# JacobChalk/TIM

Measured on AMD Instinct MI355X. Metric: interval-queries/sec (fwd+bwd), d=512 L=6 EPIC-100 window, higher is better.
Workload: dtype fp16; 1 GPU; C2a: EPIC-100 A+V recognition, d_model 512 (E 1024), 6 layers, 8 heads, 50+50 feature tokens, 15+10 interval queries, train-mode dropout; windows_per_gpu=64, global_batch=64, parallelism=dp1, precision=fp16

## Files before the change

### include/timhip.h

```cpp
#ifndef TIMHIP_H
#define TIMHIP_H

#include <stddef.h>
#include <stdint.h>

#ifdef __cplusplus
extern "C" {
#endif

#define TIMHIP_VERSION 6

enum {
  TIMHIP_OK = 0,
  TIMHIP_EINVAL = -1,
  TIMHIP_EUNSUPPORTED = -2,
  TIMHIP_EWORKSPACE = -3,
  TIMHIP_ELAUNCH = -4,
  TIMHIP_EALIGN = -5
};

enum { TIMHIP_PREC_BF16 = 0, TIMHIP_PREC_BF16X3 = 1, TIMHIP_PREC_FP32 = 2, TIMHIP_PREC_F16 = 3 };

enum {
  TIMHIP_EPI_STORE_T = 0,
  TIMHIP_EPI_RELU_T = 1,
  TIMHIP_EPI_STORE_F32 = 2,
  TIMHIP_EPI_GELU_DROP_T2 = 3,
  TIMHIP_EPI_DROP_RES_F32 = 4,
  TIMHIP_EPI_ADD_F32 = 5,
  TIMHIP_EPI_DGELU_T = 6,
  TIMHIP_EPI_DRELU_T = 7,
  TIMHIP_EPI_ATOMIC_F32 = 8,
  TIMHIP_EPI_SIGMOID_F32 = 9,
  TIMHIP_EPI_DRELU_F32IN_T = 10,
  TIMHIP_EPI_GELU_DROP_G2 = 11,
  TIMHIP_EPI_MULAUX_T = 12,
  TIMHIP_EPI_RELU_SPLIT3_T = 13,
  TIMHIP_EPI_GELU_T = 14
};

typedef struct TimDesc {
  int32_t B;
  int32_t S;
  int32_t F;
  int32_t d;
  int32_t E;
  int32_t H;
  int32_t FF;
  int32_t precision;
  float p_drop;
  uint64_t seed;
  int32_t layer;
  int32_t reserved;
  const float* grad_scale;
} TimDesc;
#define TIMHIP_DESC_ATTN_FP32 1
#define TIMHIP_DESC_ATTN_BWD_ONE_KERNEL 2
#define TIMHIP_DESC_WGRAD_OVERWRITE 4
#define TIMHIP_DESC_WGRAD_SEPARATE 8
#define TIMHIP_DESC_OUTPROJ_SPLIT 16
#define TIMHIP_DESC_INPROJ_SPLIT 32
#define TIMHIP_DESC_L1_SPLIT 64
#define TIMHIP_DESC_L2_SPLIT 128
#define TIMHIP_DESC_STREAM16 0x10000
#define TIMHIP_DESC_STREAM16_IN 0x20000
#define TIMHIP_DESC_STREAM16_OUT 0x40000
#define TIMHIP_DESC_ATTN_KEEP_BITS 0x80000

typedef struct TimLayerParams {
  const void *in_w, *in_wt;
  const void *out_w, *out_wt;
  const void *l1_w, *l1_wt;
  const void *l2_w, *l2_wt;
  const float *in_b, *out_b, *l1_b, *l2_b;
  const float *n1_w, *n1_b, *n2_w, *n2_b;
} TimLayerParams;

typedef struct TimLayerGrads {
  float *in_w, *in_b, *out_w, *out_b, *l1_w, *l1_b, *l2_w, *l2_b;
  float *n1_w, *n1_b, *n2_w, *n2_b;
  float* ln_partials;
} TimLayerGrads;
size_t timhip_layer_ln_partial_bytes(const TimDesc* d);
int timhip_ln_partials_reduce(const float* partials, int nsets, int rows, int cols, float* const* dgamma,
                              float* const* dbeta, void* stream);

int timhip_version(void);
void timhip_reload_env(void);
int timhip_gemm_p8_choice(int epi, int M, int N, int K);
int timhip_build_flags(void);
const char* timhip_strerror(int code);

size_t timhip_layer_saved_bytes(const TimDesc* d);
size_t timhip_layer_workspace_bytes(const TimDesc* d);
enum { TIMHIP_SAVED_QKV = 0, TIMHIP_SAVED_O = 1, TIMHIP_SAVED_Y1 = 2, TIMHIP_SAVED_X1T = 3, TIMHIP_SAVED_H = 4,
       TIMHIP_SAVED_Y2 = 5, TIMHIP_SAVED_FFN_KEEP_BITS = 6, TIMHIP_SAVED_ATTN_KEEP_BITS = 7 };
int timhip_layer_saved_field(const TimDesc* d, int field, size_t* offset, size_t* bytes);

int timhip_cast_weight(int precision, const float* src, int rows, int cols, void* dst, int ld,
                       int transpose, void* stream);

int timhip_cast_weight_both(int precision, const float* src, int rows, int cols, void* plain, int ldp,
                            void* tr, int ldt, void* stream);

typedef struct TimCastItem {
  const float* src;
  void* plain;
  void* tr;
  int32_t rows, cols, ldp, ldt;
} TimCastItem;
int timhip_cast_weights(int precision, const TimCastItem* items, int n, void* stream);

enum { TIMHIP_OPT_STEP = 0, TIMHIP_OPT_LR = 1, TIMHIP_OPT_NORM = 2, TIMHIP_OPT_COEF = 3, TIMHIP_OPT_FOUND_INF = 4,
       TIMHIP_OPT_SKIPPED = 5, TIMHIP_OPT_BC1 = 6, TIMHIP_OPT_BC2_SQRT = 7 };
#define TIMHIP_OPT_STATE_WORDS 8

typedef struct TimOptItem {
  float* p;
  const float* g;
  float* m;
  float* v;
  void* plain;
  void* tr;
  int32_t rows, cols, ldp, ldt;
} TimOptItem;

int timhip_optim_norm_partials(const TimOptItem* items, int n);

int timhip_optim_norm(const TimOptItem* items, int n, double* partials, void* stream);

int timhip_optim_finish(const double* partials, int n_partials, const uint32_t* const* flags, int n_flags, float max_norm,
                        float* const* states, const double* beta1, const double* beta2, int n_states, void* stream);

int timhip_optim_update(int precision, const TimOptItem* items, int n, const float* state, double beta1, double beta2,
                        double eps, double weight_decay, void* stream);

typedef struct TimEpi {
  void* out0;
  void* out1;
  const float* bias;
  const float* res;
  const void* aux;
  int32_t ld0, ld1, ldres, ldaux;
  float p_drop;
  uint32_t site;
  uint64_t seed;
  const void* mask;
  int32_t ldmask;
  int32_t reserved;
  const float* ln_stats;
  const float* ln_w;
  const float* ln_b;
  const float* acc_scale;
  int32_t a_wrap_k;
  int32_t reserved2;
} TimEpi;

typedef struct TimGemmItem {
  const void* A; const void* B;
  int32_t lda, ldb, M, N, K, reserved;
  TimEpi e;
} TimGemmItem;
int timhip_gemm_nt_group(int precision, int epi, const TimGemmItem* items, int n, void* stream);

int timhip_gemm_nt(int precision, int epi, const void* A, int lda, const void* B, int ldb, int M,
                   int N, int K, const TimEpi* e, int splitk, void* stream);

int timhip_transpose(int precision, const void* src, int rows, int cols, int lds, void* dst, int ld,
                     void* stream);

int timhip_colsum(int precision, const void* src, int rows, int cols, int ld, float* out,
                  void* stream);

int timhip_split3_many(int precision, int count, const float* const* src, const int* rows, const int* cols, const int* lds,
                       void* const* dst, const int* ldd, int mode, int relu, void* stream);

int timhip_dp_reduce(int wire_bf16, const void* recv, int world, long long per, float scale, void* out, void* stream);

int timhip_grad_scale(const float* const* cot, const long long* counts, int n, float target, float* out, void* stream);

int timhip_cast_rows(int precision, const float* src, int rows, int cols, int lds, void* dst, int ld,
                     float p_drop, uint64_t seed, uint32_t site, const float* scale, void* stream);
int timhip_cast_rows_pair(int precision, const float* const* src, const int* cols, void* const* dst, const int* ld, int rows,
                          float p_drop, uint64_t seed, const uint32_t* sites, void* stream);

int timhip_layernorm_fwd(int precision, const float* y, int rows, int cols, int ldy, int act,
                         const float* w, const float* b, float* x_f32, int ldx, void* x_T, int ldt,
                         float* stats, void* stream);
int timhip_layernorm_bwd(int precision, const float* dx, int lddx, const float* y, int ldy,
                         const float* stats, int rows, int cols, int act, const float* w,
                         float* dy_f32, int lddy, void* dy_T, int ldt, float p_drop, uint64_t seed,
                         uint32_t site, float* dgamma, float* dbeta, const float* t_scale, void* stream);
int timhip_layernorm_fwd2(int precision, const float* y, int rows, int cols, int ldy, int act, const float* w, const float* b,
                          int split_row, const float* w2, const float* b2, float* x_f32, int ldx, void* x_T, int ldt, float* stats,
                          void* stream);
int timhip_layernorm_bwd2(int precision, const float* dx, int lddx, const float* y, int ldy, const float* stats, int rows, int cols,
                          int act, const float* w, int split_row, const float* w2, float* dy_f32, int lddy, void* dy_T, int ldt,
                          float* dgamma, float* dbeta, float* dgamma2, float* dbeta2, const float* t_scale, void* stream);

int timhip_attention_fwd(const TimDesc* d, const void* qkv, void* o, float* lse, void* stream);
int timhip_attention_fwd_rows(const TimDesc* d, const void* qkv, int s0, void* o_rows, void* stream);
int timhip_attn_keep_bits(const TimDesc* d, int nlayers, void* const* saved, void* stream);
int timhip_attention_bwd(const TimDesc* d, const void* qkv, const void* o, const float* lse,
                         const void* d_o, void* dqkv, void* workspace, size_t workspace_bytes,
                         void* stream);
size_t timhip_attention_bwd_workspace_bytes(const TimDesc* d);

size_t timhip_wgrad_workspace_bytes(int precision, int Nout, int Kout, int M);
int timhip_wgrad(int precision, const void* dY, int ldy, int Nout, const void* X, int ldx, int Kout,
                 int M, float* dW, float* db, void* workspace, size_t workspace_bytes, const float* out_scale, void* stream);

typedef struct TimWgradItem {
  const void* dY;
  const void* X;
  float* dW;
  float* db;
  int32_t ldy, ldx, Nout, Kout;
} TimWgradItem;
size_t timhip_wgrad_group_workspace_bytes(int precision, const TimWgradItem* items, int n, int M);
int timhip_wgrad_group(int precision, const TimWgradItem* items, int n, int M, int accumulate, void* workspace,
                       size_t workspace_bytes, const float* out_scale, void* stream);

int timhip_dropout_rows_bwd(const float* g, int rows, int cols, int ldg, float* dx, int ldx,
                            float p_drop, uint64_t seed, uint32_t site, void* stream);

int timhip_time_l1_fwd(int precision, const float* times, int rows, int d, const float* w,
                       const float* b, void* h, int ld, void* stream);
int timhip_time_l1_fwd_split3(int precision, const float* times, int rows, int d, const float* w, const float* b, void* h3,
                              int ld, void* stream);
int timhip_time_l1_bwd(int precision, const float* times, int rows, int d, const float* w,
                       const void* dh, int ld, float* dw, float* db, float* dt, const float* out_scale, void* stream);

int timhip_dropout_mask(uint64_t seed, uint32_t site, float p, int rows, int cols, uint8_t* out,
                        void* stream);

int timhip_dropout_salt(const unsigned long long* dev_salt);

int timhip_layer_fwd(const TimDesc* d, const TimLayerParams* w, const float* x_in,
                     const void* x_in_T, float* x_out, void* x_out_T, void* saved, void* workspace,
                     size_t workspace_bytes, void* stream);
int timhip_layer_fwd_chained(const TimDesc* d, const TimLayerParams* w, const TimLayerParams* prev_w,
                             const void* prev_saved, const void* x_in_T, float* x_out, void* x_out_T, void* saved,
                             void* stream);
size_t timhip_stack_infer_workspace_bytes(const TimDesc* d, int nlayers, int tail_only);
int timhip_stack_infer(const TimDesc* d, int nlayers, const TimLayerParams* layers, const float* x_in, const void* x_in_T,
                       float* x_out, void* x_out_T, int tail_only, void* workspace, size_t workspace_bytes, void* stream);
int timhip_layer_bwd(const TimDesc* d, const TimLayerParams* w, const void* x_in_T,
                     const void* saved, float* dx_out, float* dx_in, const TimLayerGrads* g,
                     void* workspace, size_t workspace_bytes, void* stream);

size_t timhip_layer_dy_bytes(const TimDesc* d);
// ... 195 lines not shown
```

### tim_amd/_lib.py

```python
import ctypes as C
import os

_HERE = os.path.dirname(os.path.abspath(__file__))
LIB_PATH = os.environ.get("TIM_AMD_LIB") or os.path.join(_HERE, "libtimhip.so")

ABI_VERSION = 6
PREC_BF16, PREC_BF16X3, PREC_FP32, PREC_F16 = 0, 1, 2, 3
PRECISIONS = {"bf16": PREC_BF16, "bf16x3": PREC_BF16X3, "fp32": PREC_FP32, "fp16": PREC_F16}
H16 = (PREC_BF16, PREC_F16)

(EPI_STORE_T, EPI_RELU_T, EPI_STORE_F32, EPI_GELU_DROP_T2, EPI_DROP_RES_F32, EPI_ADD_F32,
 EPI_DGELU_T, EPI_DRELU_T, EPI_ATOMIC_F32, EPI_SIGMOID_F32, EPI_DRELU_F32IN_T, EPI_GELU_DROP_G2, EPI_MULAUX_T, EPI_RELU_SPLIT3_T,
 EPI_GELU_T) = range(15)

SITE_FEAT_V, SITE_FEAT_A, SITE_SEQ = 1, 2, 3
SITE_L_ATTN, SITE_L_DROP1, SITE_L_FFN, SITE_L_DROP2 = 0, 1, 2, 3


def layer_site(layer, which):
    return 16 + 8 * layer + which


SAVED_QKV, SAVED_O, SAVED_Y1, SAVED_X1T, SAVED_H, SAVED_Y2, SAVED_FFN_KEEP_BITS, SAVED_ATTN_KEEP_BITS = range(8)

vp, i32, u32, u64, f32, sz = C.c_void_p, C.c_int32, C.c_uint32, C.c_uint64, C.c_float, C.c_size_t


class TimDesc(C.Structure):
    _fields_ = [("B", i32), ("S", i32), ("F", i32), ("d", i32), ("E", i32), ("H", i32), ("FF", i32),
                ("precision", i32), ("p_drop", f32), ("seed", u64), ("layer", i32), ("reserved", i32),
                ("grad_scale", vp)]


_LP = ["in_w", "in_wt", "out_w", "out_wt", "l1_w", "l1_wt", "l2_w", "l2_wt",
       "in_b", "out_b", "l1_b", "l2_b", "n1_w", "n1_b", "n2_w", "n2_b"]
_LG = ["in_w", "in_b", "out_w", "out_b", "l1_w", "l1_b", "l2_w", "l2_b", "n1_w", "n1_b", "n2_w", "n2_b", "ln_partials"]


class TimLayerParams(C.Structure):
    _fields_ = [(n, vp) for n in _LP]


class TimLayerGrads(C.Structure):
    _fields_ = [(n, vp) for n in _LG]


DESC_ATTN_FP32, DESC_ATTN_BWD_ONE_KERNEL, DESC_WGRAD_OVERWRITE, DESC_WGRAD_SEPARATE, DESC_OUTPROJ_SPLIT = 1, 2, 4, 8, 16
DESC_INPROJ_SPLIT, DESC_L1_SPLIT, DESC_L2_SPLIT = 32, 64, 128
DESC_STREAM16, DESC_STREAM16_IN, DESC_STREAM16_OUT = 0x10000, 0x20000, 0x40000
EINVAL, EUNSUPPORTED, EWORKSPACE, ELAUNCH, EALIGN = -1, -2, -3, -4, -5
DESC_ATTN_KEEP_BITS = 0x80000


class TimCastItem(C.Structure):
    _fields_ = [("src", vp), ("plain", vp), ("tr", vp), ("rows", i32), ("cols", i32), ("ldp", i32), ("ldt", i32)]


class TimOptItem(C.Structure):
    _fields_ = [("p", vp), ("g", vp), ("m", vp), ("v", vp), ("plain", vp), ("tr", vp),
                ("rows", i32), ("cols", i32), ("ldp", i32), ("ldt", i32)]


OPT_STEP, OPT_LR, OPT_NORM, OPT_COEF, OPT_FOUND_INF, OPT_SKIPPED, OPT_BC1, OPT_BC2_SQRT = range(8)
OPT_STATE_WORDS, OPT_MAX_FLAGS, OPT_MAX_STATES = 8, 32, 8


class TimWgradItem(C.Structure):
    _fields_ = [("dY", vp), ("X", vp), ("dW", vp), ("db", vp), ("ldy", i32), ("ldx", i32), ("Nout", i32), ("Kout", i32)]


class TimEpi(C.Structure):
    _fields_ = [("out0", vp), ("out1", vp), ("bias", vp), ("res", vp), ("aux", vp),
                ("ld0", i32), ("ld1", i32), ("ldres", i32), ("ldaux", i32),
                ("p_drop", f32), ("site", u32), ("seed", u64), ("mask", vp), ("ldmask", i32), ("reserved", i32),
                ("ln_stats", vp), ("ln_w", vp), ("ln_b", vp), ("acc_scale", vp), ("a_wrap_k", i32), ("reserved2", i32)]


class TimGemmItem(C.Structure):
    _fields_ = [("A", vp), ("B", vp), ("lda", i32), ("ldb", i32), ("M", i32), ("N", i32), ("K", i32), ("reserved", i32),
                ("e", TimEpi)]


class TimRecHead(C.Structure):
    _fields_ = [("logits", vp), ("sum", vp), ("ld", C.c_int64), ("C", i32), ("pitch", i32)]


REC_MAX_HEADS = 3


class TimAvga(C.Structure):
    _fields_ = [(n, vp) for n in ("video", "audio", "w_video", "w_audio", "w_v", "w_g", "w_v_t", "w_g_t", "w_video_s", "w_audio_s", "b_video",
                                  "b_audio", "w_h")] + [("pitch", C.c_int64)] + \
               [(n, i32) for n in ("R", "S", "Cv", "Ca", "H", "map_size", "ld_audio", "ld_w_video", "ld_w_audio", "ld_w_v", "ld_w_g",
                                   "ld_w_v_t", "ld_w_g_t", "ld_w_video_s", "ld_w_audio_s", "reserved")]


class TimAvgaGrads(C.Structure):
    _fields_ = [(n, vp) for n in ("w_video", "b_video", "w_audio", "b_audio", "w_v", "w_g", "w_h")]


_SIGS = {
    "timhip_version": (C.c_int, []),
    "timhip_strerror": (C.c_char_p, [C.c_int]),
    "timhip_layer_saved_bytes": (sz, [C.POINTER(TimDesc)]),
    "timhip_layer_workspace_bytes": (sz, [C.POINTER(TimDesc)]),
    "timhip_layer_saved_field": (C.c_int, [C.POINTER(TimDesc), i32, C.POINTER(sz), C.POINTER(sz)]),
    "timhip_cast_weight": (C.c_int, [i32, vp, i32, i32, vp, i32, i32, vp]),
    "timhip_cast_weight_both": (C.c_int, [i32, vp, i32, i32, vp, i32, vp, i32, vp]),
    "timhip_cast_weights": (C.c_int, [i32, vp, i32, vp]),
    "timhip_gemm_nt": (C.c_int, [i32, i32, vp, i32, vp, i32, i32, i32, i32, C.POINTER(TimEpi), i32, vp]),
    "timhip_gemm_nt_group": (C.c_int, [i32, i32, vp, i32, vp]),
    "timhip_wgrad_workspace_bytes": (sz, [i32, i32, i32, i32]),
    "timhip_wgrad": (C.c_int, [i32, vp, i32, i32, vp, i32, i32, i32, vp, vp, vp, sz, vp, vp]),
    "timhip_wgrad_group_workspace_bytes": (sz, [i32, vp, i32, i32]),
    "timhip_wgrad_group": (C.c_int, [i32, vp, i32, i32, i32, vp, sz, vp, vp]),
    "timhip_transpose": (C.c_int, [i32, vp, i32, i32, i32, vp, i32, vp]),
    "timhip_colsum": (C.c_int, [i32, vp, i32, i32, i32, vp, vp]),
    "timhip_cast_rows": (C.c_int, [i32, vp, i32, i32, i32, vp, i32, f32, u64, u32, vp, vp]),
    "timhip_dropout_rows_bwd": (C.c_int, [vp, i32, i32, i32, vp, i32, f32, u64, u32, vp]),
    "timhip_layernorm_fwd": (C.c_int, [i32, vp, i32, i32, i32, i32, vp, vp, vp, i32, vp, i32, vp, vp]),
    "timhip_layernorm_bwd": (C.c_int, [i32, vp, i32, vp, i32, vp, i32, i32, i32, vp, vp, i32, vp, i32,
                                       f32, u64, u32, vp, vp, vp, vp]),
    "timhip_attention_fwd": (C.c_int, [C.POINTER(TimDesc), vp, vp, vp, vp]),
    "timhip_attention_fwd_rows": (C.c_int, [C.POINTER(TimDesc), vp, i32, vp, vp]),
    "timhip_attention_bwd": (C.c_int, [C.POINTER(TimDesc), vp, vp, vp, vp, vp, vp, sz, vp]),
    "timhip_attention_bwd_workspace_bytes": (sz, [C.POINTER(TimDesc)]),
    "timhip_time_l1_fwd": (C.c_int, [i32, vp, i32, i32, vp, vp, vp, i32, vp]),
    "timhip_time_l1_fwd_split3": (C.c_int, [i32, vp, i32, i32, vp, vp, vp, i32, vp]),
# ... 9 lines not shown
                                   C.POINTER(TimLayerGrads), vp, sz, vp]),
    "timhip_layer_bwd_split": (C.c_int, [C.POINTER(TimDesc), C.POINTER(TimLayerParams), vp, vp, vp, vp, vp, vp,
                                         C.POINTER(TimLayerGrads), vp, sz, vp]),
    "timhip_layer_bwd_data_split": (C.c_int, [C.POINTER(TimDesc), C.POINTER(TimLayerParams), vp, vp, vp, vp, vp, vp,
                                              C.POINTER(TimLayerGrads), vp, sz, vp]),
    "timhip_layer_dy_bytes": (sz, [C.POINTER(TimDesc)]),
    "timhip_layer_data_workspace_bytes": (sz, [C.POINTER(TimDesc)]),
    "timhip_layer_wgrad_workspace_bytes": (sz, [C.POINTER(TimDesc)]),
    "timhip_layer_bwd_data": (C.c_int, [C.POINTER(TimDesc), C.POINTER(TimLayerParams), vp, vp, vp, vp,
                                        C.POINTER(TimLayerGrads), vp, sz, vp]),
    "timhip_layer_bwd_weights": (C.c_int, [C.POINTER(TimDesc), vp, vp, vp, C.POINTER(TimLayerGrads), vp, sz, vp]),
    "timhip_layer_bwd_weights_pair": (C.c_int, [C.POINTER(TimDesc), vp, vp, vp, C.POINTER(TimLayerGrads), vp, vp, vp,
                                                C.POINTER(TimLayerGrads), vp, sz, vp]),
    "timhip_layer_wgrad_pair_wins": (C.c_int, [C.POINTER(TimDesc)]),
    "timhip_assemble_fwd": (C.c_int, [i32, vp, i32, i32, i32, vp, vp, i32, vp, vp, i32, vp, f32, u64, u32,
                                      vp, vp, vp]),
    "timhip_assemble_bwd": (C.c_int, [vp, i32, i32, i32, vp, i32, i32, f32, u64, u32, vp, vp, vp, vp, vp, vp]),
    "timhip_assemble_fwd_p": (C.c_int, [i32, vp, i32, i32, i32, vp, vp, i32, vp, i32, vp, i32, vp, i32, f32, u64, u32, vp, vp, vp]),
    "timhip_assemble_bwd_p": (C.c_int, [vp, i32, i32, i32, vp, i32, i32, f32, u64, u32, vp, vp, vp, i32, vp, vp, i32, vp]),
    "timhip_gather_rows": (C.c_int, [i32, vp, i32, i32, i32, i32, i32, vp, vp]),
    "timhip_ce_mixup_fwd": (C.c_int, [vp, i32, i32, i32, vp, vp, f32, f32, vp, vp, vp, vp]),
    "timhip_ce_mixup_bwd": (C.c_int, [vp, i32, i32, i32, vp, vp, f32, f32, vp, vp, vp, vp, i32, vp]),
    "timhip_focal_loss_fwd": (C.c_int, [vp, vp, i32, i32, vp, vp, f32, f32, vp, vp, vp]),
    "timhip_focal_loss_bwd": (C.c_int, [vp, vp, i32, i32, vp, vp, f32, f32, vp, vp, vp]),
    "timhip_diou_1d": (C.c_int, [vp, vp, i32, vp, f32, vp, vp, vp, vp]),
    "timhip_det_side_loss_fwd": (C.c_int, [vp, vp, vp, i32, i32, vp, vp, vp, f32, f32, f32, f32, f32, f32, vp, vp, vp]),
    "timhip_det_side_loss_bwd": (C.c_int, [vp, vp, vp, i32, i32, vp, vp, vp, f32, f32, f32, f32, f32, vp, vp, vp, vp, vp]),
    "timhip_softnms_1d_workspace_bytes": (C.c_size_t, [C.c_int64, i32]),
    "timhip_softnms_1d": (C.c_int, [vp, vp, vp, vp, i32, f32, f32, f32, i32, vp, vp, vp, vp, C.c_size_t, vp]),
    "timhip_nms_1d": (C.c_int, [vp, vp, vp, i32, f32, vp, vp, vp, vp]),
    "timhip_det_candidates_count": (C.c_int, [vp, C.c_int64, vp, vp, f32, vp, i32, i32, i32, f32, vp, vp, vp, vp]),
    "timhip_det_candidates_emit": (C.c_int, [vp, C.c_int64, vp, vp, vp, vp, i32, i32, i32, f32, C.c_int64, vp, vp, vp, vp, vp]),
    "timhip_ts_candidates_count": (C.c_int, [vp, C.c_int64, vp, C.c_int64, vp, vp, vp, f32, vp, i32, i32, i32, i32, i32, f32, f32, f32,
                                             vp, vp, vp, vp, vp, vp, vp]),
    "timhip_ts_candidates_emit": (C.c_int, [vp, vp, vp, vp, vp, vp, i32, i32, i32, i32, i32, C.c_int64, vp, vp, vp, vp, vp]),
    "timhip_det_match": (C.c_int, [vp, C.c_int64, vp, vp, vp, vp, vp, C.c_int64, vp, i32, vp, i32, vp, vp, vp, vp]),
    "timhip_det_ap": (C.c_int, [vp, C.c_int64, vp, vp, i32, i32, vp, vp]),
    "timhip_rec_accumulate": (C.c_int, [vp, i32, vp, vp, vp, C.c_int64, i32, i32, i32, i32, vp, vp, vp, vp, vp, vp]),
    "timhip_rec_finalize": (C.c_int, [vp, i32, i32, vp, vp, i32, i32, vp, i32, vp, vp, vp]),
    "timhip_rec_counts": (C.c_int, [vp, vp, vp, i32, vp, vp]),
    "timhip_window_gather": (C.c_int, [vp, i32, i32, vp, vp, i32, vp, i32, vp, vp, vp]),
    "timhip_window_times": (C.c_int, [vp, i32, vp, vp, i32, vp, vp, i32, vp, i32, vp, i32, vp, i32, vp, f32, vp, vp]),
    "timhip_gemm_timing_start": (C.c_int, [i32, C.c_double]),
    "timhip_gemm_timing_stop": (C.c_int, [vp, vp, vp]),
    "timhip_timing_stop_families": (C.c_int, [vp, vp, vp]),
    "timhip_drloc_gather": (C.c_int, [i32, vp, vp, C.c_int64, C.c_int64, i32, i32, i32, vp, vp, i32, vp, i32, vp]),
    "timhip_drloc_scatter_add": (C.c_int, [vp, i32, vp, vp, C.c_int64, C.c_int64, i32, i32, i32, vp, vp, i32, vp]),
    "timhip_scatter_rows_add": (C.c_int, [vp, i32, i32, i32, i32, i32, vp, vp]),
    "timhip_layer_ln_partial_bytes": (sz, [C.POINTER(TimDesc)]),
    "timhip_ln_partials_reduce": (C.c_int, [vp, i32, i32, i32, vp, vp, vp]),
    "timhip_gather_ranges": (C.c_int, [i32, vp, i32, i32, i32, i32, vp, vp, vp, vp]),
    "timhip_layernorm_fwd2": (C.c_int, [i32, vp, i32, i32, i32, i32, vp, vp, i32, vp, vp, vp, i32, vp, i32, vp, vp]),
    "timhip_layernorm_bwd2": (C.c_int, [i32, vp, i32, vp, i32, vp, i32, i32, i32, vp, i32, vp, vp, i32, vp, i32, vp, vp, vp, vp, vp, vp]),
    "timhip_cast_rows_pair": (C.c_int, [i32, vp, vp, vp, vp, i32, f32, u64, vp, vp]),
    "timhip_gather_split3_ranges": (C.c_int, [i32, vp, i32, i32, i32, i32, vp, vp, vp, vp]),
    "timhip_scatter_ranges_add": (C.c_int, [i32, i32, i32, i32, vp, vp, vp, vp, vp]),
    "timhip_dx_init": (C.c_int, [i32, i32, i32, i32, vp, i32, vp, vp, vp, vp, vp]),
    "timhip_sigmoid_bwd_rows": (C.c_int, [i32, vp, vp, i32, i32, vp, i32, vp, vp]),
    "timhip_dx_init_slabs": (C.c_int, [i32, i32, i32, i32, vp, i32, vp, vp, vp, vp, vp, vp]),
    "timhip_cast_rows_many": (C.c_int, [i32, i32, vp, vp, vp, vp, vp, vp, vp]),
    "timhip_grad_scale": (C.c_int, [vp, vp, i32, f32, vp, vp]),
    "timhip_reload_env": (None, []),
    "timhip_build_flags": (C.c_int, []),
    "timhip_attn_keep_bits": (C.c_int, [C.POINTER(TimDesc), i32, vp, vp]),
    "timhip_gemm_p8_choice": (C.c_int, [i32, i32, i32, i32]),
    "timhip_dp_reduce": (C.c_int, [i32, vp, i32, C.c_longlong, f32, vp, vp]),
    "timhip_split3_many": (C.c_int, [i32, i32, vp, vp, vp, vp, vp, vp, i32, i32, vp]),
    "timhip_label_queries": (C.c_int, [vp, vp, vp, i32, i32, i32, i32, f32, vp, vp, vp, vp]),
    "timhip_optim_norm_partials": (C.c_int, [vp, i32]),
    "timhip_optim_norm": (C.c_int, [vp, i32, vp, vp]),
    "timhip_optim_finish": (C.c_int, [vp, i32, vp, i32, f32, vp, vp, vp, i32, vp]),
    "timhip_optim_update": (C.c_int, [i32, vp, i32, vp, C.c_double, C.c_double, C.c_double, C.c_double, vp]),
    "timhip_smooth_one_hot": (C.c_int, [vp, i32, i32, C.c_int64, i32, f32, f32, vp, vp]),
    "timhip_avga_workspace_bytes": (sz, [i32, i32, i32, i32, i32, i32]),
    "timhip_avga_fwd": (C.c_int, [i32, C.POINTER(TimAvga), vp, i32, vp, i32, vp, sz, vp]),
    "timhip_avga_bwd": (C.c_int, [i32, C.POINTER(TimAvga), vp, i32, C.POINTER(TimAvgaGrads), vp, vp, sz, vp]),
}

_lib = None


class TimHipError(RuntimeError):
    pass


def load():
    global _lib
    if _lib is not None:
        return _lib
    if not os.path.exists(LIB_PATH):
        raise TimHipError("libtimhip.so not found at %s: build it with `python -c 'import __graft_entry__ as g; "
                          "g.build()'` (make -C tim_amd/csrc). There is no CPU fallback." % LIB_PATH)
    lib = C.CDLL(LIB_PATH)
    lib.timhip_version.restype = C.c_int
    if lib.timhip_version() != ABI_VERSION:
        raise TimHipError("%s is ABI version %d, this binding speaks %d: rebuild it (make -C tim_amd/csrc%s)"
                          % (LIB_PATH, lib.timhip_version(), ABI_VERSION, " TUNING=1" if "tuning" in LIB_PATH else ""))
    for name, (res, args) in _SIGS.items():
        fn = getattr(lib, name)
        fn.restype = res
        fn.argtypes = args
    _lib = lib
    return lib


def reload_env():
# ... 24 lines not shown
```

### tim_amd/csrc/api.hip

```cpp
#include <atomic>
#include "common.h"

namespace {

struct SavedLayout {
  Field qkv, o, lse, y1, st1, x1t, u, h, y2, st2, ffn_mask, attn_keep;
  size_t total;
};

SavedLayout saved_layout(const TimDesc& d) {
  const size_t M = (size_t)d.B * d.S, ts = opsize(d.precision);
  Arena a;
  SavedLayout L;
  L.qkv = a.take(M * 3 * d.E * ts);
  L.o = a.take(M * d.E * ts);
  L.lse = a.take((size_t)d.B * d.H * d.S * 4);
  L.y1 = a.take(M * d.E * 4);
  L.st1 = a.take(M * 2 * 4);
  L.x1t = a.take(M * d.E * ts);
  L.u = a.take(M * d.FF * ts);
  L.h = a.take(M * d.FF * ts);
  L.y2 = a.take(M * d.E * 4);
  L.st2 = a.take(M * 2 * 4);
  L.ffn_mask = a.take(M * d.FF / 8);
  L.attn_keep = a.take((size_t)d.B * d.H * d.S * 16);
  L.total = a.total();
  return L;
}

struct DyLayout { Field df, du, da, dqkv; size_t total; };
DyLayout dy_layout(const TimDesc& d) {
  const size_t M = (size_t)d.B * d.S, ts = opsize(d.precision);
  Arena a;
  DyLayout L;
  L.df = a.take(M * d.E * ts);
  L.du = a.take(M * d.FF * ts);
  L.da = a.take(M * d.E * ts);
  L.dqkv = a.take(M * 3 * d.E * ts);
  L.total = a.total();
  return L;
}

void layer_products(const TimDesc& d, const void* saved, const void* dy, const void* x_in_T, const TimLayerGrads* g,
                    TimWgradItem it[4]) {
  const SavedLayout L = saved_layout(d);
  const DyLayout Y = dy_layout(d);
  const int E = d.E, FF = d.FF;
  auto in = [](const void* base, const Field& f) { return base ? (const void*)f.at(base) : nullptr; };
  it[0] = TimWgradItem{in(dy, Y.df), in(saved, L.h), g ? g->l2_w : nullptr, g ? g->l2_b : nullptr, E, FF, E, FF};
  it[1] = TimWgradItem{in(dy, Y.du), in(saved, L.x1t), g ? g->l1_w : nullptr, g ? g->l1_b : nullptr, FF, E, FF, E};
  it[2] = TimWgradItem{in(dy, Y.da), in(saved, L.o), g ? g->out_w : nullptr, g ? g->out_b : nullptr, E, E, E, E};
  it[3] = TimWgradItem{in(dy, Y.dqkv), x_in_T, g ? g->in_w : nullptr, g ? g->in_b : nullptr, 3 * E, E, 3 * E, E};
}

int splitk_for(int Mout, int Nout, int Kp) {
  const int tiles = ((Mout + 127) / 128) * ((Nout + 127) / 128);
  int sk = (512 + tiles - 1) / tiles;
  const int maxk = Kp / 256 > 0 ? Kp / 256 : 1;
  if (sk > maxk) sk = maxk;
  if (sk > 8) sk = 8;
  if (sk < 1) sk = 1;
  return sk;
}

struct WgradWs { Field tA, tB, slab; size_t total; };
WgradWs wgrad_ws(int prec, int Nout, int Kout, int M) {
  const size_t Mp = round_up(M, 64), ts = opsize(prec);
  Arena a;
  WgradWs w{};
  if (h16_storage(prec)) {
    w.total = tim_wgrad_tn_ws(Nout, Kout, M);
    return w;
  }
  w.tA = a.take((size_t)Nout * Mp * ts);
  w.tB = a.take((size_t)Kout * Mp * ts);
  const int sk = splitk_for(Nout, Kout, (int)Mp);
  w.slab = a.take(sk > 1 ? (size_t)sk * Nout * Kout * 4 : 0);
  w.total = a.total();
  return w;
}

struct WsLayout {
  Field f32a, f32b, Tb, Tc, wg, attn, lnp;
  size_t total;
};

WsLayout ws_layout(const TimDesc& d) {
  const size_t M = (size_t)d.B * d.S, ts = opsize(d.precision);
  TimWgradItem it[4];
  layer_products(d, nullptr, nullptr, nullptr, nullptr, it);
  size_t wg = h16_storage(d.precision) ? tim_wgrad_group_ws(it, 4, (int)M) : 0;
  for (int i = 0; i < 4; ++i) {
    if (i == 2) continue;
    const size_t one = wgrad_ws(d.precision, it[i].Nout, it[i].Kout, (int)M).total;
    if (one > wg) wg = one;
  }
  Arena a;
  WsLayout L;
  L.f32a = a.take(M * d.E * 4);
  L.f32b = a.take(M * d.E * 4);
  L.Tb = a.take(M * d.E * ts);
  L.Tc = a.take(M * d.E * ts);
  L.wg = a.take(wg);
  L.attn = a.take(tim_attention_bwd_ws(d));
  L.lnp = a.take(tim_layernorm_bwd_ws((int)M, d.E));
  L.total = a.total();
  return L;
}

int check_layer_desc(const TimDesc& d) {
  if (d.B <= 0 || d.S <= 0 || d.F <= 0 || d.F > d.S || d.E <= 0 || d.H <= 0 || d.FF <= 0) return TIMHIP_EINVAL;
  if (d.E % 64 || d.FF % 64 || d.E % d.H) return TIMHIP_EUNSUPPORTED;
  if (!valid_precision(d.precision)) return TIMHIP_EUNSUPPORTED;
  if (d.p_drop < 0.f || d.p_drop >= 1.f) return TIMHIP_EINVAL;
  return TIMHIP_OK;
}

TimEpi epi0() {
  TimEpi e;
  e.out0 = e.out1 = nullptr; e.bias = e.res = nullptr; e.aux = nullptr;
  e.ld0 = e.ld1 = e.ldres = e.ldaux = 0; e.p_drop = 0.f; e.site = 0; e.seed = 0;
  e.mask = nullptr; e.ldmask = 0; e.reserved = 0; e.a_wrap_k = 0; e.reserved2 = 0;
  e.ln_stats = e.ln_w = e.ln_b = nullptr;
  e.acc_scale = nullptr;
  return e;
}

int wgrad(int prec, const void* dY, int ldy, int Nout, const void* X, int ldx, int Kout, int M, float* dW, float* db,
          void* ws, size_t ws_bytes, hipStream_t s, int accumulate = 1, const float* out_scale = nullptr) {
  const int Mp = round_up(M, 64);
  const WgradWs W = wgrad_ws(prec, Nout, Kout, M);
  if (ws_bytes < W.total) return TIMHIP_EWORKSPACE;
  if (h16_storage(prec)) return tim_wgrad_tn_h16(prec, dY, ldy, Nout, X, ldx, Kout, M, dW, db, ws, ws_bytes, s, accumulate, out_scale);
  if (!accumulate || out_scale) return TIMHIP_EUNSUPPORTED;
  char* w = (char*)ws;
  void* tA = W.tA.at(w); void* tB = W.tB.at(w); float* slab = (float*)W.slab.at(w);
  int rc;
  if ((rc = tim_transpose(prec, dY, M, Nout, ldy, tA, Mp, db, s))) return rc;
  if ((rc = tim_transpose(prec, X, M, Kout, ldx, tB, Mp, nullptr, s))) return rc;
  const int sk = splitk_for(Nout, Kout, Mp);
  TimEpi e = epi0();
  if (sk == 1 || (Kout % 4) != 0) {
    e.out0 = dW; e.ld0 = Kout;
    return tim_gemm_nt(prec, TIMHIP_EPI_ATOMIC_F32, tA, Mp, tB, Mp, Nout, Kout, Mp, e, sk, s);
  }
  e.out0 = slab; e.ld0 = Kout;
  if ((rc = tim_gemm_nt(prec, TIMHIP_EPI_STORE_F32, tA, Mp, tB, Mp, Nout, Kout, Mp, e, sk, s))) return rc;
  return tim_slab_reduce(slab, (long long)Nout * Kout, sk, dW, s);
}

struct LayerPass {
  const float* gs_in;
  const float* gs_out;
  int accumulate;
  const unsigned long long* akeep;
};
LayerPass layer_pass(const TimDesc& d, const unsigned long long* keep_bits = nullptr) {
  LayerPass P;
  P.gs_in = (d.precision == TIMHIP_PREC_F16 && d.grad_scale) ? d.grad_scale : nullptr;
  P.gs_out = P.gs_in ? P.gs_in + 1 : nullptr;
  P.accumulate = (d.reserved & TIMHIP_DESC_WGRAD_OVERWRITE) ? 0 : 1;
  P.akeep = ((d.reserved & TIMHIP_DESC_ATTN_KEEP_BITS) && d.p_drop > 0.f) ? keep_bits : nullptr;
  return P;
}

bool wgrad_grouped(const TimDesc& d) { return h16_storage(d.precision) && !(d.reserved & TIMHIP_DESC_WGRAD_SEPARATE); }

int linear_fwd(int prec, int epi, const void* A, const void* W, int M, int N, int K, bool split, TimEpi e, hipStream_t s) {
  if (!split) return tim_gemm_nt(prec, epi, A, K, W, K, M, N, K, e, 1, s);
  e.a_wrap_k = K; e.reserved = 2;
  return tim_gemm_nt(prec, epi, A, K, W, 3 * K, M, N, 2 * K, e, 1, s);
}

}

// ... 49 lines not shown
}

int timhip_dropout_salt(const unsigned long long* dev_salt) {
  tim_salt_ptr = dev_salt;
  return TIMHIP_OK;
}

const char* timhip_strerror(int code) {
  switch (code) {
    case TIMHIP_OK: return "ok";
    case TIMHIP_EINVAL: return "invalid argument (null pointer or bad descriptor field)";
    case TIMHIP_EUNSUPPORTED: return "shape or precision not supported by the gfx950 kernels";
    case TIMHIP_EWORKSPACE: return "workspace too small";
    case TIMHIP_ELAUNCH: return "HIP kernel launch failed";
    case TIMHIP_EALIGN: return "pointer or leading dimension not aligned";
    default: return "unknown timhip error";
  }
}

int timhip_attn_keep_bits(const TimDesc* d, int nlayers, void* const* saved, void* stream) {
  if (!d || !saved || nlayers <= 0) return TIMHIP_EINVAL;
  if (!h16_storage(d->precision) || !(d->p_drop > 0.f) || d->B <= 0 || d->S <= 0 || d->H <= 0 || d->E / d->H != 128 ||
      (d->F + 31) / 32 != 4)
    return TIMHIP_EUNSUPPORTED;
  const SavedLayout L = saved_layout(*d);
  for (int l0 = 0; l0 < nlayers; l0 += 8) {
    unsigned long long* out[8] = {};
    const int n = nlayers - l0 < 8 ? nlayers - l0 : 8;
    for (int i = 0; i < n; ++i) {
      if (!saved[l0 + i]) return TIMHIP_EINVAL;
      out[i] = reinterpret_cast<unsigned long long*>(L.attn_keep.at(saved[l0 + i]));
    }
    const int rc = tim_attn_keep_bits(*d, l0, n, out, (hipStream_t)stream);
    if (rc) return rc;
  }
  return TIMHIP_OK;
}

size_t timhip_layer_saved_bytes(const TimDesc* d) { return d ? saved_layout(*d).total : 0; }

int timhip_layer_saved_field(const TimDesc* d, int field, size_t* offset, size_t* bytes) {
  if (!d || !offset || !bytes) return TIMHIP_EINVAL;
  const SavedLayout L = saved_layout(*d);
  const Field* f;
  switch (field) {
    case TIMHIP_SAVED_QKV: f = &L.qkv; break;
    case TIMHIP_SAVED_O: f = &L.o; break;
    case TIMHIP_SAVED_Y1: f = &L.y1; break;
    case TIMHIP_SAVED_X1T: f = &L.x1t; break;
    case TIMHIP_SAVED_H: f = &L.h; break;
    case TIMHIP_SAVED_Y2: f = &L.y2; break;
    case TIMHIP_SAVED_FFN_KEEP_BITS: f = &L.ffn_mask; break;
    case TIMHIP_SAVED_ATTN_KEEP_BITS: f = &L.attn_keep; break;
    default: return TIMHIP_EINVAL;
  }
  *offset = f->off; *bytes = f->bytes;
  return TIMHIP_OK;
}

int timhip_gemm_nt(int precision, int epi, const void* A, int lda, const void* B, int ldb, int M, int N, int K,
                   const TimEpi* e, int splitk, void* stream) {
  if (!e) return TIMHIP_EINVAL;
  return tim_gemm_nt(precision, epi, A, lda, B, ldb, M, N, K, *e, splitk, (hipStream_t)stream);
}

size_t timhip_wgrad_workspace_bytes(int precision, int Nout, int Kout, int M) {
  return wgrad_ws(precision, Nout, Kout, M).total;
}

int timhip_gemm_nt_group(int precision, int epi, const TimGemmItem* items, int n, void* stream) {
  return tim_gemm_nt_group(precision, epi, items, n, (hipStream_t)stream);
}

size_t timhip_wgrad_group_workspace_bytes(int precision, const TimWgradItem* items, int n, int M) {
  return (h16_storage(precision) && items && n > 0) ? tim_wgrad_group_ws(items, n, M) : 0;
}

int timhip_wgrad_group(int precision, const TimWgradItem* items, int n, int M, int accumulate, void* workspace,
                       size_t workspace_bytes, const float* out_scale, void* stream) {
  return tim_wgrad_group_h16(precision, items, n, M, accumulate, workspace, workspace_bytes, out_scale, (hipStream_t)stream);
}

int timhip_wgrad(int precision, const void* dY, int ldy, int Nout, const void* X, int ldx, int Kout, int M,
                 float* dW, float* db, void* workspace, size_t workspace_bytes, const float* out_scale, void* stream) {
  if (!dY || !X || !dW || !workspace) return TIMHIP_EINVAL;
  return wgrad(precision, dY, ldy, Nout, X, ldx, Kout, M, dW, db, workspace, workspace_bytes, (hipStream_t)stream, 1, out_scale);
}

struct LayerBufs {
  void* qkv; void* o; float* lse; float* y1; float* st1; void* x1t; void* u; void* h; float* y2; float* st2;
  uint8_t* ffn_mask; const unsigned long long* attn_keep;
};

static LayerBufs saved_bufs(const TimDesc& d, void* saved) {
  const SavedLayout L = saved_layout(d);
  return LayerBufs{L.qkv.at(saved), L.o.at(saved), (float*)L.lse.at(saved), (float*)L.y1.at(saved), (float*)L.st1.at(saved),
                   L.x1t.at(saved), L.u.at(saved), L.h.at(saved), (float*)L.y2.at(saved), (float*)L.st2.at(saved),
                   (uint8_t*)L.ffn_mask.at(saved), reinterpret_cast<const unsigned long long*>(L.attn_keep.at(saved))};
}

static int layer_fwd_body(const TimDesc& d, const TimLayerParams* w, const float* x_in, const float* x_in_prenorm,
                          const float* x_in_stats, const float* x_in_lnw, const float* x_in_lnb, const void* x_in_T,
                          float* x_out, void* x_out_T, const LayerBufs& bufs, int s0, hipStream_t s) {
  int rc;
  const int Mall = d.B * d.S, M = d.B * (d.S - s0), E = d.E, FF = d.FF, prec = d.precision;
  void* qkv = bufs.qkv; void* o = bufs.o; float* y1 = bufs.y1; float* st1 = bufs.st1; void* x1t = bufs.x1t;
  void* u = bufs.u; void* h = bufs.h; float* y2 = bufs.y2; float* st2 = bufs.st2;

  auto split = [&](int flag) { return (d.reserved & flag) != 0 && h16_storage(prec); };
  TimEpi e = epi0();
  e.out0 = qkv; e.ld0 = 3 * E; e.bias = w->in_b;
  if ((rc = linear_fwd(prec, TIMHIP_EPI_STORE_T, x_in_T, w->in_w, Mall, 3 * E, E, split(TIMHIP_DESC_INPROJ_SPLIT), e, s))) return rc;
  if ((rc = tim_attention_fwd(d, qkv, o, bufs.lse, s, layer_pass(d, bufs.attn_keep).akeep, s0))) return rc;
  e = epi0();
  e.out0 = y1; e.ld0 = E; e.bias = w->out_b; e.ldres = E;
  if (x_in) {
    e.res = x_in;
  } else {
    e.res = x_in_prenorm; e.ln_stats = x_in_stats; e.ln_w = x_in_lnw; e.ln_b = x_in_lnb;
  }
  e.p_drop = d.p_drop; e.seed = d.seed; e.site = layer_site(d.layer, SITE_L_DROP1);
  uint8_t* fmask = d.p_drop > 0.f ? bufs.ffn_mask : nullptr;
  const bool fuse_ln = tim_knobs().fuse_ln == 1;
  const uint32_t* ln_run_if = nullptr;
  bool fused1 = false;
  if (fuse_ln && h16_storage(prec) && !split(TIMHIP_DESC_OUTPROJ_SPLIT)) {
    TimLnFuse lf{x1t, E, nullptr, 0, st1, w->n1_w, w->n1_b, fmask, FF, d.p_drop, d.seed, layer_site(d.layer, SITE_L_FFN)};
    rc = tim_gemm_nt_fuse_ln(prec, o, E, w->out_w, E, M, E, E, e, lf, &ln_run_if, s);
    if (rc == TIMHIP_OK) fused1 = true;
    else if (rc != TIMHIP_EUNSUPPORTED) return rc;
  }
  if (!fused1 && (rc = linear_fwd(prec, TIMHIP_EPI_DROP_RES_F32, o, w->out_w, M, E, E, split(TIMHIP_DESC_OUTPROJ_SPLIT), e, s))) return rc;
  if ((rc = tim_layernorm_fwd(prec, y1, M, E, E, 0, w->n1_w, w->n1_b, nullptr, 0, x1t, E, st1, s, fmask, FF, d.p_drop, d.seed,
                              layer_site(d.layer, SITE_L_FFN), fused1 ? ln_run_if : nullptr))) return rc;
  e = epi0();
  e.out0 = h; e.ld0 = FF; e.bias = w->l1_b;
  const int epi1 = u ? TIMHIP_EPI_GELU_DROP_G2 : TIMHIP_EPI_GELU_T;
  if (u) {
    e.out1 = u; e.ld1 = FF;
    e.p_drop = d.p_drop; e.seed = d.seed; e.site = layer_site(d.layer, SITE_L_FFN);
    e.mask = fmask; e.ldmask = FF / 8;
  }
  if ((rc = linear_fwd(prec, epi1, x1t, w->l1_w, M, FF, E, split(TIMHIP_DESC_L1_SPLIT), e, s))) return rc;
  e = epi0();
  e.out0 = y2; e.ld0 = E; e.bias = w->l2_b; e.ldres = E;
  e.res = y1; e.ln_stats = st1; e.ln_w = w->n1_w; e.ln_b = w->n1_b;
  e.p_drop = d.p_drop; e.seed = d.seed; e.site = layer_site(d.layer, SITE_L_DROP2);
  bool fused2 = false;
  if (fuse_ln && h16_storage(prec) && !split(TIMHIP_DESC_L2_SPLIT)) {
    TimLnFuse lf{x_out_T, E, x_out, E, st2, w->n2_w, w->n2_b, nullptr, 0, 0.f, 0, 0};
    rc = tim_gemm_nt_fuse_ln(prec, h, FF, w->l2_w, FF, M, E, FF, e, lf, &ln_run_if, s);
    if (rc == TIMHIP_OK) fused2 = true;
    else if (rc != TIMHIP_EUNSUPPORTED) return rc;
  }
  if (!fused2 && (rc = linear_fwd(prec, TIMHIP_EPI_DROP_RES_F32, h, w->l2_w, M, E, FF, split(TIMHIP_DESC_L2_SPLIT), e, s))) return rc;
  return tim_layernorm_fwd(prec, y2, M, E, E, 0, w->n2_w, w->n2_b, x_out, E, x_out_T, E, st2, s, nullptr, 0, 0.f, 0, 0,
                           fused2 ? ln_run_if : nullptr);
}

int timhip_layer_fwd(const TimDesc* dp, const TimLayerParams* w, const float* x_in, const void* x_in_T, float* x_out,
                     void* x_out_T, void* saved, void* workspace, size_t workspace_bytes, void* stream) {
  (void)workspace; (void)workspace_bytes;
  if (!dp || !w || !x_in || !x_in_T || !x_out_T || !saved) return TIMHIP_EINVAL;
  int rc = check_layer_desc(*dp);
  if (rc) return rc;
  return layer_fwd_body(*dp, w, x_in, nullptr, nullptr, nullptr, nullptr, x_in_T, x_out, x_out_T, saved_bufs(*dp, saved), 0,
                        (hipStream_t)stream);
}

int timhip_layer_fwd_chained(const TimDesc* dp, const TimLayerParams* w, const TimLayerParams* prev_w, const void* prev_saved,
                             const void* x_in_T, float* x_out, void* x_out_T, void* saved, void* stream) {
  if (!dp || !w || !prev_w || !prev_saved || !x_in_T || !x_out_T || !saved) return TIMHIP_EINVAL;
  int rc = check_layer_desc(*dp);
  if (rc) return rc;
  const SavedLayout L = saved_layout(*dp);
  return layer_fwd_body(*dp, w, nullptr, (const float*)L.y2.at(prev_saved), (const float*)L.st2.at(prev_saved), prev_w->n2_w,
                        prev_w->n2_b, x_in_T, x_out, x_out_T, saved_bufs(*dp, saved), 0, (hipStream_t)stream);
}

struct InferLayout { Field qkv, o, y1, st1, x1t, h, y2, st2, xt, resg, stg; size_t total; };
static InferLayout infer_layout(const TimDesc& d, int tail_only) {
  const size_t M = (size_t)d.B * d.S, Mt = (size_t)d.B * (d.S - d.F), ts = opsize(d.precision);
  Arena a;
  InferLayout L;
  L.qkv = a.take(M * 3 * d.E * ts);
  L.o = a.take(M * d.E * ts);
  L.y1 = a.take(M * d.E * 4);
  L.st1 = a.take(M * 2 * 4);
  L.x1t = a.take(M * d.E * ts);
  L.h = a.take(M * d.FF * ts);
  L.y2 = a.take(M * d.E * 4);
  L.st2 = a.take(M * 2 * 4);
  L.xt = a.take(M * d.E * ts);
  L.resg = a.take(tail_only ? Mt * d.E * 4 : 0);
  L.stg = a.take(tail_only ? Mt * 2 * 4 : 0);
  L.total = a.total();
  return L;
}

size_t timhip_stack_infer_workspace_bytes(const TimDesc* d, int nlayers, int tail_only) {
  (void)nlayers;
  return (d && check_layer_desc(*d) == TIMHIP_OK) ? infer_layout(*d, tail_only).total : 0;
}

int timhip_stack_infer(const TimDesc* dp, int nlayers, const TimLayerParams* layers, const float* x_in, const void* x_in_T,
                       float* x_out, void* x_out_T, int tail_only, void* workspace, size_t workspace_bytes, void* stream) {
  if (!dp || !layers || nlayers <= 0 || !x_in || !x_in_T || !x_out_T || !workspace) return TIMHIP_EINVAL;
  TimDesc d = *dp;
  int rc = check_layer_desc(d);
  if (rc) return rc;
  if (d.p_drop != 0.f || (tail_only && d.S == d.F)) return TIMHIP_EINVAL;
  const InferLayout L = infer_layout(d, tail_only);
  if (workspace_bytes < L.total) return TIMHIP_EWORKSPACE;
  hipStream_t s = (hipStream_t)stream;
  void* ws = workspace;
  const LayerBufs bufs{L.qkv.at(ws), L.o.at(ws), nullptr, (float*)L.y1.at(ws), (float*)L.st1.at(ws), L.x1t.at(ws), nullptr,
                       L.h.at(ws), (float*)L.y2.at(ws), (float*)L.st2.at(ws), nullptr, nullptr};
  d.reserved &= ~TIMHIP_DESC_ATTN_KEEP_BITS;
  for (int l = 0; l < nlayers; ++l) {
    const bool last = l == nlayers - 1;
    const int s0 = (last && tail_only) ? d.F : 0;
    d.layer = l;
    const float* res = l == 0 ? x_in : nullptr;
    const float* pre = l == 0 ? nullptr : bufs.y2;
    const float* pst = l == 0 ? nullptr : bufs.st2;
    if (s0) {
      float* resg = (float*)L.resg.at(ws); float* stg = (float*)L.stg.at(ws);
      if ((rc = timhip_gather_rows(TIMHIP_PREC_FP32, l == 0 ? x_in : pre, d.B, d.S, d.E, s0, d.S - s0, resg, stream))) return rc;
      if (l > 0 && (rc = timhip_gather_rows(TIMHIP_PREC_FP32, pst, d.B, d.S, 2, s0, d.S - s0, stg, stream))) return rc;
      if (l == 0) res = resg; else { pre = resg; pst = stg; }
    }
    const void* in_T = l == 0 ? x_in_T : (const void*)L.xt.at(ws);
    if ((rc = layer_fwd_body(d, &layers[l], res, pre, pst, l ? layers[l - 1].n2_w : nullptr, l ? layers[l - 1].n2_b : nullptr, in_T,
                             last ? x_out : nullptr, last ? x_out_T : (void*)L.xt.at(ws), bufs, s0, s))) return rc;
  }
  return TIMHIP_OK;
}

size_t timhip_layer_ln_partial_bytes(const TimDesc* d) { return d ? 2 * tim_layernorm_bwd_ws(d->B * d->S, d->E) : 0; }
size_t timhip_layer_dy_bytes(const TimDesc* d) { return d ? dy_layout(*d).total : 0; }
size_t timhip_layer_workspace_bytes(const TimDesc* d) { return d ? ws_layout(*d).total + dy_layout(*d).total : 0; }
size_t timhip_layer_data_workspace_bytes(const TimDesc* d) { return d ? ws_layout(*d).total : 0; }
size_t timhip_layer_wgrad_workspace_bytes(const TimDesc* d) { return d ? ws_layout(*d).wg.bytes : 0; }

static int layer_bwd_data_impl(const TimDesc& d, const TimLayerParams* w, const void* saved, const float* dx_out,
                               const void* dx_out_add, float* dx_in, void* dx_in_add, void* dy, const TimLayerGrads* g,
                               void* workspace, size_t workspace_bytes, hipStream_t s) {
  int rc = check_layer_desc(d);
  if (rc) return rc;
  const WsLayout W = ws_layout(d);
  if (workspace_bytes < W.total) return TIMHIP_EWORKSPACE;
  const int M = d.B * d.S, E = d.E, FF = d.FF, prec = d.precision;
  const SavedLayout L = saved_layout(d);
  const DyLayout Y = dy_layout(d);
  const void* qkv = L.qkv.at(saved); const void* o = L.o.at(saved); const float* lse = (const float*)L.lse.at(saved);
  const float* y1 = (const float*)L.y1.at(saved); const float* st1 = (const float*)L.st1.at(saved);
  const void* u = L.u.at(saved);
  const float* y2 = (const float*)L.y2.at(saved); const float* st2 = (const float*)L.st2.at(saved);
  void* ws = workspace;
  float* f32a = (float*)W.f32a.at(ws); float* f32b = (float*)W.f32b.at(ws); float* lnp = (float*)W.lnp.at(ws);
  void* Tb = W.Tb.at(ws); void* Tc = W.Tc.at(ws);
  void* df = Y.df.at(dy); void* du = Y.du.at(dy); void* da = Y.da.at(dy); void* dqkv = Y.dqkv.at(dy);
  const LayerPass P = layer_pass(d, reinterpret_cast<const unsigned long long*>(L.attn_keep.at(saved)));
  const float* gs_in = P.gs_in; const float* gs_out = P.gs_out;

  const bool s16 = gs_in != nullptr && (d.reserved & TIMHIP_DESC_STREAM16) != 0;
  const bool s16_in = s16 && (d.reserved & TIMHIP_DESC_STREAM16_IN) != 0;
  const bool s16_out = s16 && (d.reserved & TIMHIP_DESC_STREAM16_OUT) != 0;
  if (((d.reserved & (TIMHIP_DESC_STREAM16_IN | TIMHIP_DESC_STREAM16_OUT)) != 0 && !s16) || (s16_out && !dx_in_add)) return TIMHIP_EINVAL;
  if ((rc = tim_layernorm_bwd(prec, dx_out, E, y2, E, st2, M, E, 0, w->n2_w, f32a, E, df, E, d.p_drop, d.seed,
                              layer_site(d.layer, SITE_L_DROP2), g->n2_w, g->n2_b,
                              g->ln_partials ? g->ln_partials : lnp, s, g->ln_partials != nullptr, gs_in,
                              dx_out_add, E, gs_out, (s16_in ? 1 : 0) | (s16 ? 2 : 0)))) return rc;
  TimEpi e = epi0();
  e.out0 = du; e.ld0 = FF; e.aux = u; e.ldaux = FF;
  if ((rc = tim_gemm_nt(prec, TIMHIP_EPI_MULAUX_T, df, E, w->l2_wt, E, M, FF, E, e, 1, s))) return rc;
  const bool branch_split = prec != TIMHIP_PREC_BF16;
  e = epi0();
  if (branch_split) {
    e.out0 = Tb; e.ld0 = E;
    if ((rc = tim_gemm_nt(prec, TIMHIP_EPI_STORE_T, du, FF, w->l1_wt, FF, M, E, FF, e, 1, s))) return rc;
  } else {
    e.out0 = f32b; e.ld0 = E; e.res = f32a; e.ldres = E;
    if ((rc = tim_gemm_nt(prec, TIMHIP_EPI_ADD_F32, du, FF, w->l1_wt, FF, M, E, FF, e, 1, s))) return rc;
  }
  const float* ln1_in = branch_split ? f32a : f32b;
  float* dy1 = dx_in_add ? dx_in : (branch_split ? f32b : f32a);
  if ((rc = tim_layernorm_bwd(prec, ln1_in, E, y1, E, st1, M, E, 0, w->n1_w, dy1, E, da, E, d.p_drop, d.seed,
                              layer_site(d.layer, SITE_L_DROP1), g->n1_w, g->n1_b,
                              g->ln_partials ? g->ln_partials + tim_layernorm_bwd_ws(M, E) / sizeof(float) : lnp, s,
                              g->ln_partials != nullptr, gs_in, branch_split ? Tb : nullptr, E, gs_out,
                              (s16 ? 1 : 0) | (s16_out ? 2 : 0)))) return rc;
  e = epi0();
  e.out0 = Tc; e.ld0 = E;
  if ((rc = tim_gemm_nt(prec, TIMHIP_EPI_STORE_T, da, E, w->out_wt, E, M, E, E, e, 1, s))) return rc;
  if ((rc = tim_attention_bwd(d, qkv, o, lse, Tc, dqkv, W.attn.at(ws), W.attn.bytes, s, P.akeep))) return rc;
  e = epi0();
  if (dx_in_add) {
    e.out0 = dx_in_add; e.ld0 = E;
    return tim_gemm_nt(prec, TIMHIP_EPI_STORE_T, dqkv, 3 * E, w->in_wt, 3 * E, M, E, 3 * E, e, 1, s);
  }
  e.out0 = dx_in; e.ld0 = E; e.res = dy1; e.ldres = E; e.acc_scale = gs_out;
  return tim_gemm_nt(prec, TIMHIP_EPI_ADD_F32, dqkv, 3 * E, w->in_wt, 3 * E, M, E, 3 * E, e, 1, s);
}

int timhip_layer_bwd_data(const TimDesc* dp, const TimLayerParams* w, const void* saved, float* dx_out, float* dx_in,
                          void* dy, const TimLayerGrads* g, void* workspace, size_t workspace_bytes, void* stream) {
  if (!dp || !w || !saved || !dx_out || !dx_in || !dy || !g || !workspace) return TIMHIP_EINVAL;
  return layer_bwd_data_impl(*dp, w, saved, dx_out, nullptr, dx_in, nullptr, dy, g, workspace, workspace_bytes, (hipStream_t)stream);
}

int timhip_layer_bwd_data_split(const TimDesc* dp, const TimLayerParams* w, const void* saved, const float* dx_out,
                                const void* dx_out_add, float* dx_in, void* dx_in_add, void* dy, const TimLayerGrads* g,
                                void* workspace, size_t workspace_bytes, void* stream) {
  if (!dp || !w || !saved || !dx_out || !dx_in || !dy || !g || !workspace) return TIMHIP_EINVAL;
  return layer_bwd_data_impl(*dp, w, saved, dx_out, dx_out_add, dx_in, dx_in_add, dy, g, workspace, workspace_bytes,
                             (hipStream_t)stream);
}

int timhip_layer_bwd_weights(const TimDesc* dp, const void* x_in_T, const void* saved, const void* dy,
                             const TimLayerGrads* g, void* workspace, size_t workspace_bytes, void* stream) {
  if (!dp || !x_in_T || !saved || !dy || !g || !workspace) return TIMHIP_EINVAL;
  const TimDesc& d = *dp;
  int rc = check_layer_desc(d);
  if (rc) return rc;
  const int M = d.B * d.S;
  hipStream_t s = (hipStream_t)stream;
  const LayerPass P = layer_pass(d);
  TimWgradItem it[4];
  layer_products(d, saved, dy, x_in_T, g, it);
  if (wgrad_grouped(d)) return tim_wgrad_group_h16(d.precision, it, 4, M, P.accumulate, workspace, workspace_bytes, P.gs_out, s);
  for (const TimWgradItem& p : it)
    if ((rc = wgrad(d.precision, p.dY, p.ldy, p.Nout, p.X, p.ldx, p.Kout, M, p.dW, p.db, workspace, workspace_bytes, s, P.accumulate,
                    P.gs_out))) return rc;
  return TIMHIP_OK;
}

int timhip_layer_bwd_weights_pair(const TimDesc* dp, const void* x_in_T_a, const void* saved_a, const void* dy_a, const TimLayerGrads* ga,
                                  const void* x_in_T_b, const void* saved_b, const void* dy_b, const TimLayerGrads* gb,
                                  void* workspace, size_t workspace_bytes, void* stream) {
  if (!dp || !x_in_T_a || !saved_a || !dy_a || !ga || !x_in_T_b || !saved_b || !dy_b || !gb || !workspace) return TIMHIP_EINVAL;
  const TimDesc& d = *dp;
  int rc = check_layer_desc(d);
  if (rc) return rc;
  if (!wgrad_grouped(d)) return TIMHIP_EUNSUPPORTED;
// ... 44 lines not shown
```

### tim_amd/csrc/common.h

```cpp
#pragma once
#include <hip/hip_runtime.h>
#include <stdint.h>

#include "../../include/timhip.h"

typedef __bf16 bf16_t;
typedef _Float16 f16_t;
template <typename T> using vec8 = T __attribute__((ext_vector_type(8)));
template <typename T> using vec4 = T __attribute__((ext_vector_type(4)));
typedef vec8<bf16_t> bf16x8_t;
typedef vec4<bf16_t> bf16x4_t;
typedef float f32x4_t __attribute__((ext_vector_type(4)));
typedef float f32x16_t __attribute__((ext_vector_type(16)));
typedef short s16x4_t __attribute__((ext_vector_type(4)));

#define TIM_CHECK_LAUNCH()                                   \
  do {                                                       \
    if (hipGetLastError() != hipSuccess) return TIMHIP_ELAUNCH; \
  } while (0)

static inline int round_up(int x, int m) { return (x + m - 1) / m * m; }
__host__ __device__ static inline size_t align_up(size_t x, size_t a) { return (x + a - 1) / a * a; }

struct Field {
// ... 89 lines not shown
__host__ __device__ __forceinline__ Philox4 philox4x32_7(uint64_t seed, uint32_t site, uint64_t ctr) {
  uint32_t k0 = (uint32_t)seed, k1 = (uint32_t)(seed >> 32);
  uint32_t c0 = (uint32_t)ctr, c1 = (uint32_t)(ctr >> 32), c2 = site, c3 = 0x7149u;
#pragma unroll
  for (int r = 0; r < PHILOX_ROUNDS; ++r) {
    const uint64_t p0 = (uint64_t)0xD2511F53u * (uint64_t)c0, p1 = (uint64_t)0xCD9E8D57u * (uint64_t)c2;
    const uint32_t hi0 = (uint32_t)(p0 >> 32), lo0 = (uint32_t)p0, hi1 = (uint32_t)(p1 >> 32), lo1 = (uint32_t)p1;
    uint32_t n0 = hi1 ^ c1 ^ k0, n1 = lo1, n2 = hi0 ^ c3 ^ k1, n3 = lo0;
    c0 = n0; c1 = n1; c2 = n2; c3 = n3;
    k0 += 0x9E3779B9u; k1 += 0xBB67AE85u;
  }
  return Philox4{c0, c1, c2, c3};
}

extern const unsigned long long* tim_salt_ptr;
struct TimSeed {
  uint64_t base;
  const unsigned long long* salt;
  __host__ __device__ TimSeed() : base(0), salt(nullptr) {}
  __host__ TimSeed(uint64_t s) : base(s), salt(tim_salt_ptr) {}
  __device__ __forceinline__ operator uint64_t() const { return salt ? base + (uint64_t)*salt : base; }
};

__host__ __device__ __forceinline__ uint32_t drop_threshold(float p) {
  double t = (double)p * 4294967296.0;
  if (t < 0) t = 0;
  if (t > 4294967295.0) t = 4294967295.0;
  return (uint32_t)t;
}

__device__ __forceinline__ void drop_mask4(uint64_t seed, uint32_t site, uint64_t q, uint32_t thr,
                                           float scale, float& m0, float& m1, float& m2, float& m3) {
  const Philox4 r = philox4x32_7(seed, site, q >> 1);
  const uint32_t a = (q & 1) ? r.z : r.x, b = (q & 1) ? r.w : r.y, t = thr >> 16;
  m0 = (a & 0xffffu) >= t ? scale : 0.f;
  m1 = (a >> 16) >= t ? scale : 0.f;
  m2 = (b & 0xffffu) >= t ? scale : 0.f;
  m3 = (b >> 16) >= t ? scale : 0.f;
}
__device__ __forceinline__ void drop_mask4_words(uint32_t a, uint32_t b, uint32_t thr, float scale, float& m0, float& m1,
                                                 float& m2, float& m3) {
  const uint32_t t = thr >> 16;
  m0 = (a & 0xffffu) >= t ? scale : 0.f;
  m1 = (a >> 16) >= t ? scale : 0.f;
  m2 = (b & 0xffffu) >= t ? scale : 0.f;
  m3 = (b >> 16) >= t ? scale : 0.f;
}
__device__ __forceinline__ float drop_mask1(uint64_t seed, uint32_t site, uint64_t idx, uint32_t thr, float scale) {
  const Philox4 r = philox4x32_7(seed, site, idx >> 3);
  const int e = (int)(idx & 7), wsel = e >> 1;
  const uint32_t w = wsel == 0 ? r.x : (wsel == 1 ? r.y : (wsel == 2 ? r.z : r.w));
  return ((w >> (16 * (e & 1))) & 0xffffu) >= (thr >> 16) ? scale : 0.f;
}
__device__ __forceinline__ uint32_t drop_bits8(uint64_t seed, uint32_t site, uint64_t c, uint32_t thr) {
  const Philox4 r = philox4x32_7(seed, site, c);
  const uint32_t t = thr >> 16;
  return ((r.x & 0xffffu) >= t ? 1u : 0u) | ((r.x >> 16) >= t ? 2u : 0u) | ((r.y & 0xffffu) >= t ? 4u : 0u) |
         ((r.y >> 16) >= t ? 8u : 0u) | ((r.z & 0xffffu) >= t ? 16u : 0u) | ((r.z >> 16) >= t ? 32u : 0u) |
         ((r.w & 0xffffu) >= t ? 64u : 0u) | ((r.w >> 16) >= t ? 128u : 0u);
}

__device__ __forceinline__ uint32_t drop_bits32(uint64_t seed, uint32_t site, uint64_t q0, uint32_t thr) {
  uint32_t bits = 0;
#pragma unroll
  for (int j = 0; j < 4; ++j) bits |= drop_bits8(seed, site, (q0 >> 1) + j, thr) << (8 * j);
  return bits;
}
__device__ __forceinline__ void drop_mask4_bits(uint32_t nib, float scale, float& m0, float& m1, float& m2, float& m3) {
  m0 = (nib & 1u) ? scale : 0.f;
  m1 = (nib & 2u) ? scale : 0.f;
  m2 = (nib & 4u) ? scale : 0.f;
  m3 = (nib & 8u) ? scale : 0.f;
}

struct PerDeviceOnce {
  bool done[32] = {};
  bool first() {
    int dev = 0;
    (void)hipGetDevice(&dev);
    dev = dev < 0 ? 0 : (dev > 31 ? 31 : dev);
    if (done[dev]) return false;
    done[dev] = true;
    return true;
  }
};

enum {
  SITE_FEAT_V = 1, SITE_FEAT_A = 2, SITE_SEQ = 3,
  SITE_L_BASE = 16, SITE_L_ATTN = 0, SITE_L_DROP1 = 1, SITE_L_FFN = 2, SITE_L_DROP2 = 3, SITE_L_STRIDE = 8
};
static inline uint32_t layer_site(int layer, int which) {
  return SITE_L_BASE + (uint32_t)layer * SITE_L_STRIDE + (uint32_t)which;
}

__device__ __forceinline__ float erf_half_f(float x, float& e) {
  const float z = fabsf(x) * 0.70710678118654752440f;
  const float t = __builtin_amdgcn_rcpf(fmaf(0.3275911f, z, 1.0f));
  e = __expf(-0.5f * x * x);
  float p = fmaf(1.061405429f, t, -1.453152027f);
  p = fmaf(p, t, 1.421413741f);
  p = fmaf(p, t, -0.284496736f);
  p = fmaf(p, t, 0.254829592f);
  const float r = fmaf(-p * t, e, 1.0f);
  return copysignf(r, x);
}
__device__ __forceinline__ float gelu_f(float x) {
  float e;
  return 0.5f * x * (1.0f + erf_half_f(x, e));
}
__device__ __forceinline__ float gelu_grad_f(float x) {
  const float kInvSqrt2Pi = 0.3989422804014327f;
  float e;
// ... 127 lines not shown
  asm volatile("s_waitcnt vmcnt(%0)" ::"n"(N) : "memory");
}

struct TimGemmScope {
  TimGemmScope(double flops, hipStream_t s, int family = 0);
  ~TimGemmScope();
  int slot;
  hipStream_t stream;
};

int tim_gemm_nt(int precision, int epi, const void* A, int lda, const void* B, int ldb, int M, int N,
                int K, const TimEpi& e, int splitk, hipStream_t s);
int tim_gemm_nt_group(int precision, int epi, const TimGemmItem* items, int n, hipStream_t s);
bool tim_gemm_pp_wins(int M, int N, int K, int splitk);
int tim_gemm_p8_choice(int epi, int M, int N, int K);
struct TimLnFuse {
  void* xt; int ldt; float* xf; int ldx; float* stats; const float* g; const float* b;
  uint8_t* mask_out; int mask_cols; float mask_p; uint64_t mask_seed; uint32_t mask_site;
};
int tim_gemm_nt_pp_ln(int precision, const void* A, int lda, const void* B, int ldb, int M, int N, int K, const void* epi_dev,
                      const TimLnFuse& lf, const uint32_t** fail, hipStream_t s);
int tim_gemm_nt_fuse_ln(int precision, const void* A, int lda, const void* B, int ldb, int M, int N, int K, const TimEpi& te,
                        const TimLnFuse& lf, const uint32_t** fail, hipStream_t s);
int tim_gemm_nt_pp(int precision, int epi, const void* A, int lda, const void* B, int ldb, int M, int N, int K, const void* epi_dev,
                   hipStream_t s);
int tim_transpose(int precision, const void* src, int rows, int cols, int lds, void* dst, int ld,
                  float* colsum, hipStream_t s);
int tim_slab_reduce(const float* slab, long long n, int nslab, float* dW, hipStream_t s);
size_t tim_wgrad_tn_ws(int Nout, int Kout, int M);
int tim_wgrad_tn_h16(int precision, const void* dY, int ldy, int Nout, const void* X, int ldx, int Kout, int M, float* dW,
                     float* db, void* ws, size_t ws_bytes, hipStream_t s, int accumulate = 1, const float* out_scale = nullptr);
size_t tim_wgrad_group_ws(const TimWgradItem* it, int n, int M);
int tim_wgrad_group_splits(const TimWgradItem* it, int n, int M);
int tim_wgrad_group_h16(int precision, const TimWgradItem* it, int n, int M, int accumulate, void* ws, size_t ws_bytes,
                        const float* out_scale, hipStream_t s);
bool tim_wgrad_pp_wins(const TimWgradItem* it, int n, int M);
int tim_wgrad_group_pp(int precision, const TimWgradItem* it, int n, int M, int accumulate, const float* out_scale, hipStream_t s);
bool tim_wgrad_p8_wins(const TimWgradItem* it, int n, int M);
int tim_wgrad_group_p8(int precision, const TimWgradItem* it, int n, int M, int accumulate, const float* out_scale, hipStream_t s);
int tim_colsum(int precision, const void* src, int rows, int cols, int ld, float* out, hipStream_t s);
int tim_layernorm_fwd(int precision, const float* y, int rows, int cols, int ldy, int act,
                      const float* w, const float* b, float* x_f32, int ldx, void* x_T, int ldt,
                      float* stats, hipStream_t s, uint8_t* mask_out = nullptr, int mask_cols = 0, float mask_p = 0.f,
                      uint64_t mask_seed = 0, uint32_t mask_site = 0,
                      const uint32_t* run_if = nullptr,
                      int split_row = 0, const float* w2 = nullptr, const float* b2 = nullptr);
int tim_layernorm_bwd(int precision, const float* dx, int lddx, const float* y, int ldy,
                      const float* stats, int rows, int cols, int act, const float* w, float* dy_f32,
                      int lddy, void* dy_T, int ldt, float p_drop, uint64_t seed, uint32_t site,
                      float* dgamma, float* dbeta, float* partial_ws, hipStream_t s, bool defer_colsum = false,
                      const float* t_scale = nullptr,
                      const void* add_T = nullptr, int ldadd = 0, const float* add_scale = nullptr,
                      int stream16 = 0,
                      int split_row = 0, const float* w2 = nullptr, float* dgamma2 = nullptr, float* dbeta2 = nullptr);
size_t tim_layernorm_bwd_ws(int rows, int cols);
int tim_layernorm_bwd_blocks(int rows);
int tim_attention_fwd(const TimDesc& d, const void* qkv, void* o, float* lse, hipStream_t s, const unsigned long long* kbits = nullptr,
                      int s0 = 0);
int tim_attention_bwd(const TimDesc& d, const void* qkv, const void* o, const float* lse,
                      const void* d_o, void* dqkv, void* ws, size_t ws_bytes, hipStream_t s, const unsigned long long* kbits = nullptr);
int tim_attn_keep_bits(const TimDesc& d, int first_layer, int n, unsigned long long* const* out, hipStream_t s);
size_t tim_attention_bwd_ws(const TimDesc& d);

static inline bool h16_storage(int precision) { return precision == TIMHIP_PREC_BF16 || precision == TIMHIP_PREC_F16; }
static inline bool f32_storage(int precision) { return !h16_storage(precision); }
static inline bool valid_precision(int precision) { return precision >= TIMHIP_PREC_BF16 && precision <= TIMHIP_PREC_F16; }
#define DISPATCH_T(prec, ...)                                           \
  do {                                                                  \
    if (f32_storage(prec)) { using T = float; __VA_ARGS__; }            \
    else if ((prec) == TIMHIP_PREC_F16) { using T = f16_t; __VA_ARGS__; } \
    else { using T = bf16_t; __VA_ARGS__; }                             \
  } while (0)
#define DISPATCH_H16(precision, ...)                                   \
  do {                                                                 \
    if ((precision) == TIMHIP_PREC_F16) { using HT = f16_t; __VA_ARGS__; } \
    else { using HT = bf16_t; __VA_ARGS__; }                            \
  } while (0)
static inline size_t opsize(int precision) { return f32_storage(precision) ? 4 : 2; }
```

### tim_amd/csrc/gemm.hip

```cpp
#include <stdlib.h>

#include "gemm_epi.h"

namespace {

template <typename HT, int EPI, int BM, int BN, int WM, int WN, int BKT, int NST, int GM, int ABL = 0>
__device__ __forceinline__ void gemm_nt_h16_body(
    const HT* __restrict__ A, int lda, const HT* __restrict__ B, int ldb, int M, int N,
    int K, int ksteps_per_split, EpiDev e, int t, int zsplit) {
  constexpr int NW = WM * WN;
  constexpr int TM = BM / WM / 32, TN = BN / WN / 32;
  constexpr int ROWB = BKT * 2;
  constexpr int NCH = ROWB / 16;
  constexpr int RPI = 1024 / ROWB;
  constexpr int A_BYTES = BM * ROWB, B_BYTES = BN * ROWB, ST_BYTES = A_BYTES + B_BYTES;
  constexpr int A_INSTR = BM / RPI / NW, B_INSTR = BN / RPI / NW, LPS = A_INSTR + B_INSTR;
  static_assert(A_INSTR >= 1 && B_INSTR >= 1, "tile too small for the wave count");
  extern __shared__ __attribute__((aligned(16))) char lds[];

  const int tid = threadIdx.x, lane = tid & 63;
  const int wave = __builtin_amdgcn_readfirstlane(tid >> 6);
  const int wm = wave / WN, wn = wave % WN;

  const int tiles_n = (N + BN - 1) / BN, tiles_m = (M + BM - 1) / BM;
// ... 231 lines not shown
#pragma unroll
    for (int i = 0; i < TN; ++i)
#pragma unroll
      for (int q = 0; q < 4; ++q)
        *reinterpret_cast<float4*>(ep + frow * EP_LD + i * 32 + 8 * q + 4 * fhalf) =
            make_float4(acc[i][j][4 * q] * asc, acc[i][j][4 * q + 1] * asc, acc[i][j][4 * q + 2] * asc, acc[i][j][4 * q + 3] * asc);
    asm volatile("s_waitcnt lgkmcnt(0)" ::: "memory");
    if (epi_has_oct(EPI) && e.vec8) {
      constexpr int OPR = EP_COLS / 8;
#pragma unroll
      for (int it = 0; it < 32 * OPR / 64; ++it) {
        const int idx = it * 64 + lane;
        const int row = idx / OPR, ch = idx % OPR;
        const float4 lo = *reinterpret_cast<const float4*>(ep + row * EP_LD + ch * 8);
        const float4 hi = *reinterpret_cast<const float4*>(ep + row * EP_LD + ch * 8 + 4);
        const int m = m0 + wm * (BM / WM) + j * 32 + row;
        const int n = n0 + wn * (BN / WN) + ch * 8;
        if (m < M && n + 7 < N) {
          epi_oct<EPI, HT>(e, m, n, N, lo, hi, mbyte[j][it], pre_aux, abuf[j % PD][PRE_AUX ? it : 0], pre_b8, bias8[0], bias8[1]);
        } else if (m < M) {
          if (n < N) epi_quad<EPI, HT>(e, m, n, N, lo.x, lo.y, lo.z, lo.w);
          if (n + 4 < N) epi_quad<EPI, HT>(e, m, n + 4, N, hi.x, hi.y, hi.z, hi.w);
        }
      }
    } else {
      constexpr int NITQ_ = 32 * CPR / 64;
      bool has_k = false;
      if constexpr (EPI == TIMHIP_EPI_DROP_RES_F32 && (NITQ_ % 2) == 0) has_k = e.thr != 0u && !e.mask && e.vec && (N & 7) == 0 && e.pair;
      auto quad = [&](int it, bool hk, float4 kf) {
        const int idx = it * 64 + lane;
        const int row = idx / CPR, ch = idx % CPR;
        const float4 v = *reinterpret_cast<const float4*>(ep + row * EP_LD + ch * 4);
        const int m = m0 + wm * (BM / WM) + j * 32 + row;
        const int n = n0 + wn * (BN / WN) + ch * 4;
        if (m < M && n < N)
          epi_quad<EPI, HT>(e, m, n, N, v.x, v.y, v.z, v.w, pre_res && n + 3 < N, rbuf[j % PD][PRE_RES ? it : 0],
                                pre_b4 && n + 3 < N, bias4, pre_ln && pre_gb && n + 3 < N, sbuf[j % PD][PRE_RES ? it : 0],
                                lng, lnb, hk, kf);
      };
      if (has_k) {
        if constexpr ((NITQ_ % 2) == 0) {
#pragma unroll
          for (int it = 0; it < NITQ_; it += 2) {
            const int idx = (it + (lane & 1)) * 64 + (lane & ~1);
            const long long m_ = m0 + wm * (BM / WM) + j * 32 + idx / CPR, n_ = n0 + wn * (BN / WN) + (idx % CPR) * 4;
            const Philox4 r = philox4x32_7(e.seed, e.site, (uint64_t)(m_ * (long long)N + n_) >> 3);
            const bool odd = (lane & 1) != 0;
            const uint32_t sa = odd ? r.x : r.z, sb = odd ? r.y : r.w;
            const uint32_t pa = (uint32_t)__builtin_amdgcn_mov_dpp((int)sa, 0xB1, 0xF, 0xF, true);
            const uint32_t pb = (uint32_t)__builtin_amdgcn_mov_dpp((int)sb, 0xB1, 0xF, 0xF, true);
            float4 ka, kb;
            drop_mask4_words(odd ? pa : r.x, odd ? pb : r.y, e.thr, e.scale, ka.x, ka.y, ka.z, ka.w);
            drop_mask4_words(odd ? r.z : pa, odd ? r.w : pb, e.thr, e.scale, kb.x, kb.y, kb.z, kb.w);
            quad(it, true, ka);
            quad(it + 1, true, kb);
          }
        }
      } else {
#pragma unroll
        for (int it = 0; it < NITQ_; ++it) quad(it, false, make_float4(1.f, 1.f, 1.f, 1.f));
      }
    }
    asm volatile("s_waitcnt lgkmcnt(0)" ::: "memory");
  });
  if constexpr (PROF) {
    asm volatile("s_waitcnt vmcnt(0)" ::: "memory");
    const long long t_end = __builtin_readcyclecounter();
    if (tid == 0 && e.aux) {
      unsigned long long* c = (unsigned long long*)e.aux;
      atomicAdd(c + 0, (unsigned long long)t_wait);
      atomicAdd(c + 1, (unsigned long long)t_issue);
      atomicAdd(c + 2, (unsigned long long)t_mma);
      atomicAdd(c + 3, (unsigned long long)(t_end - t_loop_end));
      atomicAdd(c + 4, (unsigned long long)(t_end - t_begin));
      atomicAdd(c + 5, 1ull);
      atomicAdd(c + 6, (unsigned long long)(wall_clock64() - w_begin));
    }
  }
}

template <typename HT, int EPI, int BM, int BN, int WM, int WN, int BKT, int NST, int GM, int ABL = 0>
__global__ __launch_bounds__(WM* WN * 64) void gemm_nt_h16_kernel(
    const HT* __restrict__ A, int lda, const HT* __restrict__ B, int ldb, int M, int N,
    int K, int ksteps_per_split, EpiDev e) {
  const int tiles = ((M + BM - 1) / BM) * ((N + BN - 1) / BN);
  gemm_nt_h16_body<HT, EPI, BM, BN, WM, WN, BKT, NST, GM, ABL>(A, lda, B, ldb, M, N, K, ksteps_per_split, e,
                                                           xcd_remap(blockIdx.x, tiles), (int)blockIdx.z);
}

constexpr int GG_MAX = 6;
struct GemmGroupDev {
  const void* A[GG_MAX]; const void* B[GG_MAX];
  int lda[GG_MAX], ldb[GG_MAX], M[GG_MAX], N[GG_MAX], K[GG_MAX], tile0[GG_MAX + 1];
  EpiDev e[GG_MAX];
  int n;
};
template <typename HT, int EPI, int BM, int BN, int WM, int WN, int BKT, int NST>
__global__ __launch_bounds__(WM* WN * 64) void gemm_nt_group_kernel(const GemmGroupDev g) {
  const int t = blockIdx.x;
  int i = 0;
#pragma unroll
  for (int k = 1; k < GG_MAX; ++k)
    if (k < g.n && t >= g.tile0[k]) i = k;
  gemm_nt_h16_body<HT, EPI, BM, BN, WM, WN, BKT, NST, 1, 0>((const HT*)g.A[i], g.lda[i], (const HT*)g.B[i], g.ldb[i], g.M[i], g.N[i], g.K[i],
                                                        g.K[i] / BK, g.e[i], t - g.tile0[i], 0);
}
// ... 274 lines not shown
        case 11: launch_h16<bf16_t, EPI, 128, 128, 2, 2, 64, 2, 4>(A, lda, B, ldb, M, N, K, e, splitk, s); break;
        case 12: launch_h16<bf16_t, EPI, 128, 128, 2, 2, 64, 2, 16>(A, lda, B, ldb, M, N, K, e, splitk, s); break;
        case 13: launch_h16<bf16_t, EPI, 128, 128, 2, 2, 64, 2, 39>(A, lda, B, ldb, M, N, K, e, splitk, s); break;
        case 10: launch_h16<bf16_t, EPI, 128, 128, 2, 2, 32, 3, 8>(A, lda, B, ldb, M, N, K, e, splitk, s); break;
        case 14: launch_h16<bf16_t, EPI, 160, 128, 1, 4, 64, 2, 1>(A, lda, B, ldb, M, N, K, e, splitk, s); break;
        case 19: launch_h16<bf16_t, EPI, 192, 128, 2, 2, 64, 2, 1>(A, lda, B, ldb, M, N, K, e, splitk, s); break;
        case 22: launch_h16<bf16_t, EPI, 320, 128, 2, 4, 64, 2, 1>(A, lda, B, ldb, M, N, K, e, splitk, s); break;
        case 24: launch_h16<bf16_t, EPI, 160, 128, 1, 4, 64, 3, 1>(A, lda, B, ldb, M, N, K, e, splitk, s); break;
        case 25: launch_h16<bf16_t, EPI, 192, 128, 1, 4, 64, 2, 1>(A, lda, B, ldb, M, N, K, e, splitk, s); break;
        default: launch_h16<bf16_t, EPI, 128, 128, 2, 2, 64, 2, 1>(A, lda, B, ldb, M, N, K, e, splitk, s); break;
      }
    } else
#endif
    {
      (void)variant;
      const long long t128 = (long long)((M + 127) / 128) * ((N + 127) / 128) * splitk;
      DISPATCH_H16(precision,
        if (t128 <= 256 && M > 64) {
          const int nst = small_nst((long long)((M + 63) / 64) * ((N + 127) / 128) * splitk);
          if (nst >= 4 && tim_knobs().gemm_small_w8 != 0) launch_h16<HT, EPI, 64, 128, 2, 4, 64, 4, 1>(A, lda, B, ldb, M, N, K, e, splitk, s);
          else if (nst >= 4) launch_h16<HT, EPI, 64, 128, 1, 4, 64, 4, 1>(A, lda, B, ldb, M, N, K, e, splitk, s);
          else if (nst == 3) launch_h16<HT, EPI, 64, 128, 1, 4, 64, 3, 1>(A, lda, B, ldb, M, N, K, e, splitk, s);
          else launch_h16<HT, EPI, 64, 128, 1, 4, 64, 2, 1>(A, lda, B, ldb, M, N, K, e, splitk, s);
        } else if (tall_tile_wins(M, N, splitk))
          launch_h16<HT, EPI, 160, 128, 1, 4, 64, 2, 1>(A, lda, B, ldb, M, N, K, e, splitk, s);
        else
          launch_h16<HT, EPI, 128, 128, 2, 2, 64, 2, 1>(A, lda, B, ldb, M, N, K, e, splitk, s));
    }
  }
  if (hipGetLastError() != hipSuccess) return TIMHIP_ELAUNCH;
  return TIMHIP_OK;
}

}

static int prepare_gemm(int precision, int epi, const void* A, int lda, const void* B, int ldb, int M, int N, int K,
                        const TimEpi& te, int splitk, EpiDev& e) {
  if (!A || !B || !te.out0) return TIMHIP_EINVAL;
  if (M <= 0 || N <= 0 || K <= 0) return TIMHIP_EINVAL;
  if (!valid_precision(precision)) return TIMHIP_EUNSUPPORTED;
  const int Kp = round_up(K, 64);
  if (te.a_wrap_k < 0 || te.a_wrap_k % 64 || (te.a_wrap_k > 0 && (Kp != 2 * te.a_wrap_k || !h16_storage(precision) || splitk > 1)))
    return TIMHIP_EUNSUPPORTED;
  if (lda % 64 || ldb % 64 || lda < (te.a_wrap_k > 0 ? te.a_wrap_k : Kp) || ldb < Kp) return TIMHIP_EALIGN;
  if (((uintptr_t)A | (uintptr_t)B) & 15) return TIMHIP_EALIGN;
  if ((size_t)M * lda * 2 >= (1ull << 32) || (size_t)N * ldb * 2 >= (1ull << 32)) return TIMHIP_EUNSUPPORTED;
  if (splitk > 1 && epi != TIMHIP_EPI_ATOMIC_F32 && epi != TIMHIP_EPI_STORE_F32) return TIMHIP_EINVAL;
  e.out0 = te.out0; e.out1 = te.out1; e.bias = te.bias; e.res = te.res; e.aux = te.aux;
  e.ld0 = te.ld0; e.ld1 = te.ld1; e.ldres = te.ldres; e.ldaux = te.ldaux;
  e.thr = te.p_drop > 0.f ? drop_threshold(te.p_drop) : 0u;
  e.scale = te.p_drop > 0.f ? 1.f / (1.f - te.p_drop) : 1.f;
  e.site = te.site; e.seed = te.seed;
  e.mask = (const uint8_t*)te.mask; e.ldmask = te.ldmask;
  e.ln_stats = te.ln_stats; e.ln_w = te.ln_w; e.ln_b = te.ln_b;
  e.acc_scale = te.acc_scale;
  e.a_wrap = te.a_wrap_k / 64;
  e.pair = tim_knobs().epi_pair;
  if (e.ln_stats && (epi != TIMHIP_EPI_DROP_RES_F32 || !e.res || !e.ln_w || !e.ln_b)) return TIMHIP_EINVAL;
  if (epi == TIMHIP_EPI_RELU_SPLIT3_T && (!h16_storage(precision) || e.out1 || e.ld1 % 64 || e.ld1 < N || e.ld0 < 3 * e.ld1 || splitk > 1))
    return TIMHIP_EINVAL;
  e.slab_stride = splitk > 1 ? (long long)M * te.ld0 : 0;

  bool vec = (e.ld0 % 4 == 0) && (((uintptr_t)e.out0 & 15) == 0);
  if (e.out1) vec = vec && (e.ld1 % 4 == 0) && (((uintptr_t)e.out1 & 15) == 0);
  if (e.res) vec = vec && (e.ldres % 4 == 0) && (((uintptr_t)e.res & 15) == 0);
  if (e.aux) vec = vec && (e.ldaux % 4 == 0) && (((uintptr_t)e.aux & 15) == 0);
  if (e.bias) vec = vec && (((uintptr_t)e.bias & 15) == 0);
  e.vec = vec ? 1 : 0;
  bool vec8 = vec && h16_storage(precision) && (e.ld0 % 8 == 0);
  if (e.out1) vec8 = vec8 && (e.ld1 % 8 == 0);
  if (e.aux) vec8 = vec8 && (e.ldaux % 8 == 0);
  e.vec8 = vec8 ? 1 : 0;
  if (e.thr != 0u && (N % 4) != 0) return TIMHIP_EUNSUPPORTED;
  return TIMHIP_OK;
}

int tim_gemm_nt_group(int precision, int epi, const TimGemmItem* items, int n, hipStream_t s) {
  if (!h16_storage(precision)) return TIMHIP_EUNSUPPORTED;
  if (!items || n < 1 || n > GG_MAX) return TIMHIP_EINVAL;
  if (epi != TIMHIP_EPI_STORE_F32 && epi != TIMHIP_EPI_ADD_F32 && epi != TIMHIP_EPI_STORE_T && epi != TIMHIP_EPI_RELU_T)
    return TIMHIP_EUNSUPPORTED;
  GemmGroupDev g;
  g.n = n;
  g.tile0[0] = 0;
  double flops = 0.0;
  for (int i = 0; i < GG_MAX; ++i) {
    if (i >= n) {
      g.A[i] = g.B[i] = nullptr; g.lda[i] = g.ldb[i] = g.M[i] = g.N[i] = g.K[i] = 0; g.tile0[i + 1] = g.tile0[i];
      g.e[i] = g.e[0];
      continue;
    }
    const TimGemmItem& t = items[i];
    const int rc = prepare_gemm(precision, epi, t.A, t.lda, t.B, t.ldb, t.M, t.N, t.K, t.e, 1, g.e[i]);
    if (rc) return rc;
    g.A[i] = t.A; g.B[i] = t.B; g.lda[i] = t.lda; g.ldb[i] = t.ldb;
    g.M[i] = t.M; g.N[i] = t.N; g.K[i] = round_up(t.K, 64);
    g.tile0[i + 1] = g.tile0[i] + ((t.M + 63) / 64) * ((t.N + 127) / 128);
    flops += 2.0 * t.M * t.N * t.K / (t.reserved > 1 ? t.reserved : 1);
  }
  TimGemmScope timing(flops, s);
  if (g.tile0[n] <= 512 && epi == TIMHIP_EPI_ADD_F32) {
    for (int i = 0; i < n; ++i) g.tile0[i + 1] = g.tile0[i] + ((items[i].M + 63) / 64) * ((items[i].N + 63) / 64);
    for (int i = n; i < GG_MAX; ++i) g.tile0[i + 1] = g.tile0[n];
    DISPATCH_H16(precision, hipLaunchKernelGGL((gemm_nt_group_kernel<HT, TIMHIP_EPI_ADD_F32, 64, 64, 2, 2, 64, 2>),
                                               dim3((unsigned)g.tile0[n]), dim3(256), (size_t)2 * (64 + 64) * 64 * 2, s, g));
    return hipGetLastError() == hipSuccess ? TIMHIP_OK : TIMHIP_ELAUNCH;
// ... 68 lines not shown
```

### tim_amd/csrc/gemm_epi.h

```cpp
#pragma once
#include <utility>
#include "common.h"

namespace {


struct EpiDev {
  void* out0; void* out1;
  const float* bias; const float* res; const void* aux;
  int ld0, ld1, ldres, ldaux;
  uint32_t thr; float scale; uint32_t site; TimSeed seed;
  const uint8_t* mask; int ldmask;
  const float* ln_stats; const float* ln_w; const float* ln_b;
  const float* acc_scale;
  int vec;
  int vec8;
  long long slab_stride;
  int pair;
  int a_wrap;
};

#ifndef TIMHIP_NT_MASK
#define TIMHIP_NT_MASK 3
#endif
template <typename T>
__device__ __forceinline__ void nt_store4(T* p, float a, float b, float c, float d) {
  if constexpr ((sizeof(T) == 4 && !(TIMHIP_NT_MASK & 4)) || (sizeof(T) == 2 && !(TIMHIP_NT_MASK & 1))) {
    store4<T>(p, a, b, c, d);
  } else if constexpr (sizeof(T) == 4) {
    typedef float f4_t __attribute__((ext_vector_type(4)));
    f4_t v = {a, b, c, d};
    __builtin_nontemporal_store(v, reinterpret_cast<f4_t*>(p));
  } else {
    vec4<T> v;
    v[0] = (T)a; v[1] = (T)b; v[2] = (T)c; v[3] = (T)d;
    __builtin_nontemporal_store(v, reinterpret_cast<vec4<T>*>(p));
  }
}

template <int EPI, typename T>
__device__ __forceinline__ void epi_one(const EpiDev& e, int m, int n, int N, float v, float mask) {
  size_t i0 = (size_t)m * e.ld0 + n;
  if (e.bias && EPI != TIMHIP_EPI_ADD_F32 && EPI != TIMHIP_EPI_DGELU_T && EPI != TIMHIP_EPI_DRELU_T &&
      EPI != TIMHIP_EPI_ATOMIC_F32 && EPI != TIMHIP_EPI_DRELU_F32IN_T && EPI != TIMHIP_EPI_MULAUX_T)
    v += e.bias[n];
  if (EPI == TIMHIP_EPI_STORE_T) {
    ((T*)e.out0)[i0] = OpT<T>::from_f(v);
  } else if (EPI == TIMHIP_EPI_RELU_T) {
    ((T*)e.out0)[i0] = OpT<T>::from_f(fmaxf(v, 0.f));
  } else if (EPI == TIMHIP_EPI_STORE_F32) {
    ((float*)e.out0)[i0] = v;
  } else if (EPI == TIMHIP_EPI_GELU_DROP_T2) {
    ((T*)e.out1)[(size_t)m * e.ld1 + n] = OpT<T>::from_f(v);
    ((T*)e.out0)[i0] = OpT<T>::from_f(gelu_f(v) * mask);
  } else if (EPI == TIMHIP_EPI_GELU_DROP_G2) {
    float gl, dg;
    gelu_both_f(v, gl, dg);
    ((T*)e.out1)[(size_t)m * e.ld1 + n] = OpT<T>::from_f(dg * mask);
    ((T*)e.out0)[i0] = OpT<T>::from_f(gl * mask);
  } else if (EPI == TIMHIP_EPI_GELU_T) {
    float gl, dg;
    gelu_both_f(v, gl, dg);
    ((T*)e.out0)[i0] = OpT<T>::from_f(gl);
  } else if (EPI == TIMHIP_EPI_MULAUX_T) {
    ((T*)e.out0)[i0] = OpT<T>::from_f(v * OpT<T>::to_f(((const T*)e.aux)[(size_t)m * e.ldaux + n]));
  } else if (EPI == TIMHIP_EPI_DROP_RES_F32) {
    float r = e.res[(size_t)m * e.ldres + n];
    if (e.ln_stats) r = (r - e.ln_stats[2 * m]) * e.ln_stats[2 * m + 1] * e.ln_w[n] + e.ln_b[n];
    ((float*)e.out0)[i0] = r + v * mask;
  } else if (EPI == TIMHIP_EPI_ADD_F32) {
    ((float*)e.out0)[i0] = v + (e.res ? e.res[(size_t)m * e.ldres + n] : 0.f);
  } else if (EPI == TIMHIP_EPI_DGELU_T) {
    float u = OpT<T>::to_f(((const T*)e.aux)[(size_t)m * e.ldaux + n]);
    ((T*)e.out0)[i0] = OpT<T>::from_f(v * mask * gelu_grad_f(u));
  } else if (EPI == TIMHIP_EPI_DRELU_T) {
    float h = OpT<T>::to_f(((const T*)e.aux)[(size_t)m * e.ldaux + n]);
    ((T*)e.out0)[i0] = OpT<T>::from_f(h > 0.f ? v : 0.f);
  } else if (EPI == TIMHIP_EPI_DRELU_F32IN_T) {
    float h = ((const float*)e.aux)[(size_t)m * e.ldaux + n];
    ((T*)e.out0)[i0] = OpT<T>::from_f(h > 0.f ? v : 0.f);
  } else if (EPI == TIMHIP_EPI_ATOMIC_F32) {
    atomicAdd(((float*)e.out0) + i0, v);
  } else if (EPI == TIMHIP_EPI_SIGMOID_F32) {
    ((float*)e.out0)[i0] = 1.f / (1.f + __expf(-v));
  } else if (EPI == TIMHIP_EPI_RELU_SPLIT3_T) {
    const float r = fmaxf(v, 0.f);
    const T hi = OpT<T>::from_f(r);
    ((T*)e.out0)[i0] = hi;
    ((T*)e.out0)[i0 + e.ld1] = OpT<T>::from_f(r - OpT<T>::to_f(hi));
    ((T*)e.out0)[i0 + 2 * (size_t)e.ld1] = hi;
  }
}

constexpr bool epi_uses_dropout(int EPI) {
  return EPI == TIMHIP_EPI_GELU_DROP_T2 || EPI == TIMHIP_EPI_DROP_RES_F32 || EPI == TIMHIP_EPI_DGELU_T ||
         EPI == TIMHIP_EPI_GELU_DROP_G2;
}

template <int EPI, typename T>
__device__ __forceinline__ void epi_quad(const EpiDev& e, int m, int n, int N, float v0, float v1,
                                         float v2, float v3, bool has_pre = false,
                                         float4 pre = make_float4(0.f, 0.f, 0.f, 0.f), bool has_b = false,
                                         float4 pb = make_float4(0.f, 0.f, 0.f, 0.f), bool has_ln = false,
                                         float2 pst = make_float2(0.f, 1.f),
                                         float4 pg = make_float4(1.f, 1.f, 1.f, 1.f),
                                         float4 pbe = make_float4(0.f, 0.f, 0.f, 0.f), bool has_k = false,
                                         float4 kpre = make_float4(1.f, 1.f, 1.f, 1.f)) {
  float k0 = 1.f, k1 = 1.f, k2 = 1.f, k3 = 1.f;
  if (epi_uses_dropout(EPI) && e.thr != 0u) {
    if (has_k) {
      k0 = kpre.x; k1 = kpre.y; k2 = kpre.z; k3 = kpre.w;
    } else if (e.mask)
      drop_mask4_bits((uint32_t)e.mask[(size_t)m * e.ldmask + (n >> 3)] >> (n & 4), e.scale, k0, k1, k2, k3);
    else
      drop_mask4(e.seed, e.site, ((uint64_t)m * (uint64_t)N + (uint64_t)n) >> 2, e.thr, e.scale, k0, k1, k2, k3);
  }
  if (e.vec && n + 3 < N) {
    size_t i0 = (size_t)m * e.ld0 + n;
    if (EPI != TIMHIP_EPI_ADD_F32 && EPI != TIMHIP_EPI_DGELU_T && EPI != TIMHIP_EPI_DRELU_T &&
        EPI != TIMHIP_EPI_ATOMIC_F32 && EPI != TIMHIP_EPI_DRELU_F32IN_T && EPI != TIMHIP_EPI_MULAUX_T && e.bias) {
      float4 b = pb;
      if (!has_b) b = *reinterpret_cast<const float4*>(e.bias + n);
      v0 += b.x; v1 += b.y; v2 += b.z; v3 += b.w;
    }
    if (EPI == TIMHIP_EPI_STORE_T) {
      nt_store4<T>((T*)e.out0 + i0, v0, v1, v2, v3);
    } else if (EPI == TIMHIP_EPI_RELU_T) {
      nt_store4<T>((T*)e.out0 + i0, fmaxf(v0, 0.f), fmaxf(v1, 0.f), fmaxf(v2, 0.f), fmaxf(v3, 0.f));
    } else if (EPI == TIMHIP_EPI_STORE_F32) {
      nt_store4<float>((float*)e.out0 + i0, v0, v1, v2, v3);
    } else if (EPI == TIMHIP_EPI_GELU_DROP_T2) {
      nt_store4<T>((T*)e.out1 + (size_t)m * e.ld1 + n, v0, v1, v2, v3);
      nt_store4<T>((T*)e.out0 + i0, gelu_f(v0) * k0, gelu_f(v1) * k1, gelu_f(v2) * k2, gelu_f(v3) * k3);
    } else if (EPI == TIMHIP_EPI_GELU_DROP_G2) {
      float g0, g1, g2, g3, d0, d1, d2, d3;
      gelu_both_f(v0, g0, d0); gelu_both_f(v1, g1, d1); gelu_both_f(v2, g2, d2); gelu_both_f(v3, g3, d3);
      nt_store4<T>((T*)e.out1 + (size_t)m * e.ld1 + n, d0 * k0, d1 * k1, d2 * k2, d3 * k3);
      nt_store4<T>((T*)e.out0 + i0, g0 * k0, g1 * k1, g2 * k2, g3 * k3);
    } else if (EPI == TIMHIP_EPI_GELU_T) {
      float g0, g1, g2, g3, d0, d1, d2, d3;
      gelu_both_f(v0, g0, d0); gelu_both_f(v1, g1, d1); gelu_both_f(v2, g2, d2); gelu_both_f(v3, g3, d3);
      nt_store4<T>((T*)e.out0 + i0, g0, g1, g2, g3);
    } else if (EPI == TIMHIP_EPI_MULAUX_T) {
      float u0, u1, u2, u3;
      load4<T>((const T*)e.aux + (size_t)m * e.ldaux + n, u0, u1, u2, u3);
      nt_store4<T>((T*)e.out0 + i0, v0 * u0, v1 * u1, v2 * u2, v3 * u3);
    } else if (EPI == TIMHIP_EPI_DROP_RES_F32) {
      float4 r = pre;
      if (!has_pre) r = *reinterpret_cast<const float4*>(e.res + (size_t)m * e.ldres + n);
      if (e.ln_stats) {
        float2 st = pst;
        float4 g = pg, be = pbe;
        if (!has_ln) {
          st = *reinterpret_cast<const float2*>(e.ln_stats + 2 * (size_t)m);
          g = *reinterpret_cast<const float4*>(e.ln_w + n);
          be = *reinterpret_cast<const float4*>(e.ln_b + n);
        }
        r.x = (r.x - st.x) * st.y * g.x + be.x; r.y = (r.y - st.x) * st.y * g.y + be.y;
        r.z = (r.z - st.x) * st.y * g.z + be.z; r.w = (r.w - st.x) * st.y * g.w + be.w;
      }
      nt_store4<float>((float*)e.out0 + i0, r.x + v0 * k0, r.y + v1 * k1, r.z + v2 * k2, r.w + v3 * k3);
    } else if (EPI == TIMHIP_EPI_ADD_F32) {
      float4 r = make_float4(0.f, 0.f, 0.f, 0.f);
      if (has_pre) r = pre;
      else if (e.res) r = *reinterpret_cast<const float4*>(e.res + (size_t)m * e.ldres + n);
      nt_store4<float>((float*)e.out0 + i0, r.x + v0, r.y + v1, r.z + v2, r.w + v3);
    } else if (EPI == TIMHIP_EPI_DGELU_T) {
// ... 133 lines not shown
```

### tim_amd/csrc/gemm_pp.hip

```cpp
#include <stdlib.h>
#include <mutex>

#include "gemm_epi.h"

namespace {

constexpr int PP_BN = 256, PP_ROWB = 128, PP_NST = 3, PP_TNW = 4;

__device__ __forceinline__ void pp_barrier() {
  __builtin_amdgcn_sched_barrier(0);
  __builtin_amdgcn_s_barrier();
  __builtin_amdgcn_sched_barrier(0);
}
__device__ __forceinline__ void pp_wait_lds() { asm volatile("s_waitcnt lgkmcnt(0)" ::: "memory"); }

struct PpNoSync { __device__ __forceinline__ void operator()() const {} };
template <typename HT, int EPI, int TMW, int PFD = TMW, typename AFTER = PpNoSync, int PFA = TMW>
__device__ __forceinline__ void pp_epilogue(const EpiDev& e, const f32x4_t (&acc)[PP_TNW][TMW], int mw0, int nw0, int M, int N,
                                            float* ep, int lane, AFTER after = AFTER{}) {
  constexpr int EP_COLS = 64, EP_LD = EP_COLS + 4, CPR = EP_COLS / 4, OPR = EP_COLS / 8, RBS = 16;
  constexpr int NITQ = RBS * CPR / 64, NITO = RBS * OPR / 64;
  const float asc = e.acc_scale ? *e.acc_scale : 1.f;
  const int frow = lane & 15, fq = lane >> 4;

// ... 72 lines not shown
      lnb = *reinterpret_cast<const float4*>(e.ln_b + n4);
      pre_gb = true;
    }
  }

  static_for<TMW>([&](auto jc) {
    constexpr int j = decltype(jc)::value;
#pragma unroll
    for (int i = 0; i < PP_TNW; ++i)
      *reinterpret_cast<float4*>(ep + frow * EP_LD + i * 16 + 4 * fq) =
          make_float4(acc[i][j][0] * asc, acc[i][j][1] * asc, acc[i][j][2] * asc, acc[i][j][3] * asc);
    pp_wait_lds();
    if (epi_has_oct(EPI) && e.vec8) {
#pragma unroll
      for (int it = 0; it < NITO; ++it) {
        const int idx = it * 64 + lane;
        const int row = idx / OPR, ch = idx % OPR;
        const float4 lo = *reinterpret_cast<const float4*>(ep + row * EP_LD + ch * 8);
        const float4 hi = *reinterpret_cast<const float4*>(ep + row * EP_LD + ch * 8 + 4);
        const int m = mw0 + j * RBS + row, n = nw0 + ch * 8;
        if (m < M && n + 7 < N) {
          epi_oct<EPI, HT>(e, m, n, N, lo, hi, mbyte[j][it], pre_aux, abuf[j % PFA][PRE_AUX ? it : 0], pre_b8, bias8[0], bias8[1]);
        } else if (m < M) {
          if (n < N) epi_quad<EPI, HT>(e, m, n, N, lo.x, lo.y, lo.z, lo.w);
          if (n + 4 < N) epi_quad<EPI, HT>(e, m, n + 4, N, hi.x, hi.y, hi.z, hi.w);
        }
      }
    } else {
      bool has_k = false;
      if constexpr (EPI == TIMHIP_EPI_DROP_RES_F32 && (NITQ % 2) == 0) has_k = e.thr != 0u && !e.mask && e.vec && (N & 7) == 0 && e.pair;
      auto quad = [&](int it, bool hk, float4 kf) {
        const int idx = it * 64 + lane;
        const int row = idx / CPR, ch = idx % CPR;
        const float4 v = *reinterpret_cast<const float4*>(ep + row * EP_LD + ch * 4);
        const int m = mw0 + j * RBS + row, n = nw0 + ch * 4;
        if (m < M && n < N)
          epi_quad<EPI, HT>(e, m, n, N, v.x, v.y, v.z, v.w, pre_res && n + 3 < N, rbuf[j % PFD][PRE_RES ? it : 0], pre_b4 && n + 3 < N,
                            bias4, pre_ln && pre_gb && n + 3 < N, sbuf[j % PFD][PRE_RES ? it : 0], lng, lnb, hk, kf);
      };
      if (has_k) {
        if constexpr ((NITQ % 2) == 0) {
#pragma unroll
          for (int it = 0; it < NITQ; it += 2) {
            const int idx = (it + (lane & 1)) * 64 + (lane & ~1);
            const long long m_ = mw0 + j * RBS + idx / CPR, n_ = nw0 + (idx % CPR) * 4;
            const Philox4 r = philox4x32_7(e.seed, e.site, (uint64_t)(m_ * (long long)N + n_) >> 3);
            const bool odd = (lane & 1) != 0;
            const uint32_t sa = odd ? r.x : r.z, sb = odd ? r.y : r.w;
            const uint32_t pa = (uint32_t)__builtin_amdgcn_mov_dpp((int)sa, 0xB1, 0xF, 0xF, true);
            const uint32_t pb = (uint32_t)__builtin_amdgcn_mov_dpp((int)sb, 0xB1, 0xF, 0xF, true);
            float4 ka, kb;
            drop_mask4_words(odd ? pa : r.x, odd ? pb : r.y, e.thr, e.scale, ka.x, ka.y, ka.z, ka.w);
            drop_mask4_words(odd ? r.z : pa, odd ? r.w : pb, e.thr, e.scale, kb.x, kb.y, kb.z, kb.w);
            quad(it, true, ka);
            quad(it + 1, true, kb);
          }
        }
      } else {
#pragma unroll
        for (int it = 0; it < NITQ; ++it) quad(it, false, make_float4(1.f, 1.f, 1.f, 1.f));
      }
    }
    if constexpr (j + PFD < TMW) fetch_res(std::integral_constant<int, j + PFD>{});
    if constexpr (j + PFA < TMW) fetch_aux(std::integral_constant<int, j + PFA>{});
    pp_wait_lds();
    after();
  });
}

template <int TMW, int G> struct PpShare {
  static constexpr int CNT = G == 0 ? 7 : 6, P0 = G == 0 ? 4 : 3;
  static_assert(4 * 7 + 4 * 6 == 2 * TMW * 2 + 32, "the share table is written for the 160 x 256 tile");
};

template <typename HT, int TMW, int G, bool PROF = false, int ABL = 0, bool LATE_ = false>
__device__ __forceinline__ void pp_mainloop(const HT* __restrict__ A, const HT* __restrict__ B, int nk, const char* lds, uint32_t lds0,
                                            const uint32_t (&off)[7], int first_piece, int a_frag, int b_frag, int c0, int c1,
                                            f32x4_t (&acc)[PP_TNW][TMW], long long* prof = nullptr, bool primed = false,
                                            int a_wrap = 0x7fffffff) {
  constexpr int BM = 32 * TMW, A_PIECES = BM / 8;
  constexpr int A_BYTES = BM * PP_ROWB, B_BYTES = PP_BN * PP_ROWB, ST_BYTES = A_BYTES + B_BYTES;
  constexpr int CNT = PpShare<TMW, G>::CNT;
  constexpr bool LATE = LATE_ && G == 0;

  auto piece = [&](int kt, int slot, int i) {
    const int p = first_piece + i;
    if constexpr (ABL == 4) {
      const char* g = p < A_PIECES ? reinterpret_cast<const char*>(A) + (size_t)kt * A_BYTES : reinterpret_cast<const char*>(B) + (size_t)kt * B_BYTES;
      glds16_s(uniform_ptr(g), off[i], lds0 + slot * ST_BYTES + p * 1024);
      return;
    }
    const char* g = p < A_PIECES ? reinterpret_cast<const char*>(A) + (size_t)(kt >= a_wrap ? kt - a_wrap : kt) * PP_ROWB
                                 : reinterpret_cast<const char*>(B) + (size_t)kt * PP_ROWB;
    glds16_s(uniform_ptr(g), off[i], lds0 + slot * ST_BYTES + p * 1024);
  };

  if (primed) {
    glds_wait<0>();
  } else {
#pragma unroll
    for (int i = 0; i < CNT; ++i) piece(0, 0, i);
    if (nk > 1) {
#pragma unroll
      for (int i = 0; i < CNT; ++i) piece(1, 1, i);
      glds_wait<CNT>();
    } else {
// ... 1280 lines not shown
```

### tim_amd/csrc/rowops.hip

```cpp
#include <stdlib.h>

#include "common.h"

namespace {

template <typename T>
__global__ void cast_weight_kernel(const float* __restrict__ src, int rows, int cols, T* __restrict__ dst,
                                   int ld) {
  const int r = blockIdx.y;
  for (int c = blockIdx.x * blockDim.x + threadIdx.x; c < ld; c += gridDim.x * blockDim.x)
    dst[(size_t)r * ld + c] = OpT<T>::from_f(c < cols ? src[(size_t)r * cols + c] : 0.f);
}

constexpr int TP_ROWS = 256;
template <typename TS, typename TD>
__global__ __launch_bounds__(256) void transpose_kernel(const TS* __restrict__ src, int rows, int cols, int lds_,
                                                        TD* __restrict__ dst, int ld, float* __restrict__ colsum) {
  __shared__ float tile[32][33];
  __shared__ float part[8][32];
  const int c0 = blockIdx.x * 32, rp0 = blockIdx.y * TP_ROWS;
  const int tx = threadIdx.x & 31, ty = threadIdx.x >> 5;
  float acc = 0.f;
  for (int r0 = rp0; r0 < rp0 + TP_ROWS && r0 < ld; r0 += 32) {
    for (int i = ty; i < 32; i += 8) {
// ... 329 lines not shown
  }
  float s = 0.f;
#pragma unroll
  for (int i = 0; i < NS; ++i)
#pragma unroll
    for (int h = 0; h < 2; ++h) {
      float4 t = v[i][h];
      t.x = act_f(act, t.x); t.y = act_f(act, t.y); t.z = act_f(act, t.z); t.w = act_f(act, t.w);
      v[i][h] = t;
      s += (t.x + t.y) + (t.z + t.w);
    }
  const float mean = wave_sum(s) / (float)cols;
  float q = 0.f;
#pragma unroll
  for (int i = 0; i < NS; ++i)
#pragma unroll
    for (int h = 0; h < 2; ++h) {
      const float a0 = v[i][h].x - mean, a1 = v[i][h].y - mean, a2 = v[i][h].z - mean, a3 = v[i][h].w - mean;
      q += (a0 * a0 + a1 * a1) + (a2 * a2 + a3 * a3);
    }
  const float var = wave_sum(q) / (float)cols;
  const float rstd = rsqrtf(var + 1e-5f);
  if (lane == 0 && stats) *reinterpret_cast<float2*>(stats + 2 * row) = make_float2(mean, rstd);
#pragma unroll
  for (int i = 0; i < NS; ++i) {
    float o[8];
#pragma unroll
    for (int h = 0; h < 2; ++h) {
      const float4 t = v[i][h], g = gw[i][h], be = gb[i][h];
      o[4 * h] = (t.x - mean) * rstd * g.x + be.x; o[4 * h + 1] = (t.y - mean) * rstd * g.y + be.y;
      o[4 * h + 2] = (t.z - mean) * rstd * g.z + be.z; o[4 * h + 3] = (t.w - mean) * rstd * g.w + be.w;
    }
    const int c = i * 512 + lane * 8;
    if (xf) {
      store4<float>(xf + (size_t)row * ldx + c, o[0], o[1], o[2], o[3]);
      store4<float>(xf + (size_t)row * ldx + c + 4, o[4], o[5], o[6], o[7]);
    }
    if (xt) {
      if constexpr (sizeof(T) == 2) {
        typedef T v8_t __attribute__((ext_vector_type(8)));
        v8_t pk;
#pragma unroll
        for (int u = 0; u < 8; ++u) pk[u] = OpT<T>::from_f(o[u]);
        *reinterpret_cast<v8_t*>(xt + (size_t)row * ldt + c) = pk;
      } else {
        store4<T>(xt + (size_t)row * ldt + c, o[0], o[1], o[2], o[3]);
        store4<T>(xt + (size_t)row * ldt + c + 4, o[4], o[5], o[6], o[7]);
      }
    }
  }
  }
}

template <typename T, int LN_MAXV, bool ACT0 = false, int S16 = 0>
__global__ __launch_bounds__(256) void ln_bwd_kernel(const float* __restrict__ dx, int lddx,
                                                     const float* __restrict__ y, int ldy,
                                                     const float* __restrict__ stats, int rows, int cols, int act,
                                                     const float* __restrict__ w, float* __restrict__ dyf, int lddy,
                                                     T* __restrict__ dyt, int ldt, uint32_t thr, float scale,
                                                     TimSeed seed, uint32_t site, float* __restrict__ dgamma,
                                                     float* __restrict__ dbeta, int rows_pb,
                                                     float* __restrict__ partial, const float* __restrict__ t_scale,
                                                     const T* __restrict__ addt, int ldadd, const float* __restrict__ add_scale,
                                                     LnSplit sp, int pair_sw) {
  extern __shared__ float red[];
  if (blockIdx.x * rows_pb >= sp.row) { w = sp.w2; dgamma = sp.dg2; dbeta = sp.db2; }
  const float ts = t_scale ? *t_scale : 1.f;
  const float as = ((addt || (S16 & 1) != 0) && add_scale) ? *add_scale : 1.f;
  const int lane = threadIdx.x & 63, wave = threadIdx.x >> 6;
  const int nv = (cols + 255) >> 8;
  float4 ag[LN_MAXV], ab[LN_MAXV];
#pragma unroll
  for (int i = 0; i < LN_MAXV; ++i) { ag[i] = make_float4(0, 0, 0, 0); ab[i] = make_float4(0, 0, 0, 0); }
  const int r0 = blockIdx.x * rows_pb, r1 = min(rows, r0 + rows_pb);
  float4 ww[LN_MAXV];
#pragma unroll
  for (int i = 0; i < LN_MAXV; ++i) {
    const int c = (i * 64 + lane) * 4;
    ww[i] = (i < nv && c < cols) ? *reinterpret_cast<const float4*>(w + c) : make_float4(0, 0, 0, 0);
  }
  constexpr bool IN16 = (S16 & 1) != 0, OUT16 = (S16 & 2) != 0;
  float4 tn[LN_MAXV], dn[LN_MAXV];
  typedef T t4_t __attribute__((ext_vector_type(4)));
  t4_t an[LN_MAXV], dn16[LN_MAXV];
  float2 stn = make_float2(0.f, 0.f);
  auto fetch = [&](int row) {
    stn = *reinterpret_cast<const float2*>(stats + 2 * row);
#pragma unroll
    for (int i = 0; i < LN_MAXV; ++i) {
      const int c = (i * 64 + lane) * 4;
      if (i < nv && c < cols) {
        {
          typedef float f4_t __attribute__((ext_vector_type(4)));
          const f4_t q0_ = __builtin_nontemporal_load(reinterpret_cast<const f4_t*>(y + (size_t)row * ldy + c));
          tn[i] = make_float4(q0_[0], q0_[1], q0_[2], q0_[3]);
        }
        if constexpr (IN16) dn16[i] = *reinterpret_cast<const t4_t*>(reinterpret_cast<const T*>(dx) + (size_t)row * lddx + c);
        else dn[i] = *reinterpret_cast<const float4*>(dx + (size_t)row * lddx + c);
        if (addt) an[i] = *reinterpret_cast<const t4_t*>(addt + (size_t)row * ldadd + c);
      }
    }
  };
  if (r0 + wave < r1) fetch(r0 + wave);
  float kq[4] = {1.f, 1.f, 1.f, 1.f};
  const bool pair_ok = (cols % 512) == 0 && nv <= LN_MAXV && pair_sw;
#pragma unroll 1
  for (int row = r0 + wave; row < r1; row += 4) {
    const float mean = stn.x, rstd = stn.y;
    float4 xh[LN_MAXV], d[LN_MAXV], ga[LN_MAXV];
#pragma unroll
    for (int i = 0; i < LN_MAXV; ++i) {
      xh[i] = tn[i];
      if constexpr (IN16) {
        d[i] = make_float4(OpT<T>::to_f(dn16[i][0]) * as, OpT<T>::to_f(dn16[i][1]) * as, OpT<T>::to_f(dn16[i][2]) * as,
                           OpT<T>::to_f(dn16[i][3]) * as);
      } else {
        d[i] = dn[i];
      }
      if (addt) {
        d[i].x = fmaf(OpT<T>::to_f(an[i][0]), as, d[i].x); d[i].y = fmaf(OpT<T>::to_f(an[i][1]), as, d[i].y);
        d[i].z = fmaf(OpT<T>::to_f(an[i][2]), as, d[i].z); d[i].w = fmaf(OpT<T>::to_f(an[i][3]), as, d[i].w);
      }
    }
    if (row + 4 < r1) fetch(row + 4);
    float s1 = 0.f, s2 = 0.f;
#pragma unroll
    for (int i = 0; i < LN_MAXV; ++i) {
      const int c = (i * 64 + lane) * 4;
      if (i < nv && c < cols) {
        const float4 t = xh[i];
        if (!ACT0 && act != 0) ga[i] = make_float4(act_grad_f(act, t.x), act_grad_f(act, t.y), act_grad_f(act, t.z),
                                          act_grad_f(act, t.w));
        float4 h;
        if (ACT0) {
          h.x = (t.x - mean) * rstd; h.y = (t.y - mean) * rstd; h.z = (t.z - mean) * rstd; h.w = (t.w - mean) * rstd;
        } else {
          h.x = (act_f(act, t.x) - mean) * rstd; h.y = (act_f(act, t.y) - mean) * rstd;
          h.z = (act_f(act, t.z) - mean) * rstd; h.w = (act_f(act, t.w) - mean) * rstd;
        }
        xh[i] = h;
        ag[i].x += d[i].x * h.x; ag[i].y += d[i].y * h.y; ag[i].z += d[i].z * h.z; ag[i].w += d[i].w * h.w;
        ab[i].x += d[i].x; ab[i].y += d[i].y; ab[i].z += d[i].z; ab[i].w += d[i].w;
        d[i].x *= ww[i].x; d[i].y *= ww[i].y; d[i].z *= ww[i].z; d[i].w *= ww[i].w;
        s1 += (d[i].x + d[i].y) + (d[i].z + d[i].w);
        s2 += (d[i].x * h.x + d[i].y * h.y) + (d[i].z * h.z + d[i].w * h.w);
      }
    }
    s1 = wave_sum(s1) / (float)cols;
    s2 = wave_sum(s2) / (float)cols;
    const bool paired = LN_MAXV >= 2 && pair_ok && thr != 0u && dyt != nullptr;
#pragma unroll
    for (int i = 0; i < LN_MAXV; ++i) {
      const int c = (i * 64 + lane) * 4;
      float kp[4] = {ts, ts, ts, ts};
      if constexpr (LN_MAXV >= 2) {
        if (paired && (i & 1) == 0) {
          const int isel = i + (lane & 1);
          const Philox4 r = philox4x32_7(seed, site, ((uint64_t)row * cols + (uint64_t)((isel * 64 + (lane & ~1)) * 4)) >> 3);
          const bool odd = (lane & 1) != 0;
          const uint32_t sa = odd ? r.x : r.z, sb = odd ? r.y : r.w;
          const uint32_t pa = (uint32_t)__builtin_amdgcn_mov_dpp((int)sa, 0xB1, 0xF, 0xF, true);
          const uint32_t pb = (uint32_t)__builtin_amdgcn_mov_dpp((int)sb, 0xB1, 0xF, 0xF, true);
          drop_mask4_words(odd ? pa : r.x, odd ? pb : r.y, thr, scale, kp[0], kp[1], kp[2], kp[3]);
          drop_mask4_words(odd ? r.z : pa, odd ? r.w : pb, thr, scale, kq[0], kq[1], kq[2], kq[3]);
#pragma unroll
          for (int u = 0; u < 4; ++u) { kp[u] *= ts; kq[u] *= ts; }
        } else if (paired) {
#pragma unroll
          for (int u = 0; u < 4; ++u) kp[u] = kq[u];
        }
      }
      if (i < nv && c < cols) {
        float o0 = rstd * (d[i].x - s1 - xh[i].x * s2), o1 = rstd * (d[i].y - s1 - xh[i].y * s2);
        float o2 = rstd * (d[i].z - s1 - xh[i].z * s2), o3 = rstd * (d[i].w - s1 - xh[i].w * s2);
        if (!ACT0 && act != 0) { o0 *= ga[i].x; o1 *= ga[i].y; o2 *= ga[i].z; o3 *= ga[i].w; }
        if constexpr (OUT16) {
          if (dyf) store4<T>(reinterpret_cast<T*>(dyf) + (size_t)row * lddy + c, o0 * ts, o1 * ts, o2 * ts, o3 * ts);
        } else {
          if (dyf) store4<float>(dyf + (size_t)row * lddy + c, o0, o1, o2, o3);
        }
        if (dyt) {
          float k0 = kp[0], k1 = kp[1], k2 = kp[2], k3 = kp[3];
          if (thr != 0u && !paired) {
            drop_mask4(seed, site, ((uint64_t)row * cols + c) >> 2, thr, scale, k0, k1, k2, k3);
            k0 *= ts; k1 *= ts; k2 *= ts; k3 *= ts;
          }
          store4<T>(dyt + (size_t)row * ldt + c, o0 * k0, o1 * k1, o2 * k2, o3 * k3);
        }
      }
    }
  }
  float* rg = red + (size_t)wave * 2 * cols;
  float* rb = rg + cols;
#pragma unroll
  for (int i = 0; i < LN_MAXV; ++i) {
    const int c = (i * 64 + lane) * 4;
    if (i < nv && c < cols) {
      *reinterpret_cast<float4*>(rg + c) = ag[i];
      *reinterpret_cast<float4*>(rb + c) = ab[i];
    }
  }
  __syncthreads();
  for (int c = threadIdx.x; c < cols; c += 256) {
    float sg = 0.f, sb = 0.f;
#pragma unroll
    for (int k = 0; k < 4; ++k) { sg += red[(size_t)k * 2 * cols + c]; sb += red[(size_t)k * 2 * cols + cols + c]; }
    if (partial) {
      partial[(size_t)blockIdx.x * 2 * cols + c] = sg;
      partial[(size_t)blockIdx.x * 2 * cols + cols + c] = sb;
    } else {
      if (dgamma) atomicAdd(dgamma + c, sg);
      if (dbeta) atomicAdd(dbeta + c, sb);
    }
  }
}

template <typename T>
__global__ __launch_bounds__(256) void time_l1_fwd_kernel(const float* __restrict__ times, int rows, int d,
                                                          const float* __restrict__ w, const float* __restrict__ b,
                                                          T* __restrict__ h, int ld, int rows_pb, int split) {
  const int rs = split ? 3 * ld : ld;
  const int r0 = blockIdx.x * rows_pb, r1 = min(rows, r0 + rows_pb);
  if ((ld & 3) == 0) {
    const int nq = ld >> 2, rl_n = max(1, 256 / nq);
    const int q = threadIdx.x % nq, rl = threadIdx.x / nq;
    if (threadIdx.x >= nq * rl_n && nq <= 256) return;
    for (int q0 = q; q0 < nq; q0 += 256) {
      float w0[4], w1[4], bb[4];
#pragma unroll
      for (int u = 0; u < 4; ++u) {
        const int j = 4 * q0 + u;
        w0[u] = j < d ? w[2 * j] : 0.f; w1[u] = j < d ? w[2 * j + 1] : 0.f; bb[u] = j < d ? b[j] : 0.f;
      }
      for (int r = r0 + (nq <= 256 ? rl : 0); r < r1; r += (nq <= 256 ? rl_n : 1)) {
        const float t0 = times[2 * r], t1 = times[2 * r + 1];
        float v[4];
// ... 522 lines not shown
  if (mask_out && mask_p > 0.f) {
    if (mask_cols % 32 || ((uintptr_t)mask_out & 3)) return TIMHIP_EUNSUPPORTED;
    mbits = (uint32_t*)mask_out; mwords = mask_cols / 32; mthr = drop_threshold(mask_p);
  }
#define LN_FWD(NV) hipLaunchKernelGGL((ln_fwd_kernel<T, NV>), grid, dim3(256), 0, s, y, rows, cols, ldy, act, w, b, \
                                   xf, ldx, (T*)xt, ldt, stats, mbits, mwords, mthr, TimSeed(mask_seed), mask_site, sp)
  const int nv = (cols + 255) / 256;
  const bool al8 = (ldy % 4) == 0 && (!xt || ldt % 8 == 0) && (!xf || ldx % 4 == 0) &&
                   ((((uintptr_t)y | (uintptr_t)xt | (uintptr_t)xf | (uintptr_t)w | (uintptr_t)b) & 15) == 0);
  const int frpb = tim_knobs().ln_fwd_rpb >= 4 ? tim_knobs().ln_fwd_rpb / 4 * 4 : 4;
  const dim3 grid8 = run_if ? dim3(min((int)grid.x, 256)) : dim3((rows + frpb - 1) / frpb);
#define LN_FWD8(NS) hipLaunchKernelGGL((ln_fwd8_kernel<T, NS>), grid8, dim3(256), 0, s, y, rows, ldy, act, w, b, xf, ldx, (T*)xt, ldt, \
                                     stats, mbits, mwords, mthr, TimSeed(mask_seed), mask_site, run_if, sp)
  if (run_if && !(al8 && (cols == 512 || cols == 1024 || cols == 2048))) return TIMHIP_EUNSUPPORTED;
  if (al8 && (cols == 512 || cols == 1024 || cols == 2048)) {
    DISPATCH_T(precision, if (cols == 512) LN_FWD8(1); else if (cols == 1024) LN_FWD8(2); else LN_FWD8(4));
  } else {
    DISPATCH_T(precision, if (nv <= 1) LN_FWD(1); else if (nv <= 2) LN_FWD(2); else if (nv <= 4) LN_FWD(4); else LN_FWD(8));
  }
#undef LN_FWD8
#undef LN_FWD
  TIM_CHECK_LAUNCH();
  return TIMHIP_OK;
}

struct DropArgs { uint32_t thr; float scale; };
static DropArgs drop_args(float p) { return p > 0.f ? DropArgs{drop_threshold(p), 1.f / (1.f - p)} : DropArgs{0u, 1.f}; }

static int ln_bwd_rows_per_block(int rows) {
  if (tim_knobs().ln_rpb >= 4) return tim_knobs().ln_rpb / 4 * 4;
  int rpb = 16;
  if (rows > 16 * 768) rpb = (((rows + 767) / 768) + 3) / 4 * 4;
  else if (rows < 16 * 512) { rpb = (((rows + 511) / 512) + 3) / 4 * 4; if (rpb < 4) rpb = 4; }
  else {
    double best = 0.0;
    for (int c = 16; c <= 24; c += 4) {
      const int blocks = (rows + c - 1) / c, rounds = (blocks + 255) / 256;
      const double fill = (double)blocks / (rounds * 256.0);
      if (fill > best + 0.02) { best = fill; rpb = c; }
    }
  }
  return rpb;
}

size_t tim_layernorm_bwd_ws(int rows, int cols) {
  const int rpb = ln_bwd_rows_per_block(rows);
  return (size_t)((rows + rpb - 1) / rpb) * 2 * cols * sizeof(float);
}

int tim_layernorm_bwd(int precision, const float* dx, int lddx, const float* y, int ldy, const float* stats,
                      int rows, int cols, int act, const float* w, float* dyf, int lddy, void* dyt, int ldt,
                      float p_drop, uint64_t seed, uint32_t site, float* dgamma, float* dbeta, float* partial_ws,
                      hipStream_t s, bool defer_colsum, const float* t_scale, const void* addt, int ldadd,
                      const float* add_scale, int stream16, int split_row, const float* w2, float* dgamma2, float* dbeta2) {
  if (!dx || !y || !stats || !w || rows <= 0) return TIMHIP_EINVAL;
  TimGemmScope timing((double)rows * cols * (8 + (addt ? 2 : 0) + (dyf ? 4 : 0) + (dyt ? (f32_storage(precision) ? 4 : 2) : 0)), s, 2);
  LnSplit sp{0x7fffffff, nullptr, nullptr, nullptr, nullptr};
  if (stream16 && (act != 0 || !h16_storage(precision) || !add_scale || !t_scale)) return TIMHIP_EUNSUPPORTED;
  if (cols % 4 || cols > 256 * LN_MAXV_MAX || ldy % 4 || lddx % 4 || (dyf && lddy % 4) || (dyt && ldt % 4) || (addt && ldadd % 4))
    return TIMHIP_EUNSUPPORTED;
  int rpb = ln_bwd_rows_per_block(rows);
  if (!partial_ws && tim_knobs().ln_rpb_small >= 4) rpb = tim_knobs().ln_rpb_small / 4 * 4;
  if (split_row > 0 && split_row < rows) {
    if (!w2 || partial_ws) return TIMHIP_EINVAL;
    if (split_row % rpb) {
      rpb = 0;
      for (int c = 16; c >= 4 && !rpb; c -= 4) if (split_row % c == 0) rpb = c;
      if (!rpb) return TIMHIP_EINVAL;
    }
    sp.row = split_row; sp.w2 = w2; sp.dg2 = dgamma2; sp.db2 = dbeta2;
  }
  dim3 grid((rows + rpb - 1) / rpb);
  const size_t shmem = (size_t)4 * 2 * cols * sizeof(float);
  const DropArgs dr = drop_args(p_drop);
  const int pair_sw = tim_knobs().ln_pair;
  const int nv = (cols + 255) / 256;
#define LN_BWD(T_, NV, ACT0, S16) hipLaunchKernelGGL((ln_bwd_kernel<T_, NV, ACT0, S16>), grid, dim3(256), shmem, s, dx, lddx, y, ldy, stats, \
                                   rows, cols, act, w, dyf, lddy, (T_*)dyt, ldt, dr.thr, dr.scale, seed, site, dgamma, dbeta, rpb, partial_ws, \
                                   t_scale, (const T_*)addt, ldadd, add_scale, sp, pair_sw)
#define LN_BWD_NV(T_, ACT0, S16) do { if (nv <= 1) LN_BWD(T_, 1, ACT0, S16); else if (nv <= 2) LN_BWD(T_, 2, ACT0, S16); \
                                      else if (nv <= 4) LN_BWD(T_, 4, ACT0, S16); else LN_BWD(T_, 8, ACT0, S16); } while (0)
  if (stream16) {
    DISPATCH_H16(precision, { if (stream16 == 1) LN_BWD_NV(HT, true, 1); else if (stream16 == 2) LN_BWD_NV(HT, true, 2); else LN_BWD_NV(HT, true, 3); });
  } else if (act == 0 && nv == 4) {
    DISPATCH_T(precision, LN_BWD(T, 4, true, 0));
  } else {
    DISPATCH_T(precision, LN_BWD_NV(T, false, 0));
  }
#undef LN_BWD_NV
#undef LN_BWD
  TIM_CHECK_LAUNCH();
  if (partial_ws && (dgamma || dbeta) && !defer_colsum) {
    hipLaunchKernelGGL(partial_colsum_kernel, dim3((2 * cols + 255) / 256, 32), dim3(256), 0, s, partial_ws,
                       (int)grid.x, cols, dgamma, dbeta);
    TIM_CHECK_LAUNCH();
  }
  return TIMHIP_OK;
}

int tim_layernorm_bwd_blocks(int rows) {
  const int rpb = ln_bwd_rows_per_block(rows);
  return (rows + rpb - 1) / rpb;
}

extern "C" {

int timhip_cast_weight(int precision, const float* src, int rows, int cols, void* dst, int ld, int transpose,
                       void* stream) {
  hipStream_t s = (hipStream_t)stream;
  if (!src || !dst || rows <= 0 || cols <= 0 || ld % 64) return TIMHIP_EINVAL;
  if (!transpose) {
    if (ld < cols) return TIMHIP_EINVAL;
    dim3 grid((ld + 255) / 256, rows);
    DISPATCH_T(precision, hipLaunchKernelGGL(cast_weight_kernel<T>, grid, dim3(256), 0, s, src, rows, cols, (T*)dst, ld));
  } else {
    if (ld < rows) return TIMHIP_EINVAL;
    dim3 grid((cols + 31) / 32, (ld + TP_ROWS - 1) / TP_ROWS);
    DISPATCH_T(precision, hipLaunchKernelGGL((transpose_kernel<float, T>), grid, dim3(256), 0, s, src, rows, cols,
                                             cols, (T*)dst, ld, (float*)nullptr));
  }
  TIM_CHECK_LAUNCH();
  return TIMHIP_OK;
}

int timhip_cast_weight_both(int precision, const float* src, int rows, int cols, void* plain, int ldp, void* tr, int ldt,
                            void* stream) {
  if (!src || !plain || !tr || rows <= 0 || cols <= 0 || ldp % 64 || ldt % 64 || ldp < cols || ldt < rows)
    return TIMHIP_EINVAL;
  dim3 grid((max(ldp, cols) + 31) / 32, (max(ldt, rows) + 31) / 32);
  DISPATCH_T(precision, hipLaunchKernelGGL(cast_weight_both_kernel<T>, grid, dim3(256), 0, (hipStream_t)stream, src,
                                           rows, cols, (T*)plain, ldp, (T*)tr, ldt));
  TIM_CHECK_LAUNCH();
  return TIMHIP_OK;
}

int timhip_cast_weights(int precision, const TimCastItem* items, int n, void* stream) {
  if (!items || n < 0) return TIMHIP_EINVAL;
  for (int i0 = 0; i0 < n; i0 += CAST_MAX) {
    CastBatch cb;
    cb.n = n - i0 < CAST_MAX ? n - i0 : CAST_MAX;
    int blocks = 0;
    for (int i = 0; i < cb.n; ++i) {
      const TimCastItem& it = items[i0 + i];
// ... 26 lines not shown
  if (rows <= 0) return TIMHIP_EINVAL;
  CastRows cr = {};
  int maxq = 0;
  for (int i = 0; i < count; ++i) {
    if (!src[i] || !dst[i] || cols[i] <= 0 || ld[i] < cols[i] || ld[i] % 4) return TIMHIP_EINVAL;
    cr.src[i] = src[i]; cr.dst[i] = dst[i]; cr.cols[i] = cols[i]; cr.lds[i] = lds_[i]; cr.ld[i] = ld[i]; cr.site[i] = sites[i];
    maxq = ld[i] / 4 > maxq ? ld[i] / 4 : maxq;
  }
  const DropArgs dr = drop_args(p_drop);
  dim3 grid((maxq + 255) / 256, rows, count);
  DISPATCH_T(precision, hipLaunchKernelGGL(cast_rows_kernel<T>, grid, dim3(256), 0, (hipStream_t)stream, cr, rows, dr.thr,
                                           dr.scale, TimSeed(seed), vscale));
  TIM_CHECK_LAUNCH();
  return TIMHIP_OK;
}

int timhip_cast_rows(int precision, const float* src, int rows, int cols, int lds_, void* dst, int ld, float p_drop,
                     uint64_t seed, uint32_t site, const float* vscale, void* stream) {
  return cast_rows_launch(precision, 1, &src, &cols, &lds_, &dst, &ld, rows, p_drop, seed, &site, vscale, stream);
}

int timhip_dropout_rows_bwd(const float* g, int rows, int cols, int ldg, float* dx, int ldx, float p_drop,
                            uint64_t seed, uint32_t site, void* stream) {
  if (!g || !dx || rows <= 0 || cols <= 0) return TIMHIP_EINVAL;
  const DropArgs dr = drop_args(p_drop);
  dim3 grid(((cols + 3) / 4 + 255) / 256, rows);
  hipLaunchKernelGGL(drop_bwd_rows_kernel, grid, dim3(256), 0, (hipStream_t)stream, g, rows, cols, ldg, dx, ldx, dr.thr,
                     dr.scale, seed, site);
  TIM_CHECK_LAUNCH();
  return TIMHIP_OK;
}

int timhip_dropout_mask(uint64_t seed, uint32_t site, float p, int rows, int cols, uint8_t* out, void* stream) {
  if (!out || rows <= 0 || cols <= 0) return TIMHIP_EINVAL;
  hipLaunchKernelGGL(dropout_mask_kernel, dim3(1024), dim3(256), 0, (hipStream_t)stream, seed, site,
                     drop_threshold(p), rows, cols, out);
  TIM_CHECK_LAUNCH();
  return TIMHIP_OK;
}

int timhip_layernorm_fwd(int precision, const float* y, int rows, int cols, int ldy, int act, const float* w,
                         const float* b, float* x_f32, int ldx, void* x_T, int ldt, float* stats, void* stream) {
  return tim_layernorm_fwd(precision, y, rows, cols, ldy, act, w, b, x_f32, ldx, x_T, ldt, stats, (hipStream_t)stream);
}

int timhip_layernorm_bwd(int precision, const float* dx, int lddx, const float* y, int ldy, const float* stats,
                         int rows, int cols, int act, const float* w, float* dy_f32, int lddy, void* dy_T, int ldt,
                         float p_drop, uint64_t seed, uint32_t site, float* dgamma, float* dbeta, const float* t_scale,
                         void* stream) {
  return tim_layernorm_bwd(precision, dx, lddx, y, ldy, stats, rows, cols, act, w, dy_f32, lddy, dy_T, ldt, p_drop,
                           seed, site, dgamma, dbeta, nullptr, (hipStream_t)stream, false, t_scale);
}

int timhip_layernorm_fwd2(int precision, const float* y, int rows, int cols, int ldy, int act, const float* w, const float* b,
                          int split_row, const float* w2, const float* b2, float* x_f32, int ldx, void* x_T, int ldt, float* stats,
                          void* stream) {
  return tim_layernorm_fwd(precision, y, rows, cols, ldy, act, w, b, x_f32, ldx, x_T, ldt, stats, (hipStream_t)stream, nullptr, 0, 0.f,
                           0, 0, nullptr, split_row, w2, b2);
}

int timhip_layernorm_bwd2(int precision, const float* dx, int lddx, const float* y, int ldy, const float* stats, int rows, int cols,
                          int act, const float* w, int split_row, const float* w2, float* dy_f32, int lddy, void* dy_T, int ldt,
                          float* dgamma, float* dbeta, float* dgamma2, float* dbeta2, const float* t_scale, void* stream) {
  return tim_layernorm_bwd(precision, dx, lddx, y, ldy, stats, rows, cols, act, w, dy_f32, lddy, dy_T, ldt, 0.f, 0, 0, dgamma, dbeta,
                           nullptr, (hipStream_t)stream, false, t_scale, nullptr, 0, nullptr, 0, split_row, w2, dgamma2, dbeta2);
}

int timhip_cast_rows_pair(int precision, const float* const* src, const int* cols, void* const* dst, const int* ld, int rows,
                          float p_drop, uint64_t seed, const uint32_t* sites, void* stream) {
  if (!src || !cols || !dst || !ld || !sites) return TIMHIP_EINVAL;
  return cast_rows_launch(precision, 2, src, cols, cols, dst, ld, rows, p_drop, seed, sites, nullptr, stream);
}

int timhip_time_l1_fwd(int precision, const float* times, int rows, int d, const float* w, const float* b, void* h,
                       int ld, void* stream) {
  if (!times || !w || !b || !h || rows <= 0 || ld < d) return TIMHIP_EINVAL;
  const int rpb = rows >= 4096 ? 16 : (rows >= 512 ? 4 : 1);
  dim3 grid((rows + rpb - 1) / rpb);
  DISPATCH_T(precision, hipLaunchKernelGGL(time_l1_fwd_kernel<T>, grid, dim3(256), 0, (hipStream_t)stream, times,
                                           rows, d, w, b, (T*)h, ld, rpb, 0));
  TIM_CHECK_LAUNCH();
  return TIMHIP_OK;
}

int timhip_time_l1_fwd_split3(int precision, const float* times, int rows, int d, const float* w, const float* b, void* h3,
                              int ld, void* stream) {
  if (!times || !w || !b || !h3 || rows <= 0 || ld < d || (ld % 64) || !h16_storage(precision)) return TIMHIP_EINVAL;
  const int rpb = rows >= 4096 ? 16 : (rows >= 512 ? 4 : 1);
  dim3 grid((rows + rpb - 1) / rpb);
  DISPATCH_H16(precision, hipLaunchKernelGGL(time_l1_fwd_kernel<HT>, grid, dim3(256), 0, (hipStream_t)stream, times,
                                             rows, d, w, b, (HT*)h3, ld, rpb, 1));
  TIM_CHECK_LAUNCH();
  return TIMHIP_OK;
}

int timhip_time_l1_bwd(int precision, const float* times, int rows, int d, const float* w, const void* dh, int ld,
                       float* dw, float* db, float* dt, const float* out_scale, void* stream) {
  if (!times || !w || !dh || !dw || !db || rows <= 0) return TIMHIP_EINVAL;
  const int rpb = rows >= 2048 ? 128 : 32;
  dim3 grid((rows + rpb - 1) / rpb);
  DISPATCH_T(precision, hipLaunchKernelGGL(time_l1_bwd_kernel<T>, grid, dim3(256), 0, (hipStream_t)stream, times,
                                           rows, d, w, (const T*)dh, ld, dw, db, dt, rpb, out_scale));
  TIM_CHECK_LAUNCH();
  return TIMHIP_OK;
}

// ... 259 lines not shown
```

### tim_amd/functional.py

```python
import ctypes as C
import os
import weakref
from collections import namedtuple

import torch

from . import _lib as L
from ._lib import call, ptr


def _ru(x, m=64):
    return (x + m - 1) // m * m


def _stream():
    return torch.cuda.current_stream().cuda_stream


_SALT = {"word": None, "epoch": 0}
_SALT_STEP = 0x51B54A32D192ED03


def graph_safe_dropout(dev, enable=True):
    if not enable:
# ... 243 lines not shown

    def weight_split(self, p, mode=1):
        return self.copies.get(p, mode)[0]

    def split3(self, items, mode, relu=False):
        items = [it for it in items if it[1] > 0]
        for i0 in range(0, len(items), 6):
            grp = items[i0:i0 + 6]
            call("timhip_split3_many", self.prec, len(grp), _parr([g[0] for g in grp]), _iarr([g[1] for g in grp]),
                 _iarr([g[2] for g in grp]), _iarr([g[3] for g in grp]), _parr([g[4] for g in grp]),
                 _iarr([g[4].shape[1] for g in grp]), mode, 1 if relu else 0, _stream())

    def invalidate_weights(self):
        self.copies.invalidate()

    def next_seed(self):
        self.step += 1
        self.last_seed = self._next_seed()
        return self.last_seed

    def _next_seed(self):
        if _SALT["word"] is not None:
            _SALT["word"].add_(_SALT_STEP)
            _SALT["epoch"] += 1
            return (self.seed * 0x9E3779B97F4A7C15) & 0xFFFFFFFFFFFFFFFF
        return (self.seed * 0x9E3779B97F4A7C15 + self.step * 0xD1B54A32D192ED03) & 0xFFFFFFFFFFFFFFFF

    def grad_scale(self, cotangents, dev, out=None):
        if self.prec != L.PREC_F16:
            return None
        dev = torch.device(dev)
        gs = out if out is not None else torch.zeros(8, dtype=torch.float32, device=dev)
        self.nonfinite.add(gs, dev.type == "cuda" and torch.cuda.is_current_stream_capturing())
        cots = [c for c in cotangents if c is not None and c.numel() > 0]
        if not cots:
            gs[:2] = 1.0
            return gs
        for i0 in range(0, len(cots), 8):
            grp = cots[i0:i0 + 8]
            call("timhip_grad_scale", _parr(grp), (C.c_longlong * len(grp))(*[c.numel() for c in grp]), len(grp),
                 float(self.grad_scale_target), ptr(gs), _stream())
        return gs

    def adopt_captured(self, since=0):
        return self.nonfinite.adopt(since)

    def forget_captured(self):
        self.nonfinite.forget()

    def grads_finite(self, reset=True):
        return self.nonfinite.read(reset)

    def gemm(self, epi, A, B, M, N, K, out0, ld0, out1=None, ld1=0, bias=None, res=None, ldres=0, aux=None,
             ldaux=0, p_drop=0.0, seed=0, site=0, splitk=1, mask=None, ldmask=0, ln=None, acc_scale=None, rep=0, a_wrap_k=0):
        if M == 0 or N == 0:
            return
        st_, g_, b_ = ln if ln is not None else (None, None, None)
        e = L.TimEpi(ptr(out0), ptr(out1), ptr(bias), ptr(res), ptr(aux), ld0, ld1, ldres, ldaux,
                     float(p_drop), site, seed, ptr(mask), ldmask, rep, ptr(st_), ptr(g_), ptr(b_), acc_scale, a_wrap_k, 0)
        call("timhip_gemm_nt", self.prec, epi, ptr(A), A.stride(0), ptr(B), B.stride(0), M, N, K,
             C.byref(e), splitk, _stream())

    def wgrad(self, dY, Nout, X, Kout, M, dW, db, out_scale=None):
        if M == 0:
            return
        nbytes = L.load().timhip_wgrad_workspace_bytes(self.prec, Nout, Kout, M)
        ws = torch.empty(nbytes, dtype=torch.uint8, device=dY.device)
        call("timhip_wgrad", self.prec, ptr(dY), dY.stride(0), Nout, ptr(X), X.stride(0), Kout, M, ptr(dW),
             ptr(db), ptr(ws), nbytes, out_scale, _stream())

    def gemm_many(self, epi, items, acc_scale=None):
        items = [it for it in items if it["M"] > 0 and it["N"] > 0]
        if not self.h16 or len(items) < 2:
            for it in items:
                self.gemm(epi, it["A"], it["B"], it["M"], it["N"], it["K"], it["out0"], it["ld0"], bias=it.get("bias"),
                          res=it.get("res"), ldres=it.get("ldres", 0), acc_scale=acc_scale, rep=it.get("rep", 0))
            return
        for i0 in range(0, len(items), 6):
            grp = items[i0:i0 + 6]
            arr = (L.TimGemmItem * len(grp))()
            for a, it in zip(arr, grp):
                a.A, a.B = ptr(it["A"]), ptr(it["B"])
                a.lda, a.ldb = it["A"].stride(0), it["B"].stride(0)
                a.M, a.N, a.K, a.reserved = it["M"], it["N"], it["K"], it.get("rep", 0)
                a.e = L.TimEpi(ptr(it["out0"]), None, ptr(it.get("bias")), ptr(it.get("res")), None, it["ld0"], 0,
                               it.get("ldres", 0), 0, 0.0, 0, 0, None, 0, 0, None, None, None, acc_scale)
            call("timhip_gemm_nt_group", self.prec, epi, C.cast(arr, C.c_void_p), len(grp), _stream())

    def wgrad_many(self, items, out_scale=None):
        if not self.h16:
            for dY, Nout, X, Kout, M, dW, db in items:
                self.wgrad(dY, Nout, X, Kout, M, dW, db, out_scale)
            return
        by_m = {}
        for it in items:
            dY, Nout, X, Kout, M, dW, db = it
            if M == 0:
                continue
            if (Nout * Kout) % 4:
                self.wgrad(dY, Nout, X, Kout, M, dW, db, out_scale)
            else:
                by_m.setdefault(M, []).append((dY, Nout, X, Kout, dW, db))
        for M, grp in by_m.items():
            for i in range(0, len(grp), 8):
                self.wgrad_group(grp[i:i + 8], M, accumulate=True, out_scale=out_scale)

    def wgrad_group(self, items, M, accumulate=True, out_scale=None):
        arr = (L.TimWgradItem * len(items))(*[L.TimWgradItem(ptr(dY), ptr(X), ptr(dW), ptr(db), dY.stride(0), X.stride(0),
                                                             Nout, Kout) for dY, Nout, X, Kout, dW, db in items])
        pa = C.cast(arr, C.c_void_p)
        nbytes = L.load().timhip_wgrad_group_workspace_bytes(self.prec, pa, len(items), M)
        ws = torch.empty(max(nbytes, 16), dtype=torch.uint8, device=items[0][0].device)
# ... 195 lines not shown
    prec = rt.prec if prec is None else prec
    for i0 in range(0, len(ranges), 6):
        grp = ranges[i0:i0 + 6]
        call("timhip_gather_ranges", prec, ptr(x), B, S, E, len(grp), _iarr([r[0] for r in grp]), _iarr([r[1] for r in grp]),
             _parr([r[2] for r in grp]), st)


def _scatter_head_rows(B, S, E, items, dx, st):
    groups = []
    for it in items:
        if not groups or len(groups[-1]) == 6 or any(it[1] < g[1] + g[2] and g[1] < it[1] + it[2] for g in groups[-1]):
            groups.append([])
        groups[-1].append(it)
    for grp in groups:
        call("timhip_scatter_ranges_add", B, S, E, len(grp), _iarr([g[1] for g in grp]), _iarr([g[2] for g in grp]),
             _parr([g[0] for g in grp]), ptr(dx), st)


class _Pass:
    __slots__ = ("model", "rt", "cfg", "plan", "names", "dev", "st", "B", "T", "d", "S", "F", "M", "E", "R", "p_feat", "p_seq",
                 "p_enc", "seed", "salt_epoch")

    def __init__(self, model, plan, dev, B, T, training, seed):
        cfg = model.cfg
        self.model, self.rt, self.cfg, self.plan, self.names = model, model.rt, cfg, plan, model._encoder_param_names
        self.dev, self.st, self.seed = dev, _stream(), seed
        self.B, self.T, self.d, self.E, self.S, self.F = B, T, cfg.d_model, cfg.E, plan.S, plan.F
        self.M, self.R = B * plan.S, B * cfg.num_feats
        self.p_feat, self.p_seq, self.p_enc = (cfg.feat_drop, cfg.seq_drop, cfg.enc_dropout) if training else (0.0, 0.0, 0.0)
        self.salt_epoch = _SALT["epoch"] if training else None


_Embedder = namedtuple("_Embedder", "name slot xT u stats Cin site")
_Embedded = namedtuple("_Embedded", "mods paired u_all stats_all")
_Stack = namedtuple("_Stack", "saved xs_t lparams keep_flag")
_Head = namedtuple("_Head", "slot pname s0 n rows")
_RegHead = namedtuple("_RegHead", "slot pname s0 n rows h1 h2 y")
_Back = namedtuple("_Back", "P G gs_in gs_out")

_FE = "feature_encoding."


def _keep_bits_fwd(q, Lyr):
    rt, cfg = q.rt, q.cfg
    desc = L.TimDesc(q.B, q.S, q.F, q.d, q.E, cfg.nhead, cfg.FF, rt.prec, q.p_enc, q.seed, 0, rt.layer_split_flags(q.E, cfg.FF), None)
    saved_bytes = L.load().timhip_layer_saved_bytes(C.byref(desc))
    layer_saved = [torch.empty(saved_bytes, dtype=torch.uint8, device=q.dev) for _ in range(Lyr)]
    if q.p_enc > 0.0 and rt.h16 and os.environ.get("TIM_AMD_ATTN_KEEP_BITS", "1") != "0":
        rc = L.load().timhip_attn_keep_bits(C.byref(desc), Lyr, _parr(layer_saved), q.st)
        if rc == 0:
            desc.reserved |= L.DESC_ATTN_KEEP_BITS
        elif rc != L.EUNSUPPORTED:
            L.check(rc, "timhip_attn_keep_bits")
    return desc, layer_saved


def _embedders_fwd(q, P, visual, audio):
    rt, dev, st, plan, R, d = q.rt, q.dev, q.st, q.plan, q.R, q.d
    B, nf = q.B, q.cfg.num_feats
    inputs = [visual if name == "visual" else audio for name, _ in plan.embedders]
    for (name, _), x in zip(plan.embedders, inputs):
        if x.dim() != 3 or x.shape[0] != B or x.shape[1] != nf:
            raise ValueError("%s input must be [B=%d, num_feats=%d, C], got %s" % (name, B, nf, tuple(x.shape)))
    ne = len(plan.embedders)
    paired = ne == 2 and R % 16 == 0
    u_all = torch.empty((ne * R, d), dtype=torch.float32, device=dev)
    e_all = torch.empty((ne * R, d), dtype=torch.float32, device=dev)
    stats_all = torch.empty((ne * R, 2), dtype=torch.float32, device=dev)
    x2s = [_f32c(x).reshape(R, x.shape[2]) for x in inputs]
    xTs = [torch.empty((R, _ru(x.shape[2])), dtype=rt.op_dtype, device=dev) for x in inputs]
    sites = [L.SITE_FEAT_V if name == "visual" else L.SITE_FEAT_A for name, _ in plan.embedders]
    if paired:
        call("timhip_cast_rows_pair", rt.prec, _parr(x2s), _iarr([t.shape[1] for t in x2s]), _parr(xTs),
             _iarr([t.shape[1] for t in xTs]), R, q.p_feat, q.seed, (C.c_uint32 * 2)(*sites), st)
    mods, gemms, e_bufs = [], [], [None, None]
    for i, (name, slot) in enumerate(plan.embedders):
        x2, xT, site = x2s[i], xTs[i], sites[i]
        Cin = x2.shape[1]
        if not paired:
            call("timhip_cast_rows", rt.prec, ptr(x2), R, Cin, Cin, ptr(xT), xT.shape[1], q.p_feat, q.seed, site, None, st)
        u = u_all[i * R:(i + 1) * R]
        gemms.append(dict(A=xT, B=rt.weight(P[_FE + name + "_embedder.1.weight"]), M=R, N=d, K=Cin, out0=u, ld0=d,
                          bias=_f32c(P[_FE + name + "_embedder.1.bias"])))
        mods.append(_Embedder(name, slot, xT, u, stats_all[i * R:(i + 1) * R], Cin, site))
        e_bufs[slot] = e_all[i * R:(i + 1) * R]
    rt.gemm_many(L.EPI_STORE_F32, gemms)
    lnp = [(_f32c(P[_FE + name + "_embedder.3.weight"]), _f32c(P[_FE + name + "_embedder.3.bias"])) for name, _ in plan.embedders]
    if paired:
        call("timhip_layernorm_fwd2", rt.prec, ptr(u_all), 2 * R, d, d, 2, ptr(lnp[0][0]), ptr(lnp[0][1]), R, ptr(lnp[1][0]),
             ptr(lnp[1][1]), ptr(e_all), d, None, 0, ptr(stats_all), st)
    else:
        for m, (w, b) in zip(mods, lnp):
            rt.ln_fwd(m.u, R, d, 2, w, b, xf=e_bufs[m.slot], ldx=d, stats=m.stats)
    return _Embedded(mods, paired, u_all, stats_all), e_bufs


def _assemble_fwd(q, P, e_bufs, te_c):
    rt, plan = q.rt, q.plan
    cls_v = [_f32c(P[_FE + n]).reshape(-1) for n in plan.cls_names]
    mod_v = [_f32c(P[_FE + n]).reshape(-1) for n in plan.mod_names]
    x_f = torch.empty((q.M, q.E), dtype=torch.float32, device=q.dev)
    x_t = torch.empty((q.M, q.E), dtype=rt.op_dtype, device=q.dev)
    call("timhip_assemble_fwd_p", rt.prec, ptr(plan.table(q.dev)), q.B, q.S, q.d, ptr(e_bufs[0]), ptr(e_bufs[1]), q.cfg.num_feats,
         _parr(cls_v), len(cls_v), ptr(te_c), q.T, _parr(mod_v), len(mod_v), q.p_seq, q.seed, L.SITE_SEQ, ptr(x_f), ptr(x_t), q.st)
    return x_f, x_t


def _layers_fwd(q, P, desc, layer_saved, x0_f, x0_t):
    rt, model, dev, st = q.rt, q.model, q.dev, q.st
    Lyr = len(layer_saved)
    xL_f = torch.empty((q.M, q.E), dtype=torch.float32, device=dev)
    xs_t = [x0_t] + [torch.empty((q.M, q.E), dtype=rt.op_dtype, device=dev) for _ in range(Lyr)]
    ws_bytes = L.load().timhip_layer_workspace_bytes(C.byref(desc))
    ws = model._workspace(ws_bytes, dev)
    lparams = []
    for l in range(Lyr):
        lp = model._layer_params(rt, P, "%s.layers.%d." % (model._stack_prefix, l))
        lparams.append(lp)
        desc.layer = l
        out_f = xL_f if l == Lyr - 1 else None
        if l == 0:
            call("timhip_layer_fwd", C.byref(desc), C.byref(lp[0]), ptr(x0_f), ptr(x0_t), ptr(out_f),
                 ptr(xs_t[1]), ptr(layer_saved[0]), ptr(ws), ws_bytes, st)
        else:
            call("timhip_layer_fwd_chained", C.byref(desc), C.byref(lp[0]), C.byref(lparams[l - 1][0]),
                 ptr(layer_saved[l - 1]), ptr(xs_t[l]), ptr(out_f), ptr(xs_t[l + 1]), ptr(layer_saved[l]), st)
    return _Stack(layer_saved, xs_t, lparams, desc.reserved & L.DESC_ATTN_KEEP_BITS), xL_f


def _heads_fwd(q, P, xL_f, xL_t, outs, row0=0):
    rt, dev, st, B, S, E = q.rt, q.dev, q.st, q.B, q.S - row0, q.E
    heads, gemms, ranges = [], [], []
    for slot, pname, s0, n in q.plan.heads:
        w = P["cls_head." + pname + ".weight"]
        Cn = w.shape[0]
        logits = torch.empty((B * n, Cn), dtype=torch.float32, device=dev)
        bias = _f32c(P["cls_head." + pname + ".bias"])
        if rt.split:
            rows = torch.empty((B * n, 3 * E), dtype=rt.op_dtype, device=dev)
            item = dict(A=rows, B=rt.weight_split(w), M=B * n, N=Cn, K=3 * E, out0=logits, ld0=Cn, bias=bias, rep=3) if n > 0 else None
            heads.append(_Head(slot, pname, s0, n, rows[:, :E] if n > 0 else None))
        else:
            rows = torch.empty((B * n, E), dtype=rt.op_dtype, device=dev)
            item = dict(A=rows, B=rt.weight(w), M=B * n, N=Cn, K=E, out0=logits, ld0=Cn, bias=bias) if n > 0 else None
            heads.append(_Head(slot, pname, s0, n, rows))
        if n > 0:
            ranges.append((s0 - row0, n, rows))
            gemms.append(item)
        outs[slot] = logits
    if rt.split:
        for i0 in range(0, len(ranges), 6):
            grp = ranges[i0:i0 + 6]
            call("timhip_gather_split3_ranges", rt.prec, ptr(xL_f), B, S, E, len(grp), _iarr([r[0] for r in grp]),
                 _iarr([r[1] for r in grp]), _parr([r[2] for r in grp]), st)
    else:
        _gather_head_rows(rt, xL_t, B, S, E, ranges, st)
    rt.gemm_many(L.EPI_STORE_F32, gemms)
    return heads


def _reg_heads_fwd(q, P, xL_t, outs, row0=0):
    rt, dev, B, E = q.rt, q.dev, q.B, q.E
    hid = E // 2
    regs = []
    for slot, pname, s0, n in q.plan.reg:
        pre = "reg_head." + pname + "."
        rows = torch.empty((B * n, E), dtype=rt.op_dtype, device=dev)
        h1 = rt.out_op(B * n, hid, dev)
        h2 = rt.out_op(B * n, hid, dev)
        y = torch.empty((B * n, 2), dtype=torch.float32, device=dev)
        if n > 0:
            _gather_head_rows(rt, xL_t, B, q.S - row0, E, [(s0 - row0, n, rows)], q.st)
            rt.gemm(L.EPI_RELU_T, rows, rt.weight(P[pre + "0.weight"]), B * n, hid, E, h1, h1.shape[1],
                    bias=_f32c(P[pre + "0.bias"]))
            rt.gemm(L.EPI_RELU_T, h1, rt.weight(P[pre + "2.weight"]), B * n, hid, hid, h2, h2.shape[1],
                    bias=_f32c(P[pre + "2.bias"]))
            rt.gemm(L.EPI_SIGMOID_F32, h2, rt.weight(P[pre + "4.weight"]), B * n, 2, hid, y, 2,
                    bias=_f32c(P[pre + "4.bias"]))
        outs[slot] = y
        regs.append(_RegHead(slot, pname, s0, n, rows, h1, h2, y))
# ... 360 lines not shown
```

Baseline: 332,700 interval-queries/s.

## Save residual dropout keep bits in forward and reuse them in LayerNorm backward

The forward residual-dropout GEMM epilogues now write a packed keep-bit mask per element into new saved-activation fields. The LayerNorm backward kernel then reads these bits instead of regenerating the Philox random stream, through a new BITS template path. This removes Philox recomputation from the backward LN pass. In exchange it adds byte stores in the forward epilogue and extra saved memory. It also disables fused-LN forward and the paired LN backward path whenever the bits are used, which may cost more than it saves.

```diff
diff --git a/include/timhip.h b/include/timhip.h
--- a/include/timhip.h
+++ b/include/timhip.h
@@ -66,6 +66,7 @@
 #define TIMHIP_DESC_STREAM16_IN 0x20000
 #define TIMHIP_DESC_STREAM16_OUT 0x40000
 #define TIMHIP_DESC_ATTN_KEEP_BITS 0x80000
+#define TIMHIP_DESC_RES_KEEP_BITS 0x100000
 
 typedef struct TimLayerParams {
   const void *in_w, *in_wt;
@@ -94,7 +95,8 @@
 size_t timhip_layer_saved_bytes(const TimDesc* d);
 size_t timhip_layer_workspace_bytes(const TimDesc* d);
 enum { TIMHIP_SAVED_QKV = 0, TIMHIP_SAVED_O = 1, TIMHIP_SAVED_Y1 = 2, TIMHIP_SAVED_X1T = 3, TIMHIP_SAVED_H = 4,
-       TIMHIP_SAVED_Y2 = 5, TIMHIP_SAVED_FFN_KEEP_BITS = 6, TIMHIP_SAVED_ATTN_KEEP_BITS = 7 };
+       TIMHIP_SAVED_Y2 = 5, TIMHIP_SAVED_FFN_KEEP_BITS = 6, TIMHIP_SAVED_ATTN_KEEP_BITS = 7, TIMHIP_SAVED_RES1_KEEP_BITS = 8,
+       TIMHIP_SAVED_RES2_KEEP_BITS = 9 };
 int timhip_layer_saved_field(const TimDesc* d, int field, size_t* offset, size_t* bytes);
 
 int timhip_cast_weight(int precision, const float* src, int rows, int cols, void* dst, int ld,
@@ -154,6 +156,7 @@
   const float* acc_scale;
   int32_t a_wrap_k;
   int32_t reserved2;
+  void* keep_out;
 } TimEpi;
 
 typedef struct TimGemmItem {
@@ -197,6 +200,11 @@
 int timhip_layernorm_bwd2(int precision, const float* dx, int lddx, const float* y, int ldy, const float* stats, int rows, int cols,
                           int act, const float* w, int split_row, const float* w2, float* dy_f32, int lddy, void* dy_T, int ldt,
                           float* dgamma, float* dbeta, float* dgamma2, float* dbeta2, const float* t_scale, void* stream);
+int timhip_layernorm_bwd3(int precision, const void* dx, int lddx, const float* y, int ldy, const float* stats, int rows, int cols,
+                          int act, const float* w, void* dy_res, int lddy, void* dy_T, int ldt, float p_drop, uint64_t seed,
+                          uint32_t site, float* dgamma, float* dbeta, const float* t_scale, const void* add_T, int ldadd,
+                          const float* add_scale, int stream16, const void* keep_bits, void* partial_ws, size_t partial_bytes,
+                          void* stream);
 
 int timhip_attention_fwd(const TimDesc* d, const void* qkv, void* o, float* lse, void* stream);
 int timhip_attention_fwd_rows(const TimDesc* d, const void* qkv, int s0, void* o_rows, void* stream);
diff --git a/tim_amd/_lib.py b/tim_amd/_lib.py
--- a/tim_amd/_lib.py
+++ b/tim_amd/_lib.py
@@ -22,6 +22,7 @@
 
 
 SAVED_QKV, SAVED_O, SAVED_Y1, SAVED_X1T, SAVED_H, SAVED_Y2, SAVED_FFN_KEEP_BITS, SAVED_ATTN_KEEP_BITS = range(8)
+SAVED_RES1_KEEP_BITS, SAVED_RES2_KEEP_BITS = 8, 9
 
 vp, i32, u32, u64, f32, sz = C.c_void_p, C.c_int32, C.c_uint32, C.c_uint64, C.c_float, C.c_size_t
 
@@ -50,6 +51,7 @@
 DESC_STREAM16, DESC_STREAM16_IN, DESC_STREAM16_OUT = 0x10000, 0x20000, 0x40000
 EINVAL, EUNSUPPORTED, EWORKSPACE, ELAUNCH, EALIGN = -1, -2, -3, -4, -5
 DESC_ATTN_KEEP_BITS = 0x80000
+DESC_RES_KEEP_BITS = 0x100000
 
 
 class TimCastItem(C.Structure):
@@ -73,7 +75,8 @@
     _fields_ = [("out0", vp), ("out1", vp), ("bias", vp), ("res", vp), ("aux", vp),
                 ("ld0", i32), ("ld1", i32), ("ldres", i32), ("ldaux", i32),
                 ("p_drop", f32), ("site", u32), ("seed", u64), ("mask", vp), ("ldmask", i32), ("reserved", i32),
-                ("ln_stats", vp), ("ln_w", vp), ("ln_b", vp), ("acc_scale", vp), ("a_wrap_k", i32), ("reserved2", i32)]
+                ("ln_stats", vp), ("ln_w", vp), ("ln_b", vp), ("acc_scale", vp), ("a_wrap_k", i32), ("reserved2", i32),
+                ("keep_out", vp)]
 
 
 class TimGemmItem(C.Structure):
@@ -189,6 +192,8 @@
     "timhip_gather_ranges": (C.c_int, [i32, vp, i32, i32, i32, i32, vp, vp, vp, vp]),
     "timhip_layernorm_fwd2": (C.c_int, [i32, vp, i32, i32, i32, i32, vp, vp, i32, vp, vp, vp, i32, vp, i32, vp, vp]),
     "timhip_layernorm_bwd2": (C.c_int, [i32, vp, i32, vp, i32, vp, i32, i32, i32, vp, i32, vp, vp, i32, vp, i32, vp, vp, vp, vp, vp, vp]),
+    "timhip_layernorm_bwd3": (C.c_int, [i32, vp, i32, vp, i32, vp, i32, i32, i32, vp, vp, i32, vp, i32, f32, u64, u32, vp, vp, vp, vp, i32,
+                                        vp, i32, vp, vp, sz, vp]),
     "timhip_cast_rows_pair": (C.c_int, [i32, vp, vp, vp, vp, i32, f32, u64, vp, vp]),
     "timhip_gather_split3_ranges": (C.c_int, [i32, vp, i32, i32, i32, i32, vp, vp, vp, vp]),
     "timhip_scatter_ranges_add": (C.c_int, [i32, i32, i32, i32, vp, vp, vp, vp, vp]),
diff --git a/tim_amd/csrc/api.hip b/tim_amd/csrc/api.hip
--- a/tim_amd/csrc/api.hip
+++ b/tim_amd/csrc/api.hip
@@ -4,7 +4,7 @@
 namespace {
 
 struct SavedLayout {
-  Field qkv, o, lse, y1, st1, x1t, u, h, y2, st2, ffn_mask, attn_keep;
+  Field qkv, o, lse, y1, st1, x1t, u, h, y2, st2, ffn_mask, attn_keep, res1_keep, res2_keep;
   size_t total;
 };
 
@@ -24,6 +24,8 @@
   L.st2 = a.take(M * 2 * 4);
   L.ffn_mask = a.take(M * d.FF / 8);
   L.attn_keep = a.take((size_t)d.B * d.H * d.S * 16);
+  L.res1_keep = a.take(M * d.E / 8);
+  L.res2_keep = a.take(M * d.E / 8);
   L.total = a.total();
   return L;
 }
@@ -120,7 +122,7 @@
   TimEpi e;
   e.out0 = e.out1 = nullptr; e.bias = e.res = nullptr; e.aux = nullptr;
   e.ld0 = e.ld1 = e.ldres = e.ldaux = 0; e.p_drop = 0.f; e.site = 0; e.seed = 0;
-  e.mask = nullptr; e.ldmask = 0; e.reserved = 0; e.a_wrap_k = 0; e.reserved2 = 0;
+  e.mask = nullptr; e.ldmask = 0; e.reserved = 0; e.a_wrap_k = 0; e.reserved2 = 0; e.keep_out = nullptr;
   e.ln_stats = e.ln_w = e.ln_b = nullptr;
   e.acc_scale = nullptr;
   return e;
@@ -276,6 +278,8 @@
     case TIMHIP_SAVED_Y2: f = &L.y2; break;
     case TIMHIP_SAVED_FFN_KEEP_BITS: f = &L.ffn_mask; break;
     case TIMHIP_SAVED_ATTN_KEEP_BITS: f = &L.attn_keep; break;
+    case TIMHIP_SAVED_RES1_KEEP_BITS: f = &L.res1_keep; break;
+    case TIMHIP_SAVED_RES2_KEEP_BITS: f = &L.res2_keep; break;
     default: return TIMHIP_EINVAL;
   }
   *offset = f->off; *bytes = f->bytes;
@@ -314,13 +318,15 @@
 struct LayerBufs {
   void* qkv; void* o; float* lse; float* y1; float* st1; void* x1t; void* u; void* h; float* y2; float* st2;
   uint8_t* ffn_mask; const unsigned long long* attn_keep;
+  uint8_t* res1_keep; uint8_t* res2_keep;
 };
 
 static LayerBufs saved_bufs(const TimDesc& d, void* saved) {
   const SavedLayout L = saved_layout(d);
   return LayerBufs{L.qkv.at(saved), L.o.at(saved), (float*)L.lse.at(saved), (float*)L.y1.at(saved), (float*)L.st1.at(saved),
                    L.x1t.at(saved), L.u.at(saved), L.h.at(saved), (float*)L.y2.at(saved), (float*)L.st2.at(saved),
-                   (uint8_t*)L.ffn_mask.at(saved), reinterpret_cast<const unsigned long long*>(L.attn_keep.at(saved))};
+                   (uint8_t*)L.ffn_mask.at(saved), reinterpret_cast<const unsigned long long*>(L.attn_keep.at(saved)),
+                   (uint8_t*)L.res1_keep.at(saved), (uint8_t*)L.res2_keep.at(saved)};
 }
 
 static int layer_fwd_body(const TimDesc& d, const TimLayerParams* w, const float* x_in, const float* x_in_prenorm,
@@ -345,7 +351,9 @@
   }
   e.p_drop = d.p_drop; e.seed = d.seed; e.site = layer_site(d.layer, SITE_L_DROP1);
   uint8_t* fmask = d.p_drop > 0.f ? bufs.ffn_mask : nullptr;
-  const bool fuse_ln = tim_knobs().fuse_ln == 1;
+  const bool res_keep = (d.reserved & TIMHIP_DESC_RES_KEEP_BITS) != 0 && d.p_drop > 0.f && bufs.res1_keep && bufs.res2_keep;
+  e.keep_out = res_keep ? bufs.res1_keep : nullptr;
+  const bool fuse_ln = tim_knobs().fuse_ln == 1 && !res_keep;
   const uint32_t* ln_run_if = nullptr;
   bool fused1 = false;
   if (fuse_ln && h16_storage(prec) && !split(TIMHIP_DESC_OUTPROJ_SPLIT)) {
@@ -370,6 +378,7 @@
   e.out0 = y2; e.ld0 = E; e.bias = w->l2_b; e.ldres = E;
   e.res = y1; e.ln_stats = st1; e.ln_w = w->n1_w; e.ln_b = w->n1_b;
   e.p_drop = d.p_drop; e.seed = d.seed; e.site = layer_site(d.layer, SITE_L_DROP2);
+  e.keep_out = res_keep ? bufs.res2_keep : nullptr;
   bool fused2 = false;
   if (fuse_ln && h16_storage(prec) && !split(TIMHIP_DESC_L2_SPLIT)) {
     TimLnFuse lf{x_out_T, E, x_out, E, st2, w->n2_w, w->n2_b, nullptr, 0, 0.f, 0, 0};
@@ -439,8 +448,8 @@
   hipStream_t s = (hipStream_t)stream;
   void* ws = workspace;
   const LayerBufs bufs{L.qkv.at(ws), L.o.at(ws), nullptr, (float*)L.y1.at(ws), (float*)L.st1.at(ws), L.x1t.at(ws), nullptr,
-                       L.h.at(ws), (float*)L.y2.at(ws), (float*)L.st2.at(ws), nullptr, nullptr};
-  d.reserved &= ~TIMHIP_DESC_ATTN_KEEP_BITS;
+                       L.h.at(ws), (float*)L.y2.at(ws), (float*)L.st2.at(ws), nullptr, nullptr, nullptr, nullptr};
+  d.reserved &= ~(TIMHIP_DESC_ATTN_KEEP_BITS | TIMHIP_DESC_RES_KEEP_BITS);
   for (int l = 0; l < nlayers; ++l) {
     const bool last = l == nlayers - 1;
     const int s0 = (last && tail_only) ? d.F : 0;
@@ -491,11 +500,14 @@
   const bool s16 = gs_in != nullptr && (d.reserved & TIMHIP_DESC_STREAM16) != 0;
   const bool s16_in = s16 && (d.reserved & TIMHIP_DESC_STREAM16_IN) != 0;
   const bool s16_out = s16 && (d.reserved & TIMHIP_DESC_STREAM16_OUT) != 0;
+  const bool res_keep = (d.reserved & TIMHIP_DESC_RES_KEEP_BITS) != 0 && d.p_drop > 0.f;
+  const uint8_t* keep1 = res_keep ? (const uint8_t*)L.res1_keep.at(saved) : nullptr;
+  const uint8_t* keep2 = res_keep ? (const uint8_t*)L.res2_keep.at(saved) : nullptr;
   if (((d.reserved & (TIMHIP_DESC_STREAM16_IN | TIMHIP_DESC_STREAM16_OUT)) != 0 && !s16) || (s16_out && !dx_in_add)) return TIMHIP_EINVAL;
   if ((rc = tim_layernorm_bwd(prec, dx_out, E, y2, E, st2, M, E, 0, w->n2_w, f32a, E, df, E, d.p_drop, d.seed,
                               layer_site(d.layer, SITE_L_DROP2), g->n2_w, g->n2_b,
                               g->ln_partials ? g->ln_partials : lnp, s, g->ln_partials != nullptr, gs_in,
-                              dx_out_add, E, gs_out, (s16_in ? 1 : 0) | (s16 ? 2 : 0)))) return rc;
+                              dx_out_add, E, gs_out, (s16_in ? 1 : 0) | (s16 ? 2 : 0), 0, nullptr, nullptr, nullptr, keep2))) return rc;
   TimEpi e = epi0();
   e.out0 = du; e.ld0 = FF; e.aux = u; e.ldaux = FF;
   if ((rc = tim_gemm_nt(prec, TIMHIP_EPI_MULAUX_T, df, E, w->l2_wt, E, M, FF, E, e, 1, s))) return rc;
@@ -514,7 +526,7 @@
                               layer_site(d.layer, SITE_L_DROP1), g->n1_w, g->n1_b,
                               g->ln_partials ? g->ln_partials + tim_layernorm_bwd_ws(M, E) / sizeof(float) : lnp, s,
                               g->ln_partials != nullptr, gs_in, branch_split ? Tb : nullptr, E, gs_out,
-                              (s16 ? 1 : 0) | (s16_out ? 2 : 0)))) return rc;
+                              (s16 ? 1 : 0) | (s16_out ? 2 : 0), 0, nullptr, nullptr, nullptr, keep1))) return rc;
   e = epi0();
   e.out0 = Tc; e.ld0 = E;
   if ((rc = tim_gemm_nt(prec, TIMHIP_EPI_STORE_T, da, E, w->out_wt, E, M, E, E, e, 1, s))) return rc;
diff --git a/tim_amd/csrc/common.h b/tim_amd/csrc/common.h
--- a/tim_amd/csrc/common.h
+++ b/tim_amd/csrc/common.h
@@ -165,12 +165,14 @@
   const uint32_t w = wsel == 0 ? r.x : (wsel == 1 ? r.y : (wsel == 2 ? r.z : r.w));
   return ((w >> (16 * (e & 1))) & 0xffffu) >= (thr >> 16) ? scale : 0.f;
 }
-__device__ __forceinline__ uint32_t drop_bits8(uint64_t seed, uint32_t site, uint64_t c, uint32_t thr) {
-  const Philox4 r = philox4x32_7(seed, site, c);
+__device__ __forceinline__ uint32_t keep_byte(const Philox4& r, uint32_t thr) {
   const uint32_t t = thr >> 16;
   return ((r.x & 0xffffu) >= t ? 1u : 0u) | ((r.x >> 16) >= t ? 2u : 0u) | ((r.y & 0xffffu) >= t ? 4u : 0u) |
          ((r.y >> 16) >= t ? 8u : 0u) | ((r.z & 0xffffu) >= t ? 16u : 0u) | ((r.z >> 16) >= t ? 32u : 0u) |
          ((r.w & 0xffffu) >= t ? 64u : 0u) | ((r.w >> 16) >= t ? 128u : 0u);
+}
+__device__ __forceinline__ uint32_t drop_bits8(uint64_t seed, uint32_t site, uint64_t c, uint32_t thr) {
+  return keep_byte(philox4x32_7(seed, site, c), thr);
 }
 
 __device__ __forceinline__ uint32_t drop_bits32(uint64_t seed, uint32_t site, uint64_t q0, uint32_t thr) {
@@ -404,7 +406,8 @@
                       const float* t_scale = nullptr,
                       const void* add_T = nullptr, int ldadd = 0, const float* add_scale = nullptr,
                       int stream16 = 0,
-                      int split_row = 0, const float* w2 = nullptr, float* dgamma2 = nullptr, float* dbeta2 = nullptr);
+                      int split_row = 0, const float* w2 = nullptr, float* dgamma2 = nullptr, float* dbeta2 = nullptr,
+                      const uint8_t* keep_bits = nullptr);
 size_t tim_layernorm_bwd_ws(int rows, int cols);
 int tim_layernorm_bwd_blocks(int rows);
 int tim_attention_fwd(const TimDesc& d, const void* qkv, void* o, float* lse, hipStream_t s, const unsigned long long* kbits = nullptr,
diff --git a/tim_amd/csrc/gemm.hip b/tim_amd/csrc/gemm.hip
--- a/tim_amd/csrc/gemm.hip
+++ b/tim_amd/csrc/gemm.hip
@@ -307,6 +307,7 @@
             float4 ka, kb;
             drop_mask4_words(odd ? pa : r.x, odd ? pb : r.y, e.thr, e.scale, ka.x, ka.y, ka.z, ka.w);
             drop_mask4_words(odd ? r.z : pa, odd ? r.w : pb, e.thr, e.scale, kb.x, kb.y, kb.z, kb.w);
+            if (e.keep_out && m_ < M && n_ < N) e.keep_out[(size_t)m_ * (size_t)(N >> 3) + (size_t)(n_ >> 3)] = (uint8_t)keep_byte(r, e.thr);
             quad(it, true, ka);
             quad(it + 1, true, kb);
           }
@@ -687,6 +688,7 @@
   e.scale = te.p_drop > 0.f ? 1.f / (1.f - te.p_drop) : 1.f;
   e.site = te.site; e.seed = te.seed;
   e.mask = (const uint8_t*)te.mask; e.ldmask = te.ldmask;
+  e.keep_out = (epi == TIMHIP_EPI_DROP_RES_F32 && te.p_drop > 0.f && !te.mask && (N % 8) == 0) ? (uint8_t*)te.keep_out : nullptr;
   e.ln_stats = te.ln_stats; e.ln_w = te.ln_w; e.ln_b = te.ln_b;
   e.acc_scale = te.acc_scale;
   e.a_wrap = te.a_wrap_k / 64;
diff --git a/tim_amd/csrc/gemm_epi.h b/tim_amd/csrc/gemm_epi.h
--- a/tim_amd/csrc/gemm_epi.h
+++ b/tim_amd/csrc/gemm_epi.h
@@ -11,6 +11,7 @@
   int ld0, ld1, ldres, ldaux;
   uint32_t thr; float scale; uint32_t site; TimSeed seed;
   const uint8_t* mask; int ldmask;
+  uint8_t* keep_out;
   const float* ln_stats; const float* ln_w; const float* ln_b;
   const float* acc_scale;
   int vec;
@@ -112,7 +113,12 @@
       k0 = kpre.x; k1 = kpre.y; k2 = kpre.z; k3 = kpre.w;
     } else if (e.mask)
       drop_mask4_bits((uint32_t)e.mask[(size_t)m * e.ldmask + (n >> 3)] >> (n & 4), e.scale, k0, k1, k2, k3);
-    else
+    else if (EPI == TIMHIP_EPI_DROP_RES_F32 && e.keep_out) {
+      const Philox4 r = philox4x32_7(e.seed, e.site, ((uint64_t)m * (uint64_t)N + (uint64_t)n) >> 3);
+      const bool hi = (n & 4) != 0;
+      drop_mask4_words(hi ? r.z : r.x, hi ? r.w : r.y, e.thr, e.scale, k0, k1, k2, k3);
+      if (!hi) e.keep_out[(size_t)m * (size_t)(N >> 3) + (size_t)(n >> 3)] = (uint8_t)keep_byte(r, e.thr);
+    } else
       drop_mask4(e.seed, e.site, ((uint64_t)m * (uint64_t)N + (uint64_t)n) >> 2, e.thr, e.scale, k0, k1, k2, k3);
   }
   if (e.vec && n + 3 < N) {
diff --git a/tim_amd/csrc/gemm_pp.hip b/tim_amd/csrc/gemm_pp.hip
--- a/tim_amd/csrc/gemm_pp.hip
+++ b/tim_amd/csrc/gemm_pp.hip
@@ -148,6 +148,7 @@
             float4 ka, kb;
             drop_mask4_words(odd ? pa : r.x, odd ? pb : r.y, e.thr, e.scale, ka.x, ka.y, ka.z, ka.w);
             drop_mask4_words(odd ? r.z : pa, odd ? r.w : pb, e.thr, e.scale, kb.x, kb.y, kb.z, kb.w);
+            if (e.keep_out && m_ < M && n_ < N) e.keep_out[(size_t)m_ * (size_t)(N >> 3) + (size_t)(n_ >> 3)] = (uint8_t)keep_byte(r, e.thr);
             quad(it, true, ka);
             quad(it + 1, true, kb);
           }
diff --git a/tim_amd/csrc/rowops.hip b/tim_amd/csrc/rowops.hip
--- a/tim_amd/csrc/rowops.hip
+++ b/tim_amd/csrc/rowops.hip
@@ -405,8 +405,13 @@
   }
 }
 
-template <typename T, int LN_MAXV, bool ACT0 = false, int S16 = 0>
-__global__ __launch_bounds__(256) void ln_bwd_kernel(const float* __restrict__ dx, int lddx,
+#if defined(TIMHIP_LN_BITS_WPE) && TIMHIP_LN_BITS_WPE > 1
+#define LN_BWD_BOUNDS(BITS_) __launch_bounds__(256, (BITS_) ? TIMHIP_LN_BITS_WPE : 1)
+#else
+#define LN_BWD_BOUNDS(BITS_) __launch_bounds__(256)
+#endif
+template <typename T, int LN_MAXV, bool ACT0 = false, int S16 = 0, bool BITS = false>
+__global__ LN_BWD_BOUNDS(BITS) void ln_bwd_kernel(const float* __restrict__ dx, int lddx,
                                                      const float* __restrict__ y, int ldy,
                                                      const float* __restrict__ stats, int rows, int cols, int act,
                                                      const float* __restrict__ w, float* __restrict__ dyf, int lddy,
@@ -415,7 +420,7 @@
                                                      float* __restrict__ dbeta, int rows_pb,
                                                      float* __restrict__ partial, const float* __restrict__ t_scale,
                                                      const T* __restrict__ addt, int ldadd, const float* __restrict__ add_scale,
-                                                     LnSplit sp, int pair_sw) {
+                                                     LnSplit sp, int pair_sw, const uint8_t* __restrict__ kbits) {
   extern __shared__ float red[];
   if (blockIdx.x * rows_pb >= sp.row) { w = sp.w2; dgamma = sp.dg2; dbeta = sp.db2; }
   const float ts = t_scale ? *t_scale : 1.f;
@@ -437,6 +442,8 @@
   typedef T t4_t __attribute__((ext_vector_type(4)));
   t4_t an[LN_MAXV], dn16[LN_MAXV];
   float2 stn = make_float2(0.f, 0.f);
+  uint32_t kn[BITS ? LN_MAXV : 1];
+  const bool use_bits = BITS && thr != 0u && dyt != nullptr;
   auto fetch = [&](int row) {
     stn = *reinterpret_cast<const float2*>(stats + 2 * row);
 #pragma unroll
@@ -451,19 +458,22 @@
         if constexpr (IN16) dn16[i] = *reinterpret_cast<const t4_t*>(reinterpret_cast<const T*>(dx) + (size_t)row * lddx + c);
         else dn[i] = *reinterpret_cast<const float4*>(dx + (size_t)row * lddx + c);
         if (addt) an[i] = *reinterpret_cast<const t4_t*>(addt + (size_t)row * ldadd + c);
+        if constexpr (BITS) { if (use_bits) kn[i] = kbits[((size_t)row * cols + c) >> 3]; }
       }
     }
   };
   if (r0 + wave < r1) fetch(r0 + wave);
   float kq[4] = {1.f, 1.f, 1.f, 1.f};
-  const bool pair_ok = (cols % 512) == 0 && nv <= LN_MAXV && pair_sw;
+  const bool pair_ok = !BITS && (cols % 512) == 0 && nv <= LN_MAXV && pair_sw;
 #pragma unroll 1
   for (int row = r0 + wave; row < r1; row += 4) {
     const float mean = stn.x, rstd = stn.y;
     float4 xh[LN_MAXV], d[LN_MAXV], ga[LN_MAXV];
+    uint32_t kc[BITS ? LN_MAXV : 1];
 #pragma unroll
     for (int i = 0; i < LN_MAXV; ++i) {
       xh[i] = tn[i];
+      if constexpr (BITS) kc[i] = kn[i];
       if constexpr (IN16) {
         d[i] = make_float4(OpT<T>::to_f(dn16[i][0]) * as, OpT<T>::to_f(dn16[i][1]) * as, OpT<T>::to_f(dn16[i][2]) * as,
                            OpT<T>::to_f(dn16[i][3]) * as);
@@ -534,7 +544,12 @@
         }
         if (dyt) {
           float k0 = kp[0], k1 = kp[1], k2 = kp[2], k3 = kp[3];
-          if (thr != 0u && !paired) {
+          if constexpr (BITS) {
+            if (use_bits) {
+              drop_mask4_bits(kc[i] >> (c & 4), scale, k0, k1, k2, k3);
+              k0 *= ts; k1 *= ts; k2 *= ts; k3 *= ts;
+            }
+          } else if (thr != 0u && !paired) {
             drop_mask4(seed, site, ((uint64_t)row * cols + c) >> 2, thr, scale, k0, k1, k2, k3);
             k0 *= ts; k1 *= ts; k2 *= ts; k3 *= ts;
           }
@@ -1163,8 +1178,11 @@
                       int rows, int cols, int act, const float* w, float* dyf, int lddy, void* dyt, int ldt,
                       float p_drop, uint64_t seed, uint32_t site, float* dgamma, float* dbeta, float* partial_ws,
                       hipStream_t s, bool defer_colsum, const float* t_scale, const void* addt, int ldadd,
-                      const float* add_scale, int stream16, int split_row, const float* w2, float* dgamma2, float* dbeta2) {
+                      const float* add_scale, int stream16, int split_row, const float* w2, float* dgamma2, float* dbeta2,
+                      const uint8_t* keep_bits) {
   if (!dx || !y || !stats || !w || rows <= 0) return TIMHIP_EINVAL;
+  if (keep_bits && (p_drop <= 0.f || !dyt)) keep_bits = nullptr;
+  if (keep_bits && cols % 8) return TIMHIP_EUNSUPPORTED;
   TimGemmScope timing((double)rows * cols * (8 + (addt ? 2 : 0) + (dyf ? 4 : 0) + (dyt ? (f32_storage(precision) ? 4 : 2) : 0)), s, 2);
   LnSplit sp{0x7fffffff, nullptr, nullptr, nullptr, nullptr};
   if (stream16 && (act != 0 || !h16_storage(precision) || !add_scale || !t_scale)) return TIMHIP_EUNSUPPORTED;
@@ -1186,9 +1204,10 @@
   const DropArgs dr = drop_args(p_drop);
   const int pair_sw = tim_knobs().ln_pair;
   const int nv = (cols + 255) / 256;
-#define LN_BWD(T_, NV, ACT0, S16) hipLaunchKernelGGL((ln_bwd_kernel<T_, NV, ACT0, S16>), grid, dim3(256), shmem, s, dx, lddx, y, ldy, stats, \
+#define LN_BWD_B(T_, NV, ACT0, S16, BITS) hipLaunchKernelGGL((ln_bwd_kernel<T_, NV, ACT0, S16, BITS>), grid, dim3(256), shmem, s, dx, lddx, y, ldy, stats, \
                                    rows, cols, act, w, dyf, lddy, (T_*)dyt, ldt, dr.thr, dr.scale, seed, site, dgamma, dbeta, rpb, partial_ws, \
-                                   t_scale, (const T_*)addt, ldadd, add_scale, sp, pair_sw)
+                                   t_scale, (const T_*)addt, ldadd, add_scale, sp, pair_sw, keep_bits)
+#define LN_BWD(T_, NV, ACT0, S16) do { if (keep_bits) LN_BWD_B(T_, NV, ACT0, S16, true); else LN_BWD_B(T_, NV, ACT0, S16, false); } while (0)
 #define LN_BWD_NV(T_, ACT0, S16) do { if (nv <= 1) LN_BWD(T_, 1, ACT0, S16); else if (nv <= 2) LN_BWD(T_, 2, ACT0, S16); \
                                       else if (nv <= 4) LN_BWD(T_, 4, ACT0, S16); else LN_BWD(T_, 8, ACT0, S16); } while (0)
   if (stream16) {
@@ -1200,6 +1219,7 @@
   }
 #undef LN_BWD_NV
 #undef LN_BWD
+#undef LN_BWD_B
   TIM_CHECK_LAUNCH();
   if (partial_ws && (dgamma || dbeta) && !defer_colsum) {
     hipLaunchKernelGGL(partial_colsum_kernel, dim3((2 * cols + 255) / 256, 32), dim3(256), 0, s, partial_ws,
@@ -1332,6 +1352,18 @@
                            seed, site, dgamma, dbeta, nullptr, (hipStream_t)stream, false, t_scale);
 }
 
+int timhip_layernorm_bwd3(int precision, const void* dx, int lddx, const float* y, int ldy, const float* stats, int rows, int cols,
+                          int act, const float* w, void* dy_res, int lddy, void* dy_T, int ldt, float p_drop, uint64_t seed,
+                          uint32_t site, float* dgamma, float* dbeta, const float* t_scale, const void* add_T, int ldadd,
+                          const float* add_scale, int stream16, const void* keep_bits, void* partial_ws, size_t partial_bytes,
+                          void* stream) {
+  if (stream16 < 0 || stream16 > 3) return TIMHIP_EINVAL;
+  if (partial_ws && (rows <= 0 || cols <= 0 || partial_bytes < tim_layernorm_bwd_ws(rows, cols))) return TIMHIP_EWORKSPACE;
+  return tim_layernorm_bwd(precision, (const float*)dx, lddx, y, ldy, stats, rows, cols, act, w, (float*)dy_res, lddy, dy_T, ldt, p_drop,
+                           seed, site, dgamma, dbeta, (float*)partial_ws, (hipStream_t)stream, partial_ws != nullptr, t_scale, add_T, ldadd, add_scale,
+                           stream16, 0, nullptr, nullptr, nullptr, (const uint8_t*)keep_bits);
+}
+
 int timhip_layernorm_fwd2(int precision, const float* y, int rows, int cols, int ldy, int act, const float* w, const float* b,
                           int split_row, const float* w2, const float* b2, float* x_f32, int ldx, void* x_T, int ldt, float* stats,
                           void* stream) {
diff --git a/tim_amd/functional.py b/tim_amd/functional.py
--- a/tim_amd/functional.py
+++ b/tim_amd/functional.py
@@ -319,12 +319,14 @@
         return self.nonfinite.read(reset)
 
     def gemm(self, epi, A, B, M, N, K, out0, ld0, out1=None, ld1=0, bias=None, res=None, ldres=0, aux=None,
-             ldaux=0, p_drop=0.0, seed=0, site=0, splitk=1, mask=None, ldmask=0, ln=None, acc_scale=None, rep=0, a_wrap_k=0):
+             ldaux=0, p_drop=0.0, seed=0, site=0, splitk=1, mask=None, ldmask=0, ln=None, acc_scale=None, rep=0, a_wrap_k=0,
+             keep_out=None):
         if M == 0 or N == 0:
             return
         st_, g_, b_ = ln if ln is not None else (None, None, None)
         e = L.TimEpi(ptr(out0), ptr(out1), ptr(bias), ptr(res), ptr(aux), ld0, ld1, ldres, ldaux,
-                     float(p_drop), site, seed, ptr(mask), ldmask, rep, ptr(st_), ptr(g_), ptr(b_), acc_scale, a_wrap_k, 0)
+                     float(p_drop), site, seed, ptr(mask), ldmask, rep, ptr(st_), ptr(g_), ptr(b_), acc_scale, a_wrap_k, 0,
+                     ptr(keep_out))
         call("timhip_gemm_nt", self.prec, epi, ptr(A), A.stride(0), ptr(B), B.stride(0), M, N, K,
              C.byref(e), splitk, _stream())
 
@@ -626,6 +628,8 @@
             desc.reserved |= L.DESC_ATTN_KEEP_BITS
         elif rc != L.EUNSUPPORTED:
             L.check(rc, "timhip_attn_keep_bits")
+    if q.p_enc > 0.0 and os.environ.get("TIM_AMD_RES_KEEP_BITS", "1") != "0":
+        desc.reserved |= L.DESC_RES_KEEP_BITS
     return desc, layer_saved
 
 
@@ -699,7 +703,7 @@
         else:
             call("timhip_layer_fwd_chained", C.byref(desc), C.byref(lp[0]), C.byref(lparams[l - 1][0]),
                  ptr(layer_saved[l - 1]), ptr(xs_t[l]), ptr(out_f), ptr(xs_t[l + 1]), ptr(layer_saved[l]), st)
-    return _Stack(layer_saved, xs_t, lparams, desc.reserved & L.DESC_ATTN_KEEP_BITS), xL_f
+    return _Stack(layer_saved, xs_t, lparams, desc.reserved & (L.DESC_ATTN_KEEP_BITS | L.DESC_RES_KEEP_BITS)), xL_f
 
 
 def _heads_fwd(q, P, xL_f, xL_t, outs, row0=0):
```

Result: no change. 332,700 interval-queries/s (median of 2 runs) (+0.0%).
